# richarddurbin/hash10x

Hardware: AMD Instinct MI355X
Metric: read-pairs/s through --readFQB + --hashDepthRange + --cluster (mosh construction + per-barcode clustering) (higher is better)
Workload: dtype u64; 1 GPU; yeast-like-2.5M; read_pairs=2500000, barcodes=10000, B=24, k=21, w=31, clusterThreshold=5, parallelism=single GPU

## Files before the change

### hash10x_amd/csrc/common.hpp

```cpp
#pragma once
#include <hip/hip_runtime.h>
#include <cstdint>
#include <cstdio>
#include <cstdarg>
#include <cstring>
#include <cstdlib>
#include <ctime>
#include <string>
#include <vector>
#include <map>
#include <mutex>
#include "../../include/h10x.h"

namespace h10x {

constexpr int WAVE = 64;
typedef unsigned long long u64;
typedef uint32_t u32;
typedef uint16_t u16;
typedef uint8_t  u8;

static_assert(sizeof(h10x_block) == 32, "ClusterBlock layout (hash10x.c:62-70)");
static_assert(sizeof(h10x_clushash) == 8, "ClusterHash layout (hash10x.c:35-43)");

struct DevCache {
  std::multimap<size_t, void *> parked; size_t parkedBytes = 0;
  static std::mutex &mu() { static std::mutex m; return m; }
  static DevCache &of(int device, hipStream_t st) { static std::map<std::pair<int, hipStream_t>, DevCache> m; return m[{device, st}]; }
  static bool disabled() { static int v = -1; if (v < 0) v = getenv("H10X_NOPOOL") != nullptr; return v != 0; }
  static unsigned long long &freshCalls() { static unsigned long long v = 0; return v; }
  static unsigned long long &freshBytes() { static unsigned long long v = 0; return v; }
  static int poison() { static int p = -1; if (p < 0) { const char *e = getenv("H10X_POISON"); p = e ? atoi(e) : 0; } return p; }
  void *takeLocked(size_t bytes, size_t &got) {
    auto it = parked.lower_bound(bytes);
    if (it == parked.end() || it->first > 2 * bytes + (1u << 20)) return nullptr;
    void *p = it->second; got = it->first; parkedBytes -= got; parked.erase(it);
    return p;
  }
  static void *take(int device, hipStream_t st, size_t bytes, size_t &got) {
    std::lock_guard<std::mutex> g(mu());
    void *p = of(device, st).takeLocked(bytes, got);
    if (!p && st) p = of(device, nullptr).takeLocked(bytes, got);
    return p;
  }
  static void park(int device, hipStream_t st, void *p, size_t bytes) {
    std::lock_guard<std::mutex> g(mu()); DevCache &c = of(device, st); c.parked.emplace(bytes, p); c.parkedBytes += bytes;
  }
  static void retireStream(int device, hipStream_t st) {
    std::lock_guard<std::mutex> g(mu());
    DevCache &c = of(device, st), &idle = of(device, nullptr);
    for (auto &kv : c.parked) { idle.parked.emplace(kv.first, kv.second); idle.parkedBytes += kv.first; }
    c.parked.clear(); c.parkedBytes = 0;
  }
  static void trim(int device) {
    std::lock_guard<std::mutex> g(mu());
    (void)hipDeviceSynchronize();
    static std::map<std::pair<int, hipStream_t>, DevCache> *dummy = nullptr; (void)dummy;
    for (hipStream_t st : streamsOf(device)) { DevCache &c = of(device, st); for (auto &kv : c.parked) (void)hipFree(kv.second); c.parked.clear(); c.parkedBytes = 0; }
  }
  static std::vector<hipStream_t> &streamsOf(int device) { static std::map<int, std::vector<hipStream_t>> m; auto &v = m[device]; if (v.empty()) v.push_back(nullptr); return v; }
  static void noteStream(int device, hipStream_t st) { std::lock_guard<std::mutex> g(mu()); auto &v = streamsOf(device); for (auto x : v) if (x == st) return; v.push_back(st); }
};
struct AllocScope {
  static hipStream_t &stream() { static thread_local hipStream_t s = nullptr; return s; }
  static int &device() { static thread_local int d = 0; return d; }
};
template <typename T> struct DevBuf {
  T *p = nullptr; size_t n = 0; size_t cap = 0; int dev = 0; hipStream_t st = nullptr;
  DevBuf() = default;
  DevBuf(const DevBuf &) = delete; DevBuf &operator=(const DevBuf &) = delete;
  ~DevBuf() { release(); }
  void release() {
    if (p) { if (DevCache::disabled()) (void)hipFree(p); else DevCache::park(dev, st, p, cap); }
    p = nullptr; n = 0; cap = 0;
  }
  hipError_t alloc(size_t count) {
    release();
    if (!count) count = 1;
    size_t bytes = (count * sizeof(T) + 255) & ~(size_t)255;
    dev = AllocScope::device(); st = AllocScope::stream();
    hipError_t e = hipSuccess;
    void *q = DevCache::disabled() ? nullptr : DevCache::take(dev, st, bytes, cap);
    if (!q) {
      static const bool log = getenv("H10X_ALLOC_LOG") != nullptr;
      timespec t0, t1; if (log) clock_gettime(CLOCK_MONOTONIC, &t0);
      cap = bytes; e = hipMalloc(&q, bytes);
      if (e != hipSuccess && !DevCache::disabled()) { DevCache::trim(dev); e = hipMalloc(&q, bytes); }
      if (e == hipSuccess) { __atomic_fetch_add(&DevCache::freshCalls(), 1, __ATOMIC_RELAXED); __atomic_fetch_add(&DevCache::freshBytes(), (unsigned long long)bytes, __ATOMIC_RELAXED); }
      if (log) { clock_gettime(CLOCK_MONOTONIC, &t1); fprintf(stderr, "h10x alloc: %.1f MB fresh, %.3f ms\n", bytes / 1e6, (t1.tv_sec - t0.tv_sec) * 1e3 + (t1.tv_nsec - t0.tv_nsec) / 1e6); }
    }
    if (e == hipSuccess) { p = (T *)q; n = count; } else { p = nullptr; cap = 0; }
    if (e == hipSuccess && DevCache::poison()) (void)hipMemsetAsync(p, 0xA5, bytes, AllocScope::stream());
    return e;
  }
  void swap(DevBuf &o) { std::swap(p, o.p); std::swap(n, o.n); std::swap(cap, o.cap); std::swap(dev, o.dev); std::swap(st, o.st); }
  size_t bytes() const { return n * sizeof(T); }
};

enum TimerId { T_RUNS = 0, T_MOSH, T_FALLBACK, T_COMPACT, T_SORT_HASH, T_RANK, T_PROBE, T_CLUSHASH, T_CSR,
               T_GOOD, T_CLUSTER, T_CLUSTER_K, T_CLUSTER_MAIN, T_SPLIT, T_COUNT };
static const char *const kTimerNames[T_COUNT] = {
  "block_runs", "mosh_extract", "mosh_fallback", "compact_entries", "sort_by_hash", "index_rank",
  "probe_table", "clushash_build", "csr_build", "good_hashes", "cluster", "cluster_kernel", "cluster_main", "cluster_split" };

struct Timer { hipEvent_t a = nullptr, b = nullptr; double ms = 0; uint64_t launches = 0; bool pending = false; };

enum XchgId { X_HOST_COUNTS = 0, X_ENTRIES, X_FIRST_COUNTS, X_INDEX_BACK, X_INDEX_DEPTH, X_LIST_HEADS, X_LIST_DATA, X_TABLES, X_OWNER_LISTS, X_GATHER, X_COUNT };
static const char *const kXchgNames[X_COUNT] = {
  "host_counts (small host allgathers: sizes, counts)", "entries_to_hash_owners (all-to-all)", "first_seen_counts (allgather)", "indices_back (all-to-all)",
  "index_depth (allgather)", "list_heads (allgather: index + length of the in-range hashes)", "list_data (allgather: the in-range barcode lists)",
  "hash_tables (allgather: hashValue, for --writeHash / the crib)", "owner_lists_rebuild (after --clusterSplit)", "gather_to_rank0" };
struct XchgStat { u64 calls = 0, bytesOut = 0, bytesIn = 0, maxPeerOut = 0; Timer t, tIn; int beside = -1; };

constexpr size_t ROWS_PAD = 128;
constexpr int MAX_SEGS = 8;
struct BlockSeg { u32 localStart, count, globalBase; };
struct SegMap {
  int n; BlockSeg s[MAX_SEGS];
  __host__ __device__ u32 globalOf(u32 l) const {
    for (int k = n - 1; k > 0; --k) if (l >= s[k].localStart) return s[k].globalBase + (l - s[k].localStart);
    return s[0].globalBase + l;
  }
};
struct ShardSegInfo { u32 rank, localStart, count, globalBase; u64 entries; };

struct Ctx {
  h10x_params prm{};
  u64 keyInv = 1; int keyShift = 0; int keyBits = 64;
  bool wantPacked = false; int entCodeBits = 0;
  int device = 0;
  hipStream_t stream = nullptr;
  hipStream_t aux[3] = {nullptr, nullptr, nullptr};
  hipEvent_t evFork = nullptr, evJoin[3] = {nullptr, nullptr, nullptr};
  int numCU = 256;
  bool ownStream = false;
  std::string err;

  DevBuf<u32> hashIndex;
  DevBuf<u64> hashValue;
  DevBuf<u32> hashDepth;
  DevBuf<u64> rowStart;
  DevBuf<u32> rows;
  DevBuf<h10x_block> blocks;
  DevBuf<u64> blockOff;
  DevBuf<h10x_clushash> clusHash;
  u32 hashNumber = 1, nBlocks = 0;
  u32 maxBlockHashes = 0xFFFFFFFFu;
  u64 nEntries = 0, nRecords = 0;
  bool haveState = false;

  DevBuf<u8>  within;
  DevBuf<u16> goodPos;
  DevBuf<u32> nGood;
  DevBuf<u64> goodRow;
  DevBuf<u32> goodEntries;
  DevBuf<u32> clusterRaw;
  bool haveRange = false, haveGood = false; int rangeMin = 0, rangeMax = 0;
  u32 rangeHiMax = 0;
  u32 depthBound = 0xFFFFFFFFu;
  u32 maxGoodDepth = 0, maxGood = 0, meanGood = 0;

  DevBuf<u32> cribCount[2];
  DevBuf<u64> cribFirst[2];
  DevBuf<int16_t> cribChr; DevBuf<u16> cribPos; DevBuf<u8> cribType;
  DevBuf<u32> cribHist;
  u32 cribHistDim = 0; int cribGenomes = 0; bool haveCrib = false;

  struct Comm *comm = nullptr; bool sharded = false;
  u32 codeBase = 0, nBlocksGlobal = 0;
  SegMap segs{1, {{0, 0, 0}}};
  std::vector<ShardSegInfo> allSegs;
  u64 nEntriesGlobal = 0, nRecordsGlobal = 0;
  int rowShift = 0;
  bool ownerListsStale = false;
  DevBuf<u32> oRows, oSegStart, oIndex; u32 oU = 0; u64 oM = 0;
  DevBuf<u64> oHash;
  bool tablesPending = false;

  int64_t optMaxSlots = 0;
  int64_t optClusterLds = 0;
  int64_t optFirstGlobal = 0;
  int64_t optFirstCap = 0;
  int64_t optClusterThreads0 = 0, optClusterBudget0 = 0;
  int64_t optBigRanks = 0;
  int64_t optPrivTable = 0;
  int64_t optProbedTable = 0;
  int64_t optNoPack = 0;
  int64_t optNarrowFirst = 0;
  int64_t optTrEstDiv = 0;
  int64_t optTrClassT = -1;
  int64_t optTrPacked = -1;
  int64_t optStamps = 0;
  int64_t optChunk = 0;
  int64_t optChunkEof = 1;
  std::vector<u64> mergePoints; bool replayDone = false;
  int64_t optRowShift = -1;
  int64_t optReplySort = 0;
  int64_t optOverlap = 1;
  int64_t optOwnerCut = 0;
  int64_t optDeltaLists = -1;
  int64_t optRowsFakeBase = 0;
  int64_t optNbBudget = 0;
  u64 nbStats[4] = {0, 0, 0, 0};
  DevBuf<u32> censusKeys; u64 censusN = 0; bool censusOpen = false;
  DevBuf<u32> censusCodes, censusCounts, censusGoodCodes, censusGoodCounts; u64 censusDistinct = 0, censusGood = 0; bool censusClosed = false;
  DevBuf<u64> wlSlots; u64 wlMask = 0, wlCodes = 0; bool haveWhitelist = false;
  int64_t optFqbSlab = 0;
  int64_t optMolGlobal = 0;
  DevBuf<u32> sgBlock, sgCount; DevBuf<u64> sgOffsets; u64 sgRows = 0; u32 sgCodeMin = 0, sgCodeMax = 0; bool haveShareGraph = false;
  DevBuf<u32> ingestBuf; u64 ingestRecords = 0, ingestCap = 0; bool ingestAsync = false;
  static constexpr int INGEST_SLOTS = 8; hipEvent_t ingestEv[INGEST_SLOTS] = {};
  int64_t optFaultInject = 0;
  int faultAt(int region) { if (optFaultInject != region) return 0; optFaultInject = 0; return fail("injected fault in fork/join region %d", region); }
  bool timing = false;
  u32 *startFlags = nullptr;
  Timer timers[T_COUNT];
  XchgStat xs[X_COUNT];
  h10x_counters ctr{};

  int fail(const char *fmt, ...) {
    char buf[1024]; va_list ap; va_start(ap, fmt); vsnprintf(buf, sizeof buf, fmt, ap); va_end(ap);
    err = buf; return -1;
  }
  static constexpr size_t MAIL_BYTES = 4096, MAIL_ITEMS = 12;
  unsigned char *mail = nullptr; size_t mailUsed = 0; u32 mailSeq = 0; bool mailDirect = false;
  struct PendingRead { void *dst; const void *dev; size_t off, n; };
  std::vector<PendingRead> pendingReads;
  int readback(void *dst, const void *dev, size_t n) {
    if (!mail) {
      if (hipHostMalloc((void **)&mail, MAIL_BYTES + 64, hipHostMallocCoherent | hipHostMallocMapped) != hipSuccess) { mail = nullptr; return fail("hipHostMalloc of the read-back mailbox failed"); }
      memset(mail, 0, MAIL_BYTES + 64);
    }
    const size_t off = mailUsed, step = (n + 7) & ~(size_t)7;
    if (off + step > MAIL_BYTES || pendingReads.size() >= MAIL_ITEMS) {
      mailDirect = true;
      return hipMemcpyAsync(dst, dev, n, hipMemcpyDeviceToHost, stream) == hipSuccess ? 0 : fail("hipMemcpyAsync (device to host) failed");
    }
    mailUsed += step; pendingReads.push_back(PendingRead{dst, dev, off, n});
    return 0;
  }
  int syncReadbacks();
  int forkStreams(int n) {
    if (!evFork) {
      if (hipEventCreateWithFlags(&evFork, hipEventDisableTiming) != hipSuccess) return fail("hipEventCreate failed");
      for (int i = 0; i < 3; ++i) {
        if (hipStreamCreateWithFlags(&aux[i], hipStreamNonBlocking) != hipSuccess) return fail("hipStreamCreate failed");
        if (hipEventCreateWithFlags(&evJoin[i], hipEventDisableTiming) != hipSuccess) return fail("hipEventCreate failed");
      }
    }
    if (hipEventRecord(evFork, stream) != hipSuccess) return fail("hipEventRecord failed");
    for (int i = 0; i < n; ++i) if (hipStreamWaitEvent(aux[i], evFork, 0) != hipSuccess) return fail("hipStreamWaitEvent failed");
    return 0;
  }
  hipStream_t xStream = nullptr; hipEvent_t evXFork = nullptr, evXDone = nullptr; bool xOpen = false;
  DevBuf<u32> xHold[4];
  int xFork() {
    if (!xStream) {
      if (hipStreamCreateWithFlags(&xStream, hipStreamNonBlocking) != hipSuccess) return fail("hipStreamCreate failed");
      if (hipEventCreateWithFlags(&evXFork, hipEventDisableTiming) != hipSuccess || hipEventCreateWithFlags(&evXDone, hipEventDisableTiming) != hipSuccess) return fail("hipEventCreate failed");
    }
    if (hipEventRecord(evXFork, stream) != hipSuccess || hipStreamWaitEvent(xStream, evXFork, 0) != hipSuccess) return fail("hipStreamWaitEvent failed");
    xOpen = true;
    return 0;
  }
  int xJoin() {
    if (!xOpen) return 0;
    xOpen = false;
    if (hipEventRecord(evXDone, xStream) != hipSuccess || hipStreamWaitEvent(stream, evXDone, 0) != hipSuccess) return fail("hipStreamWaitEvent failed");
    for (auto &b : xHold) b.release();
    return 0;
  }
  int joinStreams(int n) {
    for (int i = 0; i < n; ++i) {
      if (hipEventRecord(evJoin[i], aux[i]) != hipSuccess) return fail("hipEventRecord failed");
      if (hipStreamWaitEvent(stream, evJoin[i], 0) != hipSuccess) return fail("hipStreamWaitEvent failed");
    }
    return 0;
  }
  void tstart(Timer &x) {
    if (!timing) return;
    if (!x.a) { (void)hipEventCreate(&x.a); (void)hipEventCreate(&x.b); }
    flush(x);
    (void)hipEventRecord(x.a, stream);
  }
  void tstop(Timer &x) {
    if (!timing) return;
    (void)hipEventRecord(x.b, stream); x.pending = true; ++x.launches;
  }
  void flush(Timer &x) {
    if (x.pending) { float ms = 0; (void)hipEventSynchronize(x.b); (void)hipEventElapsedTime(&ms, x.a, x.b); x.ms += ms; x.pending = false; }
  }
  static constexpr int STAGE_DEPTH = 8;
  TimerId stageStack[STAGE_DEPTH]; int stageOpen = 0;
  TimerId stageTop = T_COUNT;
  Timer stageWait[T_COUNT];
  void stageReset() { stageOpen = 0; stageTop = T_COUNT; }
  void tstart(TimerId t) { if (stageOpen < STAGE_DEPTH) stageStack[stageOpen] = t; ++stageOpen; stageTop = t; tstart(timers[t]); }
  void tstop(TimerId t) {
    if (stageOpen > 0) --stageOpen;
    stageTop = stageOpen > 0 && stageOpen <= STAGE_DEPTH ? stageStack[stageOpen - 1] : T_COUNT;
    tstop(timers[t]);
  }
  void flush(TimerId t) { flush(timers[t]); }
};

struct ForkGuard {
  Ctx *c; bool armed = true;
  explicit ForkGuard(Ctx *c_) : c(c_) {}
  ForkGuard(const ForkGuard &) = delete; ForkGuard &operator=(const ForkGuard &) = delete;
  ~ForkGuard() { if (!armed) return; for (int i = 0; i < 3; ++i) if (c->aux[i]) (void)hipStreamSynchronize(c->aux[i]); (void)hipStreamSynchronize(c->stream); }
  void done() { armed = false; }
};

struct XGuard {
  Ctx *c;
  explicit XGuard(Ctx *c_) : c(c_) {}
  XGuard(const XGuard &) = delete; XGuard &operator=(const XGuard &) = delete;
  ~XGuard() { if (!c->xOpen) return; (void)hipStreamSynchronize(c->xStream); c->xOpen = false; for (auto &b : c->xHold) b.release(); }
};

#define H10X_HIP(ctx, call)                                                                      \
  do { hipError_t e__ = (call);                                                                  \
       if (e__ != hipSuccess) return (ctx)->fail("HIP error %s at %s:%d: %s", hipGetErrorName(e__), __FILE__, __LINE__, #call); } while (0)

#define H10X_TRY(expr) do { int rc__ = (expr); if (rc__) return rc__; } while (0)

static inline unsigned divUp(u64 a, u64 b) { return (unsigned)((a + b - 1) / b); }
template <typename T> static inline T hmin(T a, T b) { return a < b ? a : b; }
template <typename T> static inline T hmax(T a, T b) { return a > b ? a : b; }

__device__ __forceinline__ u32 probe_find(const u32 *__restrict__ table, const u64 *__restrict__ hashValue, int B, u64 h) {
  const u64 mask = ((u64)1 << B) - 1;
  u64 slot = h & mask; const u64 step = ((h >> B) & mask) | 1;
  u32 ix;
  while ((ix = table[slot]) && hashValue[ix] != h) slot = (slot + step) & mask;
  return ix;
}

int stageA_run(Ctx *c, const u32 *dRecords, u64 nRecords,
               DevBuf<u64> &entHash, DevBuf<u32> &entCode, DevBuf<u32> &entRead, bool hashLast = false, bool emptyIsNoBlock = false);
int stageA_sortRecords(Ctx *c, const u32 *dIn, u64 nRecords, u32 *dOut);
int stageA_runStarts(Ctx *c, const u32 *dRec, u64 nRec, std::vector<u64> &starts, std::vector<u32> &zeroRuns);
int replayChunks(const std::vector<u64> &starts, const std::vector<u32> &zeroRuns, u64 chunk, std::vector<u64> &merges, bool eofPass);
int stageB_run(Ctx *c, DevBuf<u64> &entHash, DevBuf<u32> &entCode, DevBuf<u32> &entRead);
void warm_prim(hipStream_t), warm_stageA(hipStream_t), warm_stageB(hipStream_t), warm_stageC(hipStream_t), warm_stageD(hipStream_t), warm_stageE(hipStream_t), warm_stageF(hipStream_t), warm_shard(hipStream_t);
int stageB_buildCSR(Ctx *c);
int stageB_finishClusHash(Ctx *c, DevBuf<u64> &key);
int stageB_finishClusHashFromReplies(Ctx *c, const u32 *replyIdx, const u32 *replyPos, const u32 *entRead);
#ifndef H10X_BS_T0
#define H10X_BS_T0 512
#define H10X_BS_I0 6
#define H10X_BS_T1 1024
#define H10X_BS_I1 6
#endif
constexpr u32 BLOCK_SORT_CAP0 = H10X_BS_T0 * H10X_BS_I0, BLOCK_SORT_CAP1 = H10X_BS_T1 * H10X_BS_I1, BLOCK_SORT_MAX = 8192;
int stageB_buildProbeTable(Ctx *c);
int stageB_blockClassLists(Ctx *c, DevBuf<u32> &lists, DevBuf<u32> &counts);
int stageC_depthRange(Ctx *c, int min, int max);
int stageC_cluster(Ctx *c, int codeMin, int codeMax, int threshold);
int stageC_split(Ctx *c);
int stageC_readMerge(Ctx *c, u32 code);
int stageD_cribGenome(Ctx *c, const u8 *hostCodes, const u64 *seqStart, u32 nSeq, int which, u64 *nPresent, u64 *nAbsent);
int stageD_cribFinish(Ctx *c);
int stageE_histMax(Ctx *c, int which, u64 first, u64 count, u32 *maxValue);
int stageE_histogram(Ctx *c, int which, u64 first, u64 count, u32 bins, u64 *hist);
int stageE_clusterReport(Ctx *c, u32 firstBlock, u32 nBlk, h10x_block_rep *hostB, h10x_cluster_rep *hostC, u64 clusterCap, u64 *nClusters);
int stageE_cribSummary(Ctx *c, u64 *counts12, u32 *hostSeenBase, u32 *hostSeenCluster);
int stageE_cribWords(Ctx *c, u64 first, u64 count, u32 *hostOut);
int stageF_neighbours(Ctx *c, u32 x, u32 *hash, u32 *count, u32 *first, u64 cap, u64 *n);
int stageF_neighbourMax(Ctx *c, const u32 *xs, u32 nq, u64 *maxKey, u32 *nNb);
int stageF_neighbourHist(Ctx *c, const u32 *xs, u32 nq, const u64 *offsets, u32 *hist);
int stageF_codeShare(Ctx *c, const u32 *codes, u32 nq, u64 *offsets, u32 *barcode, u32 *count, u32 *firstRank, u32 *firstHash, u64 cap);
int stageF_codeExplore(Ctx *c, int code, int threshold, u32 *out );
int stageF_codeCrib(Ctx *c, const u32 *codes, u32 n, u32 *out);
int stageL_run(Ctx *c, int64_t minShare, u32 codeMin, u32 codeMax, h10x_share_graph_info *info);
int stageL_get(Ctx *c, u64 *offsets, u32 *block, u32 *count, u64 cap, int toDevice);
void stageL_release(Ctx *c);
int stageJ_censusBegin(Ctx *c, u64 hint);
int stageJ_censusAdd(Ctx *c, const u32 *dRec, u64 n);
int stageJ_censusClose(Ctx *c, int64_t thresh, h10x_census_t *out);
int stageJ_censusExport(Ctx *c, int goodOnly, u32 *codes, u32 *counts, u64 cap);
int stageJ_whitelistSet(Ctx *c, const u32 *hostCodes, u64 n);
int stageJ_fix(Ctx *c, const u32 *dIn, u64 n, u32 *dOut, u64 *nKept, h10x_fix_stats *acc);
u64 stageJ_slab(const Ctx *c);
int stageK_map(Ctx *c, u32 *dMol, u32 *dSlot, u64 cap, h10x_molmap_info *info);
int stageK_records(Ctx *c, u64 *nRecords);
int stageK_split(Ctx *c, const u32 *dIn, u64 n, u32 *dOut, u64 *hostStart, u64 startCap);
int shard_allreduceU64(Ctx *c, u64 *v, u32 n, int op);
int shard_gatherBytes(Ctx *c, const void *send, u64 nbytes, void *recv, u64 cap, u64 *counts);
int shard_exchangeRows(Ctx *c);
int shard_split(Ctx *c, const u32 *dSubBefore, u32 totalSubLocal);
int shard_refreshLayout(Ctx *c);
int shard_materializeTables(Ctx *c);

// ... 47 lines not shown
```

### hash10x_amd/csrc/h10x_api.hip

```cpp
#include "common.hpp"
#include "comm.hpp"
#include "build_id.h"
#include <cstdlib>
#include <ctime>
#include <new>
#include <stdexcept>

using namespace h10x;

static int enter(Ctx &c) {
  if (hipSetDevice(c.device) != hipSuccess) return c.fail("hipSetDevice(%d) failed", c.device);
  AllocScope::stream() = c.stream; AllocScope::device() = c.device;
  DevCache::noteStream(c.device, c.stream);
  c.pendingReads.clear(); c.mailUsed = 0; c.mailDirect = false;
  c.stageReset();
  return 0;
}

struct h10x_ctx { Ctx c; };

extern "C" {

int h10x_abi_version(void) { return H10X_ABI_VERSION; }
const char *h10x_build_id(void) { return H10X_BUILD_ID; }
// ... 729 lines not shown

int h10x_molecule_map_device(h10x_ctx *h, uint32_t *dMol, uint32_t *dSlot, uint64_t cap, h10x_molmap_info *info) {
  if (!h) return -1;
  Ctx &c = h->c; H10X_TRY(enter(c));
  return stageK_map(&c, dMol, dSlot, cap, info);
}
int h10x_molecule_map(h10x_ctx *h, uint32_t *mol, uint32_t *slot, uint64_t cap, h10x_molmap_info *info) {
  if (!h) return -1;
  Ctx &c = h->c; H10X_TRY(enter(c));
  if (!mol && !slot) return stageK_map(&c, nullptr, nullptr, 0, info);
  u64 R = 0;
  H10X_TRY(stageK_records(&c, &R));
  if (cap < R) return c.fail("moleculeMap: room for %llu entries, the state holds %llu records", (u64)cap, R);
  DevBuf<u32> dMol, dSlot;
  if (mol) H10X_HIP(&c, dMol.alloc(R));
  if (slot) H10X_HIP(&c, dSlot.alloc(R));
  H10X_TRY(stageK_map(&c, mol ? dMol.p : nullptr, slot ? dSlot.p : nullptr, R, info));
  if (mol && R) H10X_HIP(&c, hipMemcpyAsync(mol, dMol.p, R * 4, hipMemcpyDeviceToHost, c.stream));
  if (slot && R) H10X_HIP(&c, hipMemcpyAsync(slot, dSlot.p, R * 4, hipMemcpyDeviceToHost, c.stream));
  H10X_HIP(&c, hipStreamSynchronize(c.stream));
  return 0;
}
int h10x_split_fqb_device(h10x_ctx *h, const uint32_t *dIn, uint64_t n, uint32_t *dOut, uint64_t *start, uint64_t startCap) {
  if (!h) return -1;
  Ctx &c = h->c; H10X_TRY(enter(c));
  if (n && (!dIn || !dOut)) return c.fail("h10x_split_fqb_device: null buffer");
  return stageK_split(&c, dIn, n, dOut, (u64 *)start, startCap);
}
int h10x_split_fqb(h10x_ctx *h, const uint32_t *in, uint64_t n, uint32_t *out, uint64_t *start, uint64_t startCap) {
  if (!h) return -1;
  Ctx &c = h->c; H10X_TRY(enter(c));
  if (n && (!in || !out)) return c.fail("h10x_split_fqb: null buffer");
  u64 R = 0;
  H10X_TRY(stageK_records(&c, &R));
  if (n != R) return c.fail("splitFQB: %llu records given, the state was read from %llu", (u64)n, R);
  if (n) { const uintptr_t a = (uintptr_t)in, b = (uintptr_t)out; if (a < b + n * 120 && b < a + n * 120) return c.fail("splitFQB: the input and output buffers overlap"); }
  DevBuf<u32> dIn, dOut;
  H10X_HIP(&c, dIn.alloc(n * 30)); H10X_HIP(&c, dOut.alloc(n * 30));
  if (n) H10X_HIP(&c, hipMemcpyAsync(dIn.p, in, n * 120, hipMemcpyHostToDevice, c.stream));
  H10X_TRY(stageK_split(&c, dIn.p, n, dOut.p, (u64 *)start, startCap));
  if (n) H10X_HIP(&c, hipMemcpyAsync(out, dOut.p, n * 120, hipMemcpyDeviceToHost, c.stream));
  H10X_HIP(&c, hipStreamSynchronize(c.stream));
  return 0;
}

int h10x_crib_genome(h10x_ctx *h, const uint8_t *codes, const uint64_t *seqStart, uint32_t nSeq, int which, uint64_t *nPresent, uint64_t *nAbsent) {
  if (!h) return -1;
  Ctx &c = h->c; H10X_TRY(enter(c));
  if (!seqStart || (seqStart[nSeq] && !codes)) return c.fail("h10x_crib_genome: null argument");
  return stageD_cribGenome(&c, codes, (const u64 *)seqStart, nSeq, which, (u64 *)nPresent, (u64 *)nAbsent);
}
int h10x_crib_finish(h10x_ctx *h) { if (!h) return -1; Ctx &c = h->c; H10X_TRY(enter(c)); return stageD_cribFinish(&c); }
int h10x_crib_sizes(h10x_ctx *h, uint32_t *histDim, uint32_t arrayMax[4]) {
  if (!h) return -1;
  Ctx &c = h->c; H10X_TRY(enter(c));
  if (!c.haveCrib) return c.fail("no crib: use cribBuild first");
  if (histDim) *histDim = c.cribHistDim;
  if (arrayMax) { H10X_HIP(&c, hipMemcpyAsync(arrayMax, c.cribHist.p + (size_t)4 * c.cribHistDim, 16, hipMemcpyDeviceToHost, c.stream)); H10X_HIP(&c, hipStreamSynchronize(c.stream)); }
  return 0;
}
int h10x_crib_export(h10x_ctx *h, int16_t *chr, uint16_t *pos, uint8_t *type, uint32_t *hist) {
  if (!h) return -1;
  Ctx &c = h->c; H10X_TRY(enter(c));
  if (!c.haveCrib) return c.fail("no crib: use cribBuild first");
  const size_t U1 = c.hashNumber;
  if (chr) H10X_HIP(&c, hipMemcpyAsync(chr, c.cribChr.p, U1 * 2, hipMemcpyDeviceToHost, c.stream));
  if (pos) H10X_HIP(&c, hipMemcpyAsync(pos, c.cribPos.p, U1 * 2, hipMemcpyDeviceToHost, c.stream));
  if (type) H10X_HIP(&c, hipMemcpyAsync(type, c.cribType.p, U1, hipMemcpyDeviceToHost, c.stream));
  if (hist) H10X_HIP(&c, hipMemcpyAsync(hist, c.cribHist.p, (size_t)4 * c.cribHistDim * 4, hipMemcpyDeviceToHost, c.stream));
  H10X_HIP(&c, hipStreamSynchronize(c.stream));
  return 0;
}
int h10x_export_ngood(h10x_ctx *h, uint32_t *nGood) {
  if (!h || !nGood) return -1;
  Ctx &c = h->c; H10X_TRY(enter(c));
  if (!c.haveGood) return c.fail("!! you must set hashDepthRange before clusterReport");
  H10X_HIP(&c, hipMemcpyAsync(nGood, c.nGood.p, (size_t)c.nBlocks * 4, hipMemcpyDeviceToHost, c.stream));
  H10X_HIP(&c, hipStreamSynchronize(c.stream));
  return 0;
}

int h10x_get_counters(h10x_ctx *h, h10x_counters *out) { if (!h || !out) return -1; *out = h->c.ctr; return 0; }

int h10x_shard_info(h10x_ctx *h, h10x_shard_info_t *out) {
  if (!h || !out) return -1;
  Ctx &c = h->c;
  if (!c.haveState) return c.fail("no hash state loaded: use readFQB or readHash first");
  memset(out, 0, sizeof *out);
  out->rank = c.sharded ? c.comm->rank : 0; out->nranks = c.sharded ? c.comm->n : 1;
  out->hashNumber = c.hashNumber; out->B = c.prm.B;
  if (c.sharded) { out->nBlocksGlobal = c.nBlocksGlobal; out->nEntriesGlobal = c.nEntriesGlobal; out->nRecordsGlobal = c.nRecordsGlobal; out->nSegs = (uint32_t)c.allSegs.size(); }
  else { out->nBlocksGlobal = c.nBlocks; out->nEntriesGlobal = c.nEntries; out->nRecordsGlobal = c.nRecords; out->nSegs = c.nBlocks > 1 ? 1 : 0; }
  return 0;
}
int h10x_shard_segments(h10x_ctx *h, h10x_shard_seg *out, uint32_t cap) {
  if (!h || !out) return -1;
  Ctx &c = h->c; H10X_TRY(enter(c));
  if (!c.haveState) return c.fail("no hash state loaded: use readFQB or readHash first");
  if (!c.sharded) {
    if (c.nBlocks <= 1) return 0;
    if (cap < 1) return c.fail("h10x_shard_segments: room for %u segments, 1 needed", cap);
    out[0] = h10x_shard_seg{0, 1, c.nBlocks - 1, 1, c.nEntries, 0, 0};
    return 0;
  }
  if (cap < c.allSegs.size()) return c.fail("h10x_shard_segments: room for %u segments, %zu needed", cap, c.allSegs.size());
  u64 g = 0;
  for (size_t i = 0; i < c.allSegs.size(); ++i) {
    const ShardSegInfo &s = c.allSegs[i];
    u64 local = 0;
    if ((int)s.rank == c.comm->rank) H10X_HIP(&c, hipMemcpy(&local, c.blockOff.p + s.localStart, 8, hipMemcpyDeviceToHost));
    out[i] = h10x_shard_seg{s.rank, s.localStart, s.count, s.globalBase, s.entries, local, g};
    g += s.entries;
  }
  return 0;
}
int h10x_shard_prepare_export(h10x_ctx *h) {
  if (!h) return -1;
  Ctx &c = h->c; H10X_TRY(enter(c));
  if (!c.haveState) return c.fail("no hash state loaded: use readFQB or readHash first");
  if (!c.sharded) return 0;
  return shard_materializeTables(&c);
}
int h10x_export_slice(h10x_ctx *h, int table, uint64_t first, uint64_t count, void *dst) {
  if (!h) return -1;
  Ctx &c = h->c; H10X_TRY(enter(c));
  if (!c.haveState) return c.fail("no hash state loaded: use readFQB or readHash first");
  if (!count) return 0;
  if (!dst) return c.fail("h10x_export_slice: null destination");
  const void *src = nullptr; size_t eb = 0; u64 limit = 0;
  switch (table) {
    case H10X_TABLE_HASHINDEX: src = c.hashIndex.p; eb = 4; limit = (u64)1 << c.prm.B; break;
    case H10X_TABLE_HASHVALUE: src = c.hashValue.p; eb = 8; limit = c.hashNumber; break;
    case H10X_TABLE_HASHDEPTH: src = c.hashDepth.p; eb = 4; limit = c.hashNumber; break;
    case H10X_TABLE_BLOCKS:    src = c.blocks.p; eb = sizeof(h10x_block); limit = c.nBlocks; break;
    case H10X_TABLE_CLUSHASH:  src = c.clusHash.p; eb = sizeof(h10x_clushash); limit = c.nEntries; break;
    case H10X_TABLE_CLUSTER_RAW: if (!c.clusterRaw.p || c.clusterRaw.n != 2 * (size_t)c.nBlocks) return c.fail("no --cluster has run on these blocks"); src = c.clusterRaw.p; eb = 8; limit = c.nBlocks; break;
    case H10X_TABLE_WITHIN:    if (!c.haveRange) return c.fail("no hashDepthRange set"); src = c.within.p; eb = 1; limit = c.hashNumber; break;
    case H10X_TABLE_NGOOD:     if (!c.haveGood) return c.fail("!! you must set hashDepthRange before clusterReport"); src = c.nGood.p; eb = 4; limit = c.nBlocks; break;
    default: return c.fail("h10x_export_slice: unknown table %d", table);
  }
  if ((table == H10X_TABLE_HASHINDEX || table == H10X_TABLE_HASHVALUE) && c.tablesPending) return c.fail("h10x_export_slice: call h10x_shard_prepare_export first (collective)");
  if (!src || first > limit || count > limit - first) return c.fail("h10x_export_slice: table %d, range %llu + %llu outside %llu", table, (u64)first, (u64)count, (u64)limit);
  H10X_HIP(&c, hipMemcpyAsync(dst, (const char *)src + first * eb, count * eb, hipMemcpyDeviceToHost, c.stream));
  H10X_HIP(&c, hipStreamSynchronize(c.stream));
  return 0;
}

int h10x_set_option(h10x_ctx *h, const char *name, int64_t value) {
  if (!h || !name) return -1;
  if (!strcmp(name, "stage_a_max_slots")) {
    if (value && (value < 256 || value > 16384 || (value & (value - 1)))) return h->c.fail("stage_a_max_slots must be a power of two in 256..16384 (or 0)");
    h->c.optMaxSlots = value; return 0;
  }
  if (!strcmp(name, "cluster_lds_budget")) { h->c.optClusterLds = value; return 0; }
  if (!strcmp(name, "cluster_first_global")) { h->c.optFirstGlobal = value; return 0; }
  if (!strcmp(name, "cluster_first_cap")) { h->c.optFirstCap = value; return 0; }
  if (!strcmp(name, "cluster_threads0")) { h->c.optClusterThreads0 = value; return 0; }
  if (!strcmp(name, "cluster_budget0")) { h->c.optClusterBudget0 = value; return 0; }
  if (!strcmp(name, "cluster_big_ranks")) { h->c.optBigRanks = value; return 0; }
  if (!strcmp(name, "cluster_narrow_first")) { h->c.optNarrowFirst = value; return 0; }
  if (!strcmp(name, "cluster_tr_packed")) { h->c.optTrPacked = value; return 0; }
  if (!strcmp(name, "cluster_tr_class_t")) { h->c.optTrClassT = value; return 0; }
  if (!strcmp(name, "cluster_tr_est_div")) { h->c.optTrEstDiv = value; return 0; }
  if (!strcmp(name, "index_no_pack")) { h->c.optNoPack = value; return 0; }
  if (!strcmp(name, "index_probed_table")) { if (value < 0 || value > 3) return h->c.fail("index_probed_table must be 0..3"); h->c.optProbedTable = value; return 0; }
  if (!strcmp(name, "index_priv_table")) { if (value < 0 || value > 3) return h->c.fail("index_priv_table must be 0..3"); h->c.optPrivTable = value; return 0; }
  if (!strcmp(name, "cluster_stamps")) { h->c.optStamps = value; return 0; }
  if (!strcmp(name, "chunk_size")) { if (value < 0) return h->c.fail("chunk_size must be >= 0"); h->c.optChunk = value; return 0; }
  if (!strcmp(name, "chunk_eof_pass")) { h->c.optChunkEof = value ? 1 : 0; return 0; }
  if (!strcmp(name, "fault_inject")) { h->c.optFaultInject = value; return 0; }
  if (!strcmp(name, "shard_row_shift")) { if (value < -1 || value > 8) return h->c.fail("shard_row_shift must be -1..8"); h->c.optRowShift = value; return 0; }
  if (!strcmp(name, "shard_reply_sort")) { if (value < 0 || value > 4) return h->c.fail("shard_reply_sort must be 0..4"); h->c.optReplySort = value; return 0; }
  if (!strcmp(name, "shard_overlap")) { h->c.optOverlap = value ? 1 : 0; return 0; }
  if (!strcmp(name, "shard_owner_cut")) { if (value < 0 || value > 1) return h->c.fail("shard_owner_cut must be 0 or 1"); h->c.optOwnerCut = value; return 0; }
  if (!strcmp(name, "shard_delta_lists")) { if (value < -1 || value > 1) return h->c.fail("shard_delta_lists must be -1, 0 or 1"); h->c.optDeltaLists = value; return 0; }
  if (!strcmp(name, "shard_rows_fake_base")) { if (value < 0) return h->c.fail("shard_rows_fake_base must be >= 0"); h->c.optRowsFakeBase = value; return 0; }
  if (!strcmp(name, "molmap_global")) { if (value < 0 || value > 1) return h->c.fail("molmap_global must be 0 or 1"); h->c.optMolGlobal = value; return 0; }
  if (!strcmp(name, "fqb_slab")) { if (value < 0 || value > (1 << 28)) return h->c.fail("fqb_slab must be 0..2^28"); h->c.optFqbSlab = value; return 0; }
  if (!strcmp(name, "neighbour_budget")) { if (value < 0) return h->c.fail("neighbour_budget must be >= 0"); h->c.optNbBudget = value; return 0; }
  return h->c.fail("unknown option %s", name);
}

}
```

### hash10x_amd/csrc/prim.hip

```cpp
#include "prim.hpp"
#include <thread>
#include <rocprim/rocprim.hpp>

namespace h10x {

#define PRIM_TWO_PHASE(c, t, CALL)                                                               \
  do { size_t bytes = 0; void *tmp = nullptr;                                                    \
       hipError_t e = (CALL);                                                                    \
       if (e != hipSuccess) return (c)->fail("rocPRIM size query failed: %s", hipGetErrorName(e)); \
       if (bytes > (t).buf.n) { e = (t).buf.alloc(bytes + (bytes >> 2));                         \
         if (e != hipSuccess) return (c)->fail("out of device memory for %zu bytes of sort/scan scratch", bytes); } \
       tmp = (t).buf.p;                                                                          \
       e = (CALL);                                                                               \
       if (e != hipSuccess) return (c)->fail("rocPRIM call failed: %s", hipGetErrorName(e)); } while (0)

int prim_exclusive_scan_u32(Ctx *c, PrimTemp &t, const u32 *in, u32 *out, size_t n) {
  if (!n) return 0;
  PRIM_TWO_PHASE(c, t, rocprim::exclusive_scan(tmp, bytes, in, out, (u32)0, n, rocprim::plus<u32>(), c->stream));
  return 0;
}
struct RunHead {
  const u64 *key; size_t n; int cb;
  __device__ u32 operator()(size_t i) const { return (i < n && (i == 0 || (key[i] >> cb) != (key[i - 1] >> cb))) ? 1u : 0u; }
};
int prim_run_ordinals_u64(Ctx *c, PrimTemp &t, const u64 *key, int cb, u32 *ord, size_t n) {
  auto flags = rocprim::make_transform_iterator(rocprim::counting_iterator<size_t>(0), RunHead{key, n, cb});
  PRIM_TWO_PHASE(c, t, rocprim::exclusive_scan(tmp, bytes, flags, ord, (u32)0, n + 1, rocprim::plus<u32>(), c->stream));
  return 0;
}
int prim_exclusive_scan_u32_u64(Ctx *c, PrimTemp &t, const u32 *in, u64 *out, size_t n) {
  if (!n) return 0;
  auto in64 = rocprim::make_transform_iterator(in, [] __device__(u32 v) -> u64 { return (u64)v; });
  PRIM_TWO_PHASE(c, t, rocprim::exclusive_scan(tmp, bytes, in64, out, (u64)0, n, rocprim::plus<u64>(), c->stream));
  return 0;
}
int prim_inclusive_scan_u32(Ctx *c, PrimTemp &t, const u32 *in, u32 *out, size_t n) {
  if (!n) return 0;
  PRIM_TWO_PHASE(c, t, rocprim::inclusive_scan(tmp, bytes, in, out, n, rocprim::plus<u32>(), c->stream));
  return 0;
}
int prim_sort_pairs_u64_u32(Ctx *c, PrimTemp &t, const u64 *kin, u64 *kout, const u32 *vin, u32 *vout, size_t n, int b0, int b1) {
  if (!n) return 0;
  PRIM_TWO_PHASE(c, t, rocprim::radix_sort_pairs(tmp, bytes, kin, kout, vin, vout, n, (unsigned)b0, (unsigned)b1, c->stream));
  return 0;
}
int prim_sort_pairs_u32_u32(Ctx *c, PrimTemp &t, const u32 *kin, u32 *kout, const u32 *vin, u32 *vout, size_t n, int b0, int b1) {
  if (!n) return 0;
  PRIM_TWO_PHASE(c, t, rocprim::radix_sort_pairs(tmp, bytes, kin, kout, vin, vout, n, (unsigned)b0, (unsigned)b1, c->stream));
  return 0;
}
struct MailArgs { const unsigned char *src[Ctx::MAIL_ITEMS]; u32 off[Ctx::MAIL_ITEMS], n[Ctx::MAIL_ITEMS]; u32 count; };
__global__ void mail_post_kernel(MailArgs a, unsigned char *mail, u32 *flag, u32 seq) {
  for (u32 i = 0; i < a.count; ++i)
    for (u32 b = threadIdx.x; b < a.n[i]; b += blockDim.x) mail[a.off[i] + b] = a.src[i][b];
  __threadfence_system();
  __syncthreads();
  if (threadIdx.x == 0) __hip_atomic_store(flag, seq, __ATOMIC_RELEASE, __HIP_MEMORY_SCOPE_SYSTEM);
}
int Ctx::syncReadbacks() {
  hipError_t e = hipSuccess;
  if (pendingReads.empty() || mailDirect) e = hipStreamSynchronize(stream);
  if (!pendingReads.empty() && e == hipSuccess) {
    MailArgs a; a.count = (u32)pendingReads.size();
    for (u32 i = 0; i < a.count; ++i) { a.src[i] = (const unsigned char *)pendingReads[i].dev; a.off[i] = (u32)pendingReads[i].off; a.n[i] = (u32)pendingReads[i].n; }
    u32 *flag = (u32 *)(mail + MAIL_BYTES);
    const u32 seq = ++mailSeq ? mailSeq : ++mailSeq;
    mail_post_kernel<<<1, 64, 0, stream>>>(a, mail, flag, seq);
    e = hipGetLastError();
    for (u64 spins = 0; e == hipSuccess && __atomic_load_n(flag, __ATOMIC_ACQUIRE) != seq; ++spins) {
#if !defined(__HIP_DEVICE_COMPILE__)
#if defined(__x86_64__) || defined(__i386__)
      __builtin_ia32_pause();
#else
      std::this_thread::yield();
#endif
#endif
      if ((spins & 0xFFF) == 0xFFF) {
        const hipError_t q = hipStreamQuery(stream);
        if (q == hipErrorNotReady) continue;
        if (q == hipSuccess && __atomic_load_n(flag, __ATOMIC_ACQUIRE) == seq) break;
        e = q == hipSuccess ? hipErrorUnknown : q;
      }
    }
    if (e == hipSuccess) for (const PendingRead &r : pendingReads) memcpy(r.dst, mail + r.off, r.n);
  }
  pendingReads.clear(); mailUsed = 0; mailDirect = false;
  return e == hipSuccess ? 0 : fail("HIP error %s at a read-back", hipGetErrorString(e));
}

int prim_sort_pairs_u32_v16(Ctx *c, PrimTemp &t, const u32 *kin, u32 *kout, const Val16 *vin, Val16 *vout, size_t n, int b0, int b1) {
  if (!n) return 0;
  PRIM_TWO_PHASE(c, t, rocprim::radix_sort_pairs(tmp, bytes, kin, kout, vin, vout, n, (unsigned)b0, (unsigned)b1, c->stream));
  return 0;
}
using SortKeys64Config = rocprim::radix_sort_config<rocprim::default_config, rocprim::default_config,
    rocprim::radix_sort_onesweep_config<rocprim::kernel_config<1024, 8>, rocprim::kernel_config<1024, 8>, 8, rocprim::block_radix_rank_algorithm::match>, 1024 * 1024>;
int prim_sort_keys_u64(Ctx *c, PrimTemp &t, const u64 *kin, u64 *kout, size_t n, int b0, int b1) {
  if (!n) return 0;
  PRIM_TWO_PHASE(c, t, rocprim::radix_sort_keys<SortKeys64Config>(tmp, bytes, kin, kout, n, (unsigned)b0, (unsigned)(b1 > 64 ? 64 : b1), c->stream));
  return 0;
}
int prim_sort_keys_u32(Ctx *c, PrimTemp &t, const u32 *kin, u32 *kout, size_t n, int b0, int b1) {
  if (!n) return 0;
  PRIM_TWO_PHASE(c, t, rocprim::radix_sort_keys(tmp, bytes, kin, kout, n, (unsigned)b0, (unsigned)(b1 > 32 ? 32 : b1), c->stream));
  return 0;
}
int prim_seg_sort_keys_u64(Ctx *c, PrimTemp &t, const u64 *kin, u64 *kout, u32 n, u32 nSeg, const u32 *begin, const u32 *end, int b0, int b1) {
  if (!n || !nSeg) return 0;
  PRIM_TWO_PHASE(c, t, rocprim::segmented_radix_sort_keys(tmp, bytes, kin, kout, n, nSeg, begin, end, (unsigned)b0, (unsigned)b1, c->stream));
  return 0;
}
int prim_seg_sort_keys_u32(Ctx *c, PrimTemp &t, const u32 *kin, u32 *kout, u32 n, u32 nSeg, const u32 *begin, const u32 *end, int b0, int b1) {
  if (!n || !nSeg) return 0;
  PRIM_TWO_PHASE(c, t, rocprim::segmented_radix_sort_keys(tmp, bytes, kin, kout, n, nSeg, begin, end, (unsigned)b0, (unsigned)b1, c->stream));
  return 0;
}
int prim_reduce_max_u32(Ctx *c, PrimTemp &t, const u32 *in, u32 *out, size_t n) {
  PRIM_TWO_PHASE(c, t, rocprim::reduce(tmp, bytes, in, out, (u32)0, n, rocprim::maximum<u32>(), c->stream));
  return 0;
}
int prim_reduce_sum_u32_u64(Ctx *c, PrimTemp &t, const u32 *in, u64 *out, size_t n) {
  auto in64 = rocprim::make_transform_iterator(in, [] __device__(u32 v) -> u64 { return (u64)v; });
  PRIM_TWO_PHASE(c, t, rocprim::reduce(tmp, bytes, in64, out, (u64)0, n, rocprim::plus<u64>(), c->stream));
  return 0;
}

__global__ void warm_prim_kernel() {}
void warm_prim(hipStream_t st) { warm_prim_kernel<<<1, 1, 0, st>>>(); }

}
```

### hash10x_amd/csrc/stage_a.hip

```cpp
#include "common.hpp"
#include <algorithm>
#include "prim.hpp"

namespace h10x {

constexpr u64 EMPTY64 = ~0ULL;
constexpr u32 NHASH_OVERFLOW = 0xFFFFFFFFu;
constexpr int MOSH_THREADS = 256;
constexpr int REC_TILE = 16;
constexpr int SEQ_WORDS = 12;

struct MoshConst {
  int k, w, shift1;
  int n1, n2;
  int run;
  u64 factor1;
};
#define H10X_MOSH_DBG(bit) false

__device__ __forceinline__ u64 kmer_window(const u32 *seq, int p, int k) {
  const int wi = p >> 4, s = (p & 15) * 2;
  const u64 hi = ((u64)seq[wi] << 32) | (u64)seq[wi + 1];
  const u32 lo = seq[wi + 2];
  const u64 x = s ? ((hi << s) | (u64)(lo >> (32 - s))) : hi;
  return x >> (64 - 2 * k);
}

__device__ __forceinline__ u64 revcomp_word(u64 x, int k) {
  u64 r = __brevll(~x);
  r = ((r & 0xAAAAAAAAAAAAAAAAULL) >> 1) | ((r & 0x5555555555555555ULL) << 1);
  return r >> (64 - 2 * k);
}

template <bool W31>
__device__ __forceinline__ bool divisible(u64 h, int w) {
  if (W31) {
    const u32 s = (u32)(h & 0x3FFFFFFFu) + (u32)((h >> 30) & 0x3FFFFFFFu) + (u32)(h >> 60);
    return (s % 31u) == 0;
  }
  return (h % (u64)w) == 0;
}

template <bool W31>
__device__ __forceinline__ bool mosh_of_slot(const u32 *seq, int t, const MoshConst &mc, u64 &h) {
  int p; const u32 *s;
  if (t < mc.n1) { p = 23 + t; s = seq; }
  else { p = t - mc.n1; s = seq + SEQ_WORDS; }
  const u64 f = kmer_window(s, p, mc.k);
  const u64 r = revcomp_word(f, mc.k);
  const u64 hf = (f * mc.factor1) >> mc.shift1;
  const u64 hr = (r * mc.factor1) >> mc.shift1;
  h = hf < hr ? hf : hr;
  return divisible<W31>(h, mc.w);
}

__device__ __forceinline__ void stage_records(const u32 *__restrict__ rec, u64 firstRec, int cnt, u32 *tile) {
  for (int t = threadIdx.x; t < cnt * 20; t += blockDim.x) {
    const int rr = t / 20, wi = t - rr * 20;
    const u32 v = rec[(firstRec + rr) * 30 + (wi < 10 ? wi : wi + 5)];
    tile[rr * 2 * SEQ_WORDS + (wi < 10 ? wi : wi + 2)] = v;
  }
}

__global__ void head_flags_kernel(const u32 *__restrict__ rec, u64 n, u32 *__restrict__ flags) {
  u64 i = (u64)blockIdx.x * blockDim.x + threadIdx.x;
  const u64 stride = (u64)gridDim.x * blockDim.x;
  for (; i < n; i += stride) flags[i] = (i == 0 || rec[i * 30] != rec[(i - 1) * 30]) ? 1u : 0u;
}

__global__ void block_starts_kernel(const u32 *__restrict__ flags, const u32 *__restrict__ code, u64 n, u32 nBlocks,
                                    u64 *__restrict__ startRec ) {
  u64 i = (u64)blockIdx.x * blockDim.x + threadIdx.x;
  const u64 stride = (u64)gridDim.x * blockDim.x;
  if (i == 0) { startRec[0] = 0; startRec[nBlocks] = n; }
  for (; i < n; i += stride) if (flags[i]) startRec[code[i]] = i;
}

__global__ void clear_heads_kernel(u32 *__restrict__ flags, const u64 *__restrict__ at, u32 n) {
  const u32 i = blockIdx.x * blockDim.x + threadIdx.x;
  if (i < n) flags[at[i]] = 0;
}
__global__ void zero_runs_kernel(const u32 *__restrict__ rec, const u64 *__restrict__ startRec, u32 nBlocks, u32 *__restrict__ list, u32 cap, u32 *__restrict__ count) {
  const u32 b = blockIdx.x * blockDim.x + threadIdx.x + 1;
  if (b < nBlocks && rec[startRec[b] * 30] == 0) { const u32 p = atomicAdd(count, 1u); if (p < cap) list[p] = b - 1; }
}

__global__ void classify_kernel(const u64 *__restrict__ startRec, u32 nBlocks, h10x_block *__restrict__ blocks,
                                u32 *__restrict__ slots, u32 maxSlots, int packedOK,
                                u32 *__restrict__ list0, u32 *__restrict__ list1, u32 *__restrict__ list2, u32 *__restrict__ listF,
                                u32 *__restrict__ counts , int hashLast) {
  const u32 c = blockIdx.x * blockDim.x + threadIdx.x;
  const int lane = threadIdx.x & (WAVE - 1);
  int cls = -1; u32 s = 0;
  if (c < nBlocks) {
    h10x_block b; memset(&b, 0, sizeof b);
    if (c > 0) {
      const u64 nr = startRec[c + 1] - startRec[c];
      b.nRead = (u32)nr;
      if (c + 1 < nBlocks || hashLast) {
        u64 want = 256; while (want < nr * 10) want <<= 1;
        if (packedOK && nr <= 65535 && want <= maxSlots) { s = (u32)want; cls = s <= 4096 ? 0 : (s <= 8192 ? 1 : 2); }
        else cls = 3;
      }
    }
    blocks[c] = b; slots[c] = s;
  }
  u32 *const lists[4] = {list0, list1, list2, listF};
#pragma unroll
  for (int k = 0; k < 4; ++k) {
    const u64 bal = __ballot(cls == k);
    if (!bal) continue;
    u32 base = 0;
    if (lane == 0) base = atomicAdd(&counts[k], (u32)__popcll(bal));
    base = (u32)__shfl((int)base, 0);
    if (cls == k) lists[k][base + (u32)__popcll(bal & ((1ULL << lane) - 1))] = c;
  }
}

__device__ __forceinline__ u32 lo32(u64 x) { return (u32)x; }
__device__ __forceinline__ u32 hi32(u64 x) { return (u32)(x >> 32); }
__device__ __forceinline__ u64 mk64(u32 hi, u32 lo) { return ((u64)hi << 32) | lo; }
__device__ __forceinline__ bool entry_empty(u64 v) {
  u32 t = lo32(v) & hi32(v);
  asm("" : "+v"(t));
  return t == 0xFFFFFFFFu;
}
__device__ __forceinline__ u32 set_slot_of(u32 hLo, u32 hHi, u32 mask) {
  return (((hLo ^ (hHi * 0x9E3779B1u)) * 0x85EBCA6Bu) >> 15) & mask;
}
__device__ __forceinline__ bool probe_done(u64 *table, u32 slot, u64 cur, u32 pLo, u32 pHi) {
  if (entry_empty(cur)) return true;
  if (hi32(cur) == pHi && ((lo32(cur) ^ pLo) >> 16) == 0) { atomicMin((u64 *)&table[slot], mk64(pHi, pLo)); return true; }
  return false;
}
constexpr u32 MOSH_QCAP = 96, MOSH_QKEEP = MOSH_QCAP - WAVE;
typedef __attribute__((address_space(3))) volatile u64 lds_queue_t;
__device__ __forceinline__ void queue_push(lds_queue_t *q, u32 &qn , bool ok, u32 hLo, u32 hHi, u32 read16 ) {
  const u64 bal = __builtin_amdgcn_ballot_w64(ok);
  if (!bal) return;
  const u32 pre = __builtin_amdgcn_mbcnt_hi((u32)(bal >> 32), __builtin_amdgcn_mbcnt_lo((u32)bal, 0u));
  if (ok) q[qn + pre] = mk64(hHi | read16, hLo);
  qn += (u32)__popcll(bal);
}
__device__ __forceinline__ bool queue_drain(u64 *table, u32 mask, lds_queue_t *q, u32 &qn, int lane) {
  const u32 n = qn < (u32)WAVE ? qn : (u32)WAVE;
  qn -= n;
  bool go = (u32)lane < n;
  u64 raw = 0;
  if (go) raw = q[qn + lane];
  const u32 hLo = lo32(raw), hHi = hi32(raw) & 0xFFFFu;
  const u32 pLo = (hLo << 16) | (hi32(raw) >> 16), pHi = __builtin_amdgcn_alignbit(hHi, hLo, 16);
  const u64 packed = mk64(pHi, pLo);
  u32 slot = set_slot_of(hLo, hHi, mask);
  for (u32 probes = 0; __builtin_amdgcn_ballot_w64(go); ++probes) {
    if (probes > mask) return false;
    if (go) {
      const u64 cur = atomicCAS((u64 *)&table[slot], EMPTY64, packed);
      if (probe_done(table, slot, cur, pLo, pHi)) go = false; else slot = (slot + 1) & mask;
    }
  }
  return true;
}

__device__ __forceinline__ void mul64_lo(u32 xLo, u32 xHi, u32 fLo, u32 fHi, u32 &pLo, u32 &pHi) {
  const u64 p = (u64)xLo * fLo;
  pLo = lo32(p); pHi = hi32(p) + xLo * fHi + xHi * fLo;
}

__device__ __forceinline__ void min64_halves(u32 aLo, u32 aHi, u32 bLo, u32 bHi, u32 &mLo, u32 &mHi) {
  asm("v_sub_co_u32 %0, vcc, %2, %4\n\tv_subb_co_u32 %0, vcc, %3, %5, vcc\n\tv_cndmask_b32 %0, %4, %2, vcc\n\tv_cndmask_b32 %1, %5, %3, vcc"
      : "=&v"(mLo), "=&v"(mHi) : "v"(aLo), "v"(aHi), "v"(bLo), "v"(bHi) : "vcc");
}
__device__ __forceinline__ u64 roll_product(u64 p, u64 t) {
  u64 r;
  asm("v_lshl_add_u64 %0, %1, 2, %2" : "=v"(r) : "v"(p), "v"(t));
  return r;
}
__device__ __forceinline__ void revcomp_halves(u32 lo, u32 hi, int down , u32 &rLo, u32 &rHi) {
  u32 a = __builtin_bitreverse32(~lo), b = __builtin_bitreverse32(~hi);
  a = ((a >> 1) & 0x55555555u) | ((a << 1) & 0xAAAAAAAAu);
  b = ((b >> 1) & 0x55555555u) | ((b << 1) & 0xAAAAAAAAu);
  rLo = __builtin_amdgcn_alignbit(a, b, (u32)down); rHi = a >> down;
}

template <bool W31, int L , bool FAST>
__global__ __launch_bounds__(1024)
void mosh_lds_kernel(const u32 *__restrict__ rec, const u32 *__restrict__ list, u32 nList,
                     const u64 *__restrict__ startRec, const u32 *__restrict__ slots, const u64 *__restrict__ capOff,
                     MoshConst mc, u32 tableBytes ,
                     u64 *__restrict__ stHash, u32 *__restrict__ stRead, u32 *__restrict__ nHashOut) {
  extern __shared__ __align__(16) unsigned char smem[];
  if (blockIdx.x >= nList) return;
  const u32 code = list[blockIdx.x];
  const u32 S = slots[code], mask = S - 1;
  u64 *table = (u64 *)smem;
  lds_queue_t *queue = (lds_queue_t *)(smem + tableBytes) + (u32)__builtin_amdgcn_readfirstlane((int)(threadIdx.x / WAVE)) * MOSH_QCAP;
  u32 qn = 0;
  __shared__ u32 sOverflow, sCount;
  __shared__ u64 sRoll[32];
  const u64 rec0 = startRec[code];
  const u32 nRead = (u32)(startRec[code + 1] - rec0);

  for (u32 i = threadIdx.x; i < S; i += blockDim.x) table[i] = EMPTY64;
  if (threadIdx.x == 0) { sOverflow = 0; sCount = 0; }
  if (FAST && threadIdx.x < 16) {
    const u64 a = threadIdx.x >> 2, b = threadIdx.x & 3, top = mc.factor1 << (2 * mc.k);
    sRoll[2 * threadIdx.x] = b * mc.factor1 - a * top;
    sRoll[2 * threadIdx.x + 1] = (3 - a) * mc.factor1 - (3 - b) * top;
  }
  __syncthreads();

  const int lane = threadIdx.x & (WAVE - 1), sub = lane & 31, wv = threadIdx.x / WAVE;
  const int lanes1 = (mc.n1 + L - 1) / L, lanes2 = (mc.n2 + L - 1) / L;
  int cnt = 0, pos0 = 0, wordBase = 0;
  if (sub < lanes1) { int t0 = sub * L; if (FAST) t0 = min(t0, mc.n1 - L); cnt = min(L, mc.n1 - t0); pos0 = 23 + t0; }
  else if (sub < lanes1 + lanes2) { int t0 = (sub - lanes1) * L; if (FAST) t0 = min(t0, mc.n2 - L); cnt = min(L, mc.n2 - t0); pos0 = t0; wordBase = 15; }
  const int sh = (pos0 & 15) * 2;
  const int wi = wordBase + (pos0 >> 4) - (FAST && sh == 0 ? 1 : 0);
  const u32 unal = (u32)(32 - sh) & 31u;
  const int k2 = 2 * mc.k, down = 64 - k2;
  const u32 pairsPerRound = (blockDim.x / WAVE) * 2;
  const u32 fLo = lo32(mc.factor1), fHi = hi32(mc.factor1);
  u32 r = (u32)wv * 2 + (u32)(lane >> 5);
  uint4 nx = make_uint4(0, 0, 0, 0);
  const u32 *pn = rec + (rec0 + r) * 30 + wi;
  if (r < nRead && cnt > 0) nx = make_uint4(pn[0], pn[1], pn[2], pn[3]);
  for (; __builtin_amdgcn_ballot_w64(r < nRead); r += pairsPerRound) {
    const uint4 cw = nx;
    const u32 rn = r + pairsPerRound;
    pn += (size_t)pairsPerRound * 30;
    if (rn < nRead && cnt > 0 && !H10X_MOSH_DBG(512)) nx = make_uint4(pn[0], pn[1], pn[2], pn[3]);
    if (H10X_MOSH_DBG(512)) nx = make_uint4(cw.y * 0x9E3779B1u + r, cw.x ^ 0x85EBCA6Bu, cw.w + cw.x, cw.z * 5u + 1u);
    const bool live = r < nRead && !H10X_MOSH_DBG(32);
    if (FAST) {
      const u32 x0 = __builtin_amdgcn_alignbit(cw.x, cw.y, unal), x1 = __builtin_amdgcn_alignbit(cw.y, cw.z, unal), x2 = __builtin_amdgcn_alignbit(cw.z, cw.w, unal);
      const u32 inw = __builtin_amdgcn_alignbit(x1, x2, (u32)down);
      u32 ta[L - 1];
      if constexpr (L == 8) {
        const u32 ze = (x0 & 0xCCCCCCCCu) | ((inw >> 2) & 0x33333333u), zo = ((x0 << 2) & 0xCCCCCCCCu) | (inw & 0x33333333u);
        const u32 zes = ze << 4, zos = zo << 4;
        ta[0] = (ze >> 24) & 0xF0u; ta[1] = (zo >> 24) & 0xF0u; ta[2] = (zes >> 24) & 0xF0u; ta[3] = (zos >> 24) & 0xF0u;
        ta[4] = (ze >> 16) & 0xF0u; ta[5] = (zo >> 16) & 0xF0u; ta[6] = (zes >> 16) & 0xF0u;
#pragma unroll
        for (int j = 0; j < L - 1; ++j) asm("" : "+v"(ta[j]));
      } else {
#pragma unroll
        for (int j = 0; j < L - 1; ++j) { ta[j] = (((x0 >> (30 - 2 * j)) & 3u) << 6) | (((inw >> (30 - 2 * j)) & 3u) << 4); asm("" : "+v"(ta[j])); }
      }
      u64 pr[L];
      {
        const u32 g0 = __builtin_amdgcn_alignbit(x0, x1, 32 - 2 * (L - 1)), g1 = __builtin_amdgcn_alignbit(x1, x2, 32 - 2 * (L - 1));
        u32 rl, rh;
        revcomp_halves(__builtin_amdgcn_alignbit(g0, g1, (u32)down), g0 >> down, down, rl, rh);
        u32 pl, ph;
        mul64_lo(rl, rh, fLo, fHi, pl, ph);
        pr[L - 1] = mk64(ph, pl);
      }
#pragma unroll
      for (int j = L - 2; j >= 0; --j) pr[j] = roll_product(pr[j + 1], *(const u64 *)((const char *)sRoll + ta[j] + 8));
      u64 pf;
      { u32 pl, ph; mul64_lo(__builtin_amdgcn_alignbit(x0, x1, (u32)down), x0 >> down, fLo, fHi, pl, ph); pf = mk64(ph, pl); }
      u32 thr = live && cnt > 0 ? 0xFFFFFFFFu / 31u + 1u : 0u;
      asm("" : "+v"(thr));
      const u32 r16 = r << 16;
#pragma unroll
      for (int j = 0; j < L; ++j) {
        u64 t = 0;
        if (j < L - 1) t = *(const u64 *)((const char *)sRoll + ta[j]);
        u32 mL, mH;
        min64_halves(lo32(pf), hi32(pf), lo32(pr[j]), hi32(pr[j]), mL, mH);
        const u32 hL = __builtin_amdgcn_alignbit(mH, mL, (u32)down), hH = mH >> down;
        bool ok;
        if (W31) ok = ((hL & 0x3FFFFFFFu) + __builtin_amdgcn_alignbit(hH, hL, 30)) * 0xBDEF7BDFu < thr;
        else ok = (mk64(hH, hL) % (u64)mc.w) == 0 && thr != 0;
        queue_push(queue, qn, ok, hL, hH, r16);
        if (H10X_MOSH_DBG(16)) { if (qn > MOSH_QKEEP) qn = 0; }
        else if (qn > MOSH_QKEEP && !queue_drain(table, mask, queue, qn, lane)) sOverflow = 1;
        if (j < L - 1) pf = roll_product(pf, t);
      }
      continue;
    }
    u64 hi = ((u64)cw.x << 32) | cw.y, lo = ((u64)cw.z << 32) | cw.w;
    if (sh) { hi = (hi << sh) | (lo >> (64 - sh)); lo <<= sh; }
    u64 f = hi >> down;
    u64 rc = revcomp_word(f, mc.k);
#pragma unroll
    for (int j = 0; j < L; ++j) {
      const u64 hf = (f * mc.factor1) >> mc.shift1;
      const u64 hr = (rc * mc.factor1) >> mc.shift1;
      const u64 h = hf < hr ? hf : hr;
      queue_push(queue, qn, divisible<W31>(h, mc.w) && live && j < cnt, lo32(h), hi32(h), r << 16);
      if (qn > MOSH_QKEEP && !queue_drain(table, mask, queue, qn, lane)) sOverflow = 1;
      hi = (hi << 2) | (lo >> 62); lo <<= 2;
      f = hi >> down;
      rc = (rc >> 2) | ((u64)(3u - ((u32)f & 3u)) << (k2 - 2));
    }
  }
  while (qn) if (!queue_drain(table, mask, queue, qn, lane)) { sOverflow = 1; break; }
  __syncthreads();

  const u64 out0 = capOff[code];
  const u32 cap = S - (S >> 3);
  for (u32 base = 0; base < (H10X_MOSH_DBG(64) ? 0u : S); base += blockDim.x) {
    const u32 i = base + threadIdx.x;
    const u64 v = i < S ? table[i] : EMPTY64;
    const bool valid = !entry_empty(v);
    const u64 bal = __ballot(valid);
    const int lane = threadIdx.x & (WAVE - 1);
    u32 wbase = 0;
    if (lane == 0 && bal) wbase = atomicAdd(&sCount, (u32)__popcll(bal));
    wbase = __shfl(wbase, 0);
    if (valid) {
      const u32 pos = wbase + (u32)__popcll(bal & ((1ULL << lane) - 1));
      if (pos < cap) { stHash[out0 + pos] = mk64(hi32(v) >> 16, __builtin_amdgcn_alignbit(hi32(v), lo32(v), 16)); stRead[out0 + pos] = lo32(v) & 0xFFFFu; }
    }
  }
  __syncthreads();
  if (threadIdx.x == 0) {
    u32 n = sCount;
    if (sOverflow || n > cap) n = NHASH_OVERFLOW;
    else if (n == 0) { stHash[out0] = 0; stRead[out0] = 0; n = 1; }
    nHashOut[code] = n;
  }
}

template <bool W31>
__global__ __launch_bounds__(MOSH_THREADS)
void mosh_raw_kernel(const u32 *__restrict__ rec, u64 rec0, u32 nRead, MoshConst mc, u64 *__restrict__ rawKey, u32 *__restrict__ rawSlot) {
  __shared__ u32 tile[REC_TILE * 2 * SEQ_WORDS];
  const int nk = mc.n1 + mc.n2;
  for (u32 i = threadIdx.x; i < REC_TILE * 2 * SEQ_WORDS; i += blockDim.x) tile[i] = 0;
  for (u32 r0 = blockIdx.x * REC_TILE; r0 < nRead; r0 += gridDim.x * REC_TILE) {
    const int cnt = (int)min((u32)REC_TILE, nRead - r0);
    __syncthreads();
    stage_records(rec, rec0 + r0, cnt, tile);
    __syncthreads();
    for (int rr = 0; rr < cnt; ++rr)
      for (int t = threadIdx.x; t < nk; t += blockDim.x) {
        u64 h; const bool ok = mosh_of_slot<W31>(tile + rr * 2 * SEQ_WORDS, t, mc, h);
        const u64 slot = (u64)(r0 + rr) * nk + t;
        rawKey[slot] = ok ? h : EMPTY64;
        rawSlot[slot] = (u32)slot;
      }
  }
}

__global__ void unique_flags_kernel(const u64 *__restrict__ key, u64 n, u32 *__restrict__ flags) {
  u64 i = (u64)blockIdx.x * blockDim.x + threadIdx.x;
  const u64 stride = (u64)gridDim.x * blockDim.x;
  for (; i < n; i += stride) flags[i] = (key[i] != EMPTY64 && (i == 0 || key[i] != key[i - 1])) ? 1u : 0u;
}
__global__ void unique_scatter_kernel(const u64 *__restrict__ key, const u32 *__restrict__ slot, const u32 *__restrict__ flags,
                                      const u32 *__restrict__ pos, u64 n, u32 nk, u64 *__restrict__ outHash, u32 *__restrict__ outRead) {
  u64 i = (u64)blockIdx.x * blockDim.x + threadIdx.x;
  const u64 stride = (u64)gridDim.x * blockDim.x;
  for (; i < n; i += stride) if (flags[i]) { outHash[pos[i]] = key[i]; outRead[pos[i]] = slot[i] / nk; }
}

__global__ void set_nhash_kernel(h10x_block *__restrict__ blocks, const u32 *__restrict__ nHash, u32 nBlocks) {
  const u32 c = blockIdx.x * blockDim.x + threadIdx.x;
  if (c < nBlocks) blocks[c].nHash = nHash[c];
}

struct SrcPtr { const u64 *hash; const u32 *read; };
__global__ void count_overflow_kernel(const u32 *__restrict__ nHash, u32 nBlocks, u32 *__restrict__ count) {
  const u32 c = blockIdx.x * blockDim.x + threadIdx.x;
  const u64 bal = __ballot(c < nBlocks && nHash[c] == NHASH_OVERFLOW);
  if ((threadIdx.x & (WAVE - 1)) == 0 && bal) atomicAdd(count, (u32)__popcll(bal));
}

__global__ void compact_entries_kernel(const u64 *__restrict__ stHash, const u32 *__restrict__ stRead, const u64 *__restrict__ capOff,
                                       const SrcPtr *__restrict__ fb ,
                                       const u32 *__restrict__ nHash, const u64 *__restrict__ blockOff, u32 nBlocks,
                                       u64 keyInv, int keyShift, int codeBits ,
                                       u64 *__restrict__ entHash, u32 *__restrict__ entCode, u32 *__restrict__ entRead) {
  for (u32 c = blockIdx.x + 1; c < nBlocks; c += gridDim.x) {
    const u32 n = nHash[c]; if (!n) continue;
    const u64 *sh; const u32 *sr;
    if (fb[c].hash) { sh = fb[c].hash; sr = fb[c].read; } else { sh = stHash + capOff[c]; sr = stRead + capOff[c]; }
    const u64 o = blockOff[c];
    if (codeBits) for (u32 i = threadIdx.x; i < n; i += blockDim.x) { entHash[o + i] = (((sh[i] >> keyShift) * keyInv) << codeBits) | c; entRead[o + i] = sr[i]; }
    else for (u32 i = threadIdx.x; i < n; i += blockDim.x) { entHash[o + i] = (sh[i] >> keyShift) * keyInv; entCode[o + i] = c; entRead[o + i] = sr[i]; }
  }
}

__global__ void sort_keys_kernel(const u32 *__restrict__ rec, u64 n, u32 *__restrict__ key, u32 *__restrict__ idx) {
  u64 i = (u64)blockIdx.x * blockDim.x + threadIdx.x;
  const u64 stride = (u64)gridDim.x * blockDim.x;
  for (; i < n; i += stride) { key[i] = __builtin_bswap32(rec[i * 30]); idx[i] = (u32)i; }
}
__global__ void gather_records_kernel(const u32 *__restrict__ rec, const u32 *__restrict__ idx, u64 n, u32 *__restrict__ out) {
  u64 t = (u64)blockIdx.x * blockDim.x + threadIdx.x;
  const u64 stride = (u64)gridDim.x * blockDim.x, total = n * 30;
  for (; t < total; t += stride) { const u64 j = t / 30; const u32 w = (u32)(t - j * 30); out[t] = rec[(u64)idx[j] * 30 + w]; }
}
int stageA_sortRecords(Ctx *c, const u32 *dIn, u64 n, u32 *dOut) {
  hipStream_t st = c->stream; PrimTemp pt;
  if (n >= (1ULL << 32)) return c->fail("record sort: %llu records exceed this build's 2^32 limit", (u64)n);
  if (!n) return 0;
  DevBuf<u32> key, keyS, idx, idxS;
  H10X_HIP(c, key.alloc(n)); H10X_HIP(c, keyS.alloc(n)); H10X_HIP(c, idx.alloc(n)); H10X_HIP(c, idxS.alloc(n));
  const unsigned g = (unsigned)hmin<u64>(divUp(n, 256), 65535u * 4);
  sort_keys_kernel<<<g, 256, 0, st>>>(dIn, n, key.p, idx.p);
  H10X_TRY(prim_sort_pairs_u32_u32(c, pt, key.p, keyS.p, idx.p, idxS.p, n, 0, 32));
  gather_records_kernel<<<(unsigned)hmin<u64>(divUp(n * 30, 256), 65535u * 16), 256, 0, st>>>(dIn, idxS.p, n, dOut);
  H10X_HIP(c, hipGetLastError());
  H10X_HIP(c, hipStreamSynchronize(st));
  return 0;
}

int replayChunks(const std::vector<u64> &starts, const std::vector<u32> &zeroRuns, u64 chunk, std::vector<u64> &merges, bool eofPass) {
  merges.clear();
  const size_t R = starts.size() - 1; const u64 total = starts[R];
  if (!R || !total) return 0;
  std::vector<u32> zr(zeroRuns); std::sort(zr.begin(), zr.end());
  auto isZero = [&](size_t r) { return std::binary_search(zr.begin(), zr.end(), (u32)r); };
  auto runOf = [&](u64 pos) { return (size_t)(std::upper_bound(starts.begin(), starts.begin() + R, pos) - starts.begin()) - 1; };
  std::vector<size_t> swallowed;
  u64 pos = 0, head = 0; bool open = false, barcodeZero = true;
  while (pos < total) {
    const u64 carry = open ? pos - head : 0;
    if (chunk <= carry) return 1;
    if (barcodeZero && open) {
      const size_t r = runOf(pos);
      if (starts[r] == pos) { merges.push_back(pos); swallowed.push_back(r); }
    }
    if (!open) { head = pos; open = true; }
    const u64 end = head + chunk < total ? head + chunk : total;
    size_t q = runOf(end - 1);
    barcodeZero = isZero(q);
    while (std::binary_search(swallowed.begin(), swallowed.end(), q)) --q;
    head = starts[q];
    pos = end;
  }
  if (eofPass && open && total - head >= chunk) return 1;
  return 0;
}

int stageA_runStarts(Ctx *c, const u32 *dRec, u64 nRec, std::vector<u64> &starts, std::vector<u32> &zeroRuns) {
  hipStream_t st = c->stream; PrimTemp pt;
  starts.assign(1, 0); zeroRuns.clear();
  if (!nRec) return 0;
  DevBuf<u32> flags, code; DevBuf<u64> startRec;
  H10X_HIP(c, flags.alloc(nRec)); H10X_HIP(c, code.alloc(nRec));
  const unsigned g = (unsigned)hmin<u64>(divUp(nRec, 256), 65535u * 4);
  head_flags_kernel<<<g, 256, 0, st>>>(dRec, nRec, flags.p);
  H10X_TRY(prim_inclusive_scan_u32(c, pt, flags.p, code.p, nRec));
  u32 nRuns = 0;
  H10X_TRY(c->readback(&nRuns, code.p + (nRec - 1), 4));
  H10X_TRY(c->syncReadbacks());
  const u32 nBlocks = nRuns + 1;
  H10X_HIP(c, startRec.alloc((size_t)nBlocks + 1));
  block_starts_kernel<<<g, 256, 0, st>>>(flags.p, code.p, nRec, nBlocks, startRec.p);
  constexpr u32 ZCAP = 4096;
  DevBuf<u32> zl, zc; H10X_HIP(c, zl.alloc(ZCAP)); H10X_HIP(c, zc.alloc(1)); H10X_HIP(c, hipMemsetAsync(zc.p, 0, 4, st));
  zero_runs_kernel<<<divUp(nBlocks, 256), 256, 0, st>>>(dRec, startRec.p, nBlocks, zl.p, ZCAP, zc.p);
  starts.resize((size_t)nRuns + 1);
  H10X_HIP(c, hipMemcpyAsync(starts.data(), startRec.p + 1, ((size_t)nRuns + 1) * 8, hipMemcpyDeviceToHost, st));
  u32 nz = 0;
  H10X_TRY(c->readback(&nz, zc.p, 4));
  H10X_TRY(c->syncReadbacks());
  if (nz > ZCAP) return c->fail("%u separate runs of the all-A barcode: the input is not grouped by barcode", nz);
  zeroRuns.resize(nz);
  if (nz) { H10X_HIP(c, hipMemcpyAsync(zeroRuns.data(), zl.p, (size_t)nz * 4, hipMemcpyDeviceToHost, st)); H10X_HIP(c, hipStreamSynchronize(st)); }
  return 0;
}

int stageA_run(Ctx *c, const u32 *dRec, u64 nRec, DevBuf<u64> &entHash, DevBuf<u32> &entCode, DevBuf<u32> &entRead, bool hashLast, bool emptyIsNoBlock) {
  hipStream_t st = c->stream;
  PrimTemp pt;
  const int k = c->prm.k;
  MoshConst mc; mc.k = k; mc.w = c->prm.w; mc.shift1 = 64 - 2 * k; mc.factor1 = c->prm.factor1;
  mc.n1 = 127 - k + 1 > 0 ? 127 - k + 1 : 0;
  mc.n2 = 150 - k + 1 > 0 ? 150 - k + 1 : 0;
  mc.run = 8; while ((mc.n1 + mc.run - 1) / mc.run + (mc.n2 + mc.run - 1) / mc.run > 32) ++mc.run;
  const bool w31 = c->prm.w == 31;

  c->tstart(T_RUNS);
  u32 nBlocks = 2;
  DevBuf<u64> startRec;
  if (nRec) {
    DevBuf<u32> flags, code;
    H10X_HIP(c, flags.alloc(nRec)); H10X_HIP(c, code.alloc(nRec));
    const unsigned g = (unsigned)hmin<u64>(divUp(nRec, 256), 65535u * 4);
    if (c->optChunk > 0 && !c->replayDone) {
      std::vector<u64> starts; std::vector<u32> zeroRuns;
      H10X_TRY(stageA_runStarts(c, dRec, nRec, starts, zeroRuns));
      if (replayChunks(starts, zeroRuns, (u64)c->optChunk, c->mergePoints, c->optChunkEof != 0)) return c->fail("chunkSize too small");
    }
    c->replayDone = false;
    head_flags_kernel<<<g, 256, 0, st>>>(dRec, nRec, flags.p);
    if (!c->mergePoints.empty()) {
      DevBuf<u64> at; H10X_HIP(c, at.alloc(c->mergePoints.size()));
      H10X_HIP(c, hipMemcpyAsync(at.p, c->mergePoints.data(), c->mergePoints.size() * 8, hipMemcpyHostToDevice, st));
      clear_heads_kernel<<<divUp(c->mergePoints.size(), 256), 256, 0, st>>>(flags.p, at.p, (u32)c->mergePoints.size());
      H10X_HIP(c, hipStreamSynchronize(st));
      c->mergePoints.clear();
    }
    H10X_TRY(prim_inclusive_scan_u32(c, pt, flags.p, code.p, nRec));
    u32 nRuns = 0;
    H10X_TRY(c->readback(&nRuns, code.p + (nRec - 1), 4));
    H10X_TRY(c->syncReadbacks());
    nBlocks = nRuns + 1;
    H10X_HIP(c, startRec.alloc((size_t)nBlocks + 1));
    block_starts_kernel<<<g, 256, 0, st>>>(flags.p, code.p, nRec, nBlocks, startRec.p);
  } else {
    if (emptyIsNoBlock) nBlocks = 1;
    H10X_HIP(c, startRec.alloc(3));
    H10X_HIP(c, hipMemsetAsync(startRec.p, 0, 24, st));
  }
  c->nBlocks = nBlocks; c->nRecords = nRec;
  H10X_HIP(c, c->blocks.alloc(nBlocks));

  u32 maxSlots = 16384;
  if (c->optMaxSlots > 0) maxSlots = (u32)c->optMaxSlots;
  const int packedOK = (2 * k + 16 <= 64) ? 1 : 0;
  DevBuf<u32> slots, list0, list1, list2, listF, counts, nHash;
  H10X_HIP(c, slots.alloc(nBlocks)); H10X_HIP(c, list0.alloc(nBlocks)); H10X_HIP(c, list1.alloc(nBlocks)); H10X_HIP(c, list2.alloc(nBlocks));
  H10X_HIP(c, listF.alloc(nBlocks)); H10X_HIP(c, counts.alloc(4)); H10X_HIP(c, nHash.alloc((size_t)nBlocks + 1));
  H10X_HIP(c, hipMemsetAsync(counts.p, 0, 16, st));
  H10X_HIP(c, hipMemsetAsync(nHash.p, 0, ((size_t)nBlocks + 1) * 4, st));
  classify_kernel<<<divUp(nBlocks, 256), 256, 0, st>>>(startRec.p, nBlocks, c->blocks.p, slots.p, maxSlots, packedOK,
                                                      list0.p, list1.p, list2.p, listF.p, counts.p, hashLast ? 1 : 0);
  DevBuf<u64> capOff; H10X_HIP(c, capOff.alloc((size_t)nBlocks + 1));
  H10X_TRY(prim_exclusive_scan_u32_u64(c, pt, slots.p, capOff.p, nBlocks));
  u32 hc[4]; u64 capTotal = 0; u32 lastSlots = 0;
  H10X_TRY(c->readback(hc, counts.p, 16));
  H10X_TRY(c->readback(&capTotal, capOff.p + (nBlocks - 1), 8));
  H10X_TRY(c->readback(&lastSlots, slots.p + (nBlocks - 1), 4));
  H10X_TRY(c->syncReadbacks());
  capTotal += lastSlots;
  c->tstop(T_RUNS);

  DevBuf<u64> stHash; DevBuf<u32> stRead;
  H10X_HIP(c, stHash.alloc(capTotal)); H10X_HIP(c, stRead.alloc(capTotal));
  c->tstart(T_MOSH);
  ForkGuard forkGuard(c);
  H10X_TRY(c->forkStreams(2));
#define H10X_MOSH_LAUNCH(W, LL, FK, TH, STREAM)                                                                                    \
    { if (lds > 48 * 1024) H10X_HIP(c, hipFuncSetAttribute((const void *)mosh_lds_kernel<W, LL, FK>, hipFuncAttributeMaxDynamicSharedMemorySize, (int)lds)); \
      mosh_lds_kernel<W, LL, FK><<<n, TH, lds, STREAM>>>(dRec, list, n, startRec.p, slots.p, capOff.p, mc, (u32)tableBytes, stHash.p, stRead.p, nHash.p); }
#define H10X_MOSH_CLASS(TH, STREAM)                                                                                                \
    { if (fastK && w31) H10X_MOSH_LAUNCH(true, 8, true, TH, STREAM) else if (fastK) H10X_MOSH_LAUNCH(false, 8, true, TH, STREAM)   \
      else if (w31 && mc.run == 8) H10X_MOSH_LAUNCH(true, 8, false, TH, STREAM) else if (w31) H10X_MOSH_LAUNCH(true, 9, false, TH, STREAM) \
      else if (mc.run == 8) H10X_MOSH_LAUNCH(false, 8, false, TH, STREAM) else H10X_MOSH_LAUNCH(false, 9, false, TH, STREAM) }
  const bool fastK = k >= 17 && k <= 30 && mc.run == 8;
  for (int cls = 2; cls >= 0; --cls) {
    const u32 n = hc[cls]; if (!n) continue;
    const u32 *list = cls == 0 ? list0.p : cls == 1 ? list1.p : list2.p;
    const size_t tableBytes = (size_t)hmin<u32>(4096u << cls, maxSlots) * 8;
    const size_t lds = tableBytes + (size_t)((cls == 2 ? 1024 : 512) / WAVE) * MOSH_QCAP * 8;
    if (cls == 2) H10X_MOSH_CLASS(1024, c->aux[0]) else if (cls == 1) H10X_MOSH_CLASS(512, c->aux[1]) else H10X_MOSH_CLASS(512, st)
    H10X_HIP(c, hipGetLastError());
  }
#undef H10X_MOSH_CLASS
#undef H10X_MOSH_LAUNCH
  H10X_TRY(c->faultAt(1));
  H10X_TRY(c->joinStreams(2));
  forkGuard.done();
  c->tstop(T_MOSH);

  DevBuf<u32> nOverflow; H10X_HIP(c, nOverflow.alloc(1)); H10X_HIP(c, hipMemsetAsync(nOverflow.p, 0, 4, st));
  count_overflow_kernel<<<divUp(nBlocks, 256), 256, 0, st>>>(nHash.p, nBlocks, nOverflow.p);
  H10X_HIP(c, c->blockOff.alloc((size_t)nBlocks + 1));
  H10X_TRY(prim_exclusive_scan_u32_u64(c, pt, nHash.p, c->blockOff.p, (size_t)nBlocks + 1));
  u64 H = 0, lastStart = 0; u32 hOverflow = 0, hMaxHash = 0xFFFFFFFFu;
  DevBuf<u32> dMaxHash; H10X_HIP(c, dMaxHash.alloc(1));
  H10X_TRY(prim_reduce_max_u32(c, pt, nHash.p, dMaxHash.p, nBlocks));
  H10X_TRY(c->readback(&hMaxHash, dMaxHash.p, 4));
  H10X_TRY(c->readback(&H, c->blockOff.p + nBlocks, 8));
  H10X_TRY(c->readback(&lastStart, startRec.p + (nBlocks - 1), 8));
  H10X_TRY(c->readback(&hOverflow, nOverflow.p, 4));
  H10X_TRY(c->syncReadbacks());
  const bool anyFallback = hc[3] || hOverflow;
  std::vector<u32> hNHash, hListF(hc[3]);
  std::vector<u64> hStart;
  if (anyFallback) {
    hNHash.resize(nBlocks + 1); hStart.resize(nBlocks + 1);
    H10X_HIP(c, hipMemcpyAsync(hNHash.data(), nHash.p, (size_t)nBlocks * 4, hipMemcpyDeviceToHost, st));
    H10X_HIP(c, hipMemcpyAsync(hStart.data(), startRec.p, ((size_t)nBlocks + 1) * 8, hipMemcpyDeviceToHost, st));
    if (hc[3]) H10X_HIP(c, hipMemcpyAsync(hListF.data(), listF.p, (size_t)hc[3] * 4, hipMemcpyDeviceToHost, st));
    H10X_HIP(c, hipStreamSynchronize(st));
    for (u32 b = 1; b + (hashLast ? 0 : 1) < nBlocks; ++b) if (hNHash[b] == NHASH_OVERFLOW) hListF.push_back(b);
  }
  std::vector<SrcPtr> hFb;
  std::vector<DevBuf<u64> *> keepH; std::vector<DevBuf<u32> *> keepR;
  c->ctr.fallback_blocks = hListF.size();
  if (!hListF.empty()) {
    hFb.assign(nBlocks, SrcPtr{nullptr, nullptr});
    c->tstart(T_FALLBACK);
    const u32 nk = (u32)(mc.n1 + mc.n2);
    for (u32 b : hListF) {
      const u32 nr = (u32)(hStart[b + 1] - hStart[b]);
      const u64 nSlot = (u64)nr * nk;
      DevBuf<u64> *oh = new DevBuf<u64>(); DevBuf<u32> *orr = new DevBuf<u32>(); keepH.push_back(oh); keepR.push_back(orr);
      u32 nUniq = 0;
      if (nSlot >= (1ULL << 32)) return c->fail("barcode block %u too large for the global mosh path (%llu k-mer slots)", b, (u64)nSlot);
      if (nSlot) {
        DevBuf<u64> k0, k1; DevBuf<u32> v0, v1, fl, ps;
        H10X_HIP(c, k0.alloc(nSlot)); H10X_HIP(c, k1.alloc(nSlot)); H10X_HIP(c, v0.alloc(nSlot)); H10X_HIP(c, v1.alloc(nSlot));
        H10X_HIP(c, fl.alloc(nSlot + 1)); H10X_HIP(c, ps.alloc(nSlot + 1));
        const unsigned g = (unsigned)hmin<u64>(divUp(nr, REC_TILE), 4096);
        if (w31) mosh_raw_kernel<true><<<g, MOSH_THREADS, 0, st>>>(dRec, hStart[b], nr, mc, k0.p, v0.p);
        else     mosh_raw_kernel<false><<<g, MOSH_THREADS, 0, st>>>(dRec, hStart[b], nr, mc, k0.p, v0.p);
        H10X_TRY(prim_sort_pairs_u64_u32(c, pt, k0.p, k1.p, v0.p, v1.p, nSlot, 0, 64));
        const unsigned g2 = (unsigned)hmin<u64>(divUp(nSlot, 256), 65535);
        unique_flags_kernel<<<g2, 256, 0, st>>>(k1.p, nSlot, fl.p);
        H10X_HIP(c, hipMemsetAsync(fl.p + nSlot, 0, 4, st));
        H10X_TRY(prim_exclusive_scan_u32(c, pt, fl.p, ps.p, nSlot + 1));
        H10X_HIP(c, hipMemcpyAsync(&nUniq, ps.p + nSlot, 4, hipMemcpyDeviceToHost, st));
        H10X_HIP(c, hipStreamSynchronize(st));
        H10X_HIP(c, oh->alloc(nUniq ? nUniq : 1)); H10X_HIP(c, orr->alloc(nUniq ? nUniq : 1));
        if (nUniq) unique_scatter_kernel<<<g2, 256, 0, st>>>(k1.p, v1.p, fl.p, ps.p, nSlot, nk, oh->p, orr->p);
        H10X_HIP(c, hipStreamSynchronize(st));
      } else { H10X_HIP(c, oh->alloc(1)); H10X_HIP(c, orr->alloc(1)); }
      if (!nUniq) {
        H10X_HIP(c, hipMemsetAsync(oh->p, 0, 8, st)); H10X_HIP(c, hipMemsetAsync(orr->p, 0, 4, st)); nUniq = 1;
      }
      hNHash[b] = nUniq; hFb[b] = SrcPtr{oh->p, orr->p};
    }
    H10X_HIP(c, hipMemcpyAsync(nHash.p, hNHash.data(), (size_t)nBlocks * 4, hipMemcpyHostToDevice, st));
    c->tstop(T_FALLBACK);
  }

  c->tstart(T_COMPACT);
  DevBuf<SrcPtr> dFb; H10X_HIP(c, dFb.alloc(nBlocks));
  if (hFb.empty()) H10X_HIP(c, hipMemsetAsync(dFb.p, 0, (size_t)nBlocks * sizeof(SrcPtr), st));
  else {
    H10X_HIP(c, hipMemcpyAsync(dFb.p, hFb.data(), (size_t)nBlocks * sizeof(SrcPtr), hipMemcpyHostToDevice, st));
    H10X_TRY(prim_exclusive_scan_u32_u64(c, pt, nHash.p, c->blockOff.p, (size_t)nBlocks + 1));
    H10X_HIP(c, hipMemcpyAsync(&H, c->blockOff.p + nBlocks, 8, hipMemcpyDeviceToHost, st));
    H10X_HIP(c, hipStreamSynchronize(st));
  }
  if (H >= (1ULL << 32)) return c->fail("%llu (barcode,hash) entries exceed this build's 2^32 per-GPU limit", (u64)H);
  c->nEntries = H;
  if (!hNHash.empty()) { hMaxHash = 0; for (u32 b = 0; b < nBlocks; ++b) hMaxHash = hNHash[b] > hMaxHash ? hNHash[b] : hMaxHash; }
  c->maxBlockHashes = hMaxHash;
  set_nhash_kernel<<<divUp(nBlocks, 256), 256, 0, st>>>(c->blocks.p, nHash.p, nBlocks);
  H10X_HIP(c, entHash.alloc(H)); H10X_HIP(c, entRead.alloc(H));
  {
    u64 m = (u64)c->prm.w; int s = 0; while (!(m & 1)) { m >>= 1; ++s; }
    u64 inv = m; for (int it = 0; it < 6; ++it) inv *= 2 - m * inv;
    const int k2 = 2 * c->prm.k; const u64 maxH = k2 >= 64 ? ~0ULL : ((u64)1 << k2) - 1, maxQ = maxH / (u64)c->prm.w;
    int b = 1; while (b < 64 && (maxQ >> b)) ++b;
    c->keyInv = inv; c->keyShift = s; c->keyBits = b;
    int cb = 1; while (cb < 32 && ((nBlocks - 1) >> cb)) ++cb;
    c->entCodeBits = (c->wantPacked && b + cb <= 63) ? cb : 0;
  }
  if (!c->entCodeBits) H10X_HIP(c, entCode.alloc(H));
  if (H) compact_entries_kernel<<<hmin<u32>(nBlocks, 8192), 256, 0, st>>>(stHash.p, stRead.p, capOff.p, dFb.p, nHash.p, c->blockOff.p, nBlocks,
                                                                        c->keyInv, c->keyShift, c->entCodeBits, entHash.p, entCode.p, entRead.p);
  H10X_HIP(c, hipGetLastError());
  if (!hFb.empty()) H10X_HIP(c, hipStreamSynchronize(st));
  c->tstop(T_COMPACT);
  for (auto *p : keepH) delete p;
  for (auto *p : keepR) delete p;

  u64 hashedPairs = hashLast ? nRec : (nBlocks >= 2 ? lastStart : 0);
  c->ctr.pairs = nRec; c->ctr.kmers = hashedPairs * (u64)(mc.n1 + mc.n2); c->ctr.entries = H;
  return 0;
}

__global__ void warm_stageA_kernel() {}
void warm_stageA(hipStream_t st) { warm_stageA_kernel<<<1, 1, 0, st>>>(); }

}
```

### hash10x_amd/csrc/stage_b.hip

```cpp
#include "common.hpp"
#include "prim.hpp"
#include <rocprim/block/block_radix_sort.hpp>

namespace h10x {

constexpr u32 SLOT_EMPTY = 0xFFFFFFFFu;
static int bitsFor(u64 maxValue) { int b = 1; while (b < 64 && (maxValue >> b)) ++b; return b; }

__global__ void seg_scatter_kernel(const u64 *__restrict__ sHash, const u32 *__restrict__ sCode,
                                   const u32 *__restrict__ ord, u64 n, u64 *__restrict__ dHash, u32 *__restrict__ dFirst,
                                   u32 *__restrict__ segStart, u32 *__restrict__ iota) {
  u64 i = (u64)blockIdx.x * blockDim.x + threadIdx.x;
  const u64 stride = (u64)gridDim.x * blockDim.x;
  for (; i < n; i += stride) if (ord[i + 1] != ord[i]) {
    const u32 d = ord[i];
    dHash[d] = sHash[i]; dFirst[d] = sCode[i]; segStart[d] = (u32)i; iota[d] = d;
  }
}
__global__ void seg_scatter_packed_kernel(const u64 *__restrict__ sKey, int cb,
                                          const u32 *__restrict__ ord, u64 n, Val16 *__restrict__ dVal, u32 *__restrict__ dFirst, u32 *__restrict__ rows) {
  u64 i = (u64)blockIdx.x * blockDim.x + threadIdx.x;
  const u64 stride = (u64)gridDim.x * blockDim.x;
  const u64 cmask = ((u64)1 << cb) - 1;
  for (; i < n; i += stride) {
    const u64 k = sKey[i]; const u32 code = (u32)(k & cmask);
    rows[i] = code;
    const u32 d = ord[i], d1 = ord[i + 1];
    if (d1 != d) { dVal[d].a = k >> cb; dVal[d].b = (u32)i; dFirst[d] = code; }
    if (i + 1 == n || ord[i + 2] != d1) dVal[d1 - 1].c = (u32)i + 1;
  }
}
__global__ void assign_index_v16_kernel(const Val16 *__restrict__ val, u32 U, u64 w , u64 *__restrict__ hashValue, u32 *__restrict__ hashDepth,
                                        u64 *__restrict__ rowStart) {
  const u32 i = blockIdx.x * blockDim.x + threadIdx.x;
  if (i == 0) { hashValue[0] = 0; hashDepth[0] = 0; rowStart[0] = 0; }
  if (i >= U) return;
  const Val16 v = val[i];
  hashValue[i + 1] = v.a * w; hashDepth[i + 1] = v.c - v.b; rowStart[i + 1] = v.b;
}

__global__ void assign_index_kernel(const u32 *__restrict__ order, const u64 *__restrict__ dHash, const u32 *__restrict__ segStart,
                                    u32 U, u64 w , u64 *__restrict__ hashValue, u32 *__restrict__ hashDepth, u64 *__restrict__ rowStart) {
  const u32 i = blockIdx.x * blockDim.x + threadIdx.x;
  if (i == 0) { hashValue[0] = 0; hashDepth[0] = 0; rowStart[0] = 0; }
  if (i >= U) return;
  const u32 d = order[i];
  hashValue[i + 1] = dHash[d] * w;
  hashDepth[i + 1] = segStart[d + 1] - segStart[d];
  rowStart[i + 1] = segStart[d];
}

__global__ void probe_insert_kernel(const u64 *__restrict__ hashValue, u32 hashNumber, int B, u32 *__restrict__ table) {
  const u32 first = blockIdx.x * blockDim.x + threadIdx.x + 1;
  const u64 mask = ((u64)1 << B) - 1;
  for (u32 start = first; start < hashNumber; start += gridDim.x * blockDim.x) {
    u32 cur = start;
    u64 h = hashValue[cur];
    u64 slot = h & mask, step = ((h >> B) & mask) | 1;
    for (;;) {
      const u32 old = atomicMin(&table[slot], cur);
      if (old == SLOT_EMPTY) break;
      if (old > cur) {
        cur = old; h = hashValue[cur]; step = ((h >> B) & mask) | 1;
      }
      slot = (slot + step) & mask;
    }
  }
}
__global__ void probe_finish_kernel(u32 *__restrict__ table, u64 n) {
  u64 i = (u64)blockIdx.x * blockDim.x + threadIdx.x;
  const u64 stride = (u64)gridDim.x * blockDim.x;
  for (; i < n; i += stride) if (table[i] == SLOT_EMPTY) table[i] = 0;
}

constexpr u64 SLOT_EMPTY64 = ~0ULL;
__global__ void probe_insert64_kernel(const u64 *__restrict__ hashValue, u32 hashNumber, int B, u64 w, int qBits, u64 *__restrict__ table) {
  const u32 first = blockIdx.x * blockDim.x + threadIdx.x + 1;
  const u64 mask = ((u64)1 << B) - 1, qmask = ((u64)1 << qBits) - 1;
  for (u32 start = first; start < hashNumber; start += gridDim.x * blockDim.x) {
    u64 h = hashValue[start];
    u64 cur = ((u64)start << qBits) | (h / w);
    u64 slot = h & mask, step = ((h >> B) & mask) | 1;
    for (;;) {
      const u64 old = atomicMin((unsigned long long *)&table[slot], (unsigned long long)cur);
      if (old == SLOT_EMPTY64) break;
      if (old > cur) {
        cur = old; h = (old & qmask) * w; step = ((h >> B) & mask) | 1;
      }
      slot = (slot + step) & mask;
    }
  }
}
__global__ void probe_insertP_kernel(const u64 *__restrict__ hashValue, u32 hashNumber, int B, int SH, int PB, u64 *__restrict__ table, u32 *__restrict__ fail) {
  const u32 first = blockIdx.x * blockDim.x + threadIdx.x + 1;
  const u64 mask = ((u64)1 << B) - 1, pmask = ((u64)1 << PB) - 1, umask = ((u64)1 << (SH - PB)) - 1;
  for (u32 start = first; start < hashNumber; start += gridDim.x * blockDim.x) {
    const u64 h = hashValue[start];
    u64 cur = ((u64)start << SH) | ((h >> B) << PB);
    u64 slot = h & mask, step = ((h >> B) & mask) | 1;
    for (;;) {
      const u64 old = atomicMin((unsigned long long *)&table[slot], (unsigned long long)cur);
      if (old == SLOT_EMPTY64) break;
      if (old > cur) { cur = old; step = (((cur >> PB) & umask) & mask) | 1; }
      if ((cur & pmask) == pmask) { *fail = 1; break; }
      ++cur;
      slot = (slot + step) & mask;
    }
  }
}
__global__ void probe_finish64_kernel(const u64 *__restrict__ table64, u64 n, int qBits, u32 *__restrict__ table) {
  u64 i = (u64)blockIdx.x * blockDim.x + threadIdx.x;
  const u64 stride = (u64)gridDim.x * blockDim.x;
  for (; i < n; i += stride) { const u64 e = table64[i]; table[i] = e == SLOT_EMPTY64 ? 0u : (u32)(e >> qBits); }
}
__global__ void lookup_pack64_kernel(const u64 *__restrict__ entHash , const u32 *__restrict__ entRead, u64 n,
                                     const u64 *__restrict__ table64, int B, u64 w, int qBits, int cb, u64 *__restrict__ key) {
  u64 i = (u64)blockIdx.x * blockDim.x + threadIdx.x;
  const u64 stride = (u64)gridDim.x * blockDim.x;
  const u64 mask = ((u64)1 << B) - 1, qmask = ((u64)1 << qBits) - 1;
  for (; i < n; i += stride) {
    const u64 q = entHash[i] >> cb, h = q * w;
    u64 slot = h & mask; const u64 step = ((h >> B) & mask) | 1;
    u64 e;
    while ((e = table64[slot]) != SLOT_EMPTY64 && (e & qmask) != q) slot = (slot + step) & mask;
    const u32 ix = e == SLOT_EMPTY64 ? 0u : (u32)(e >> qBits);
    key[i] = ((u64)ix << 32) | (u64)(entRead[i] & 0xFFFFu);
  }
}

constexpr u32 PRIV_MAX_DISP = 256;
__global__ void priv_insert_kernel(const u64 *__restrict__ hashValue, u32 hashNumber, u64 w, int T, u64 *__restrict__ table) {
  const u32 first = blockIdx.x * blockDim.x + threadIdx.x + 1;
  const u64 mask = ((u64)1 << T) - 1;
  for (u32 i = first; i < hashNumber; i += gridDim.x * blockDim.x) {
    const u64 q = hashValue[i] / w, low = ((q >> T) << 8);
    u64 slot = q & mask;
    for (u32 d = 0; d < PRIV_MAX_DISP; ++d, slot = (slot + 1) & mask)
      if (atomicCAS((unsigned long long *)&table[slot], (unsigned long long)SLOT_EMPTY64, (unsigned long long)(((u64)i << 32) | low | d)) == SLOT_EMPTY64) break;
  }
}
__device__ __forceinline__ u32 priv_find(const u64 *__restrict__ table, int T, u64 q, const u32 *__restrict__ hashIndex, const u64 *__restrict__ hashValue, int B, u64 w, u64 e0) {
  const u64 mask = ((u64)1 << T) - 1;
  const u32 want = (u32)((q >> T) << 8);
  u64 slot = q & mask;
  for (u32 d = 0; d < PRIV_MAX_DISP; ++d, slot = (slot + 1) & mask) {
    const u64 e = d ? table[slot] : e0;
    if ((u32)e == (want | d)) return (u32)(e >> 32);
    if (e == SLOT_EMPTY64) break;
  }
  return probe_find(hashIndex, hashValue, B, q * w);
}

__global__ void lookup_pack_kernel(const u64 *__restrict__ entHash, const u32 *__restrict__ entRead, u64 n,
                                   const u32 *__restrict__ table, const u64 *__restrict__ hashValue, int B, u64 w , int cb, u64 *__restrict__ key) {
  u64 i = (u64)blockIdx.x * blockDim.x + threadIdx.x;
  const u64 stride = (u64)gridDim.x * blockDim.x;
  for (; i < n; i += stride) {
    const u32 ix = probe_find(table, hashValue, B, (entHash[i] >> cb) * w);
    key[i] = ((u64)ix << 32) | (u64)(entRead[i] & 0xFFFFu);
  }
}
__global__ void offsets32_kernel(const u64 *__restrict__ off, u32 n, u32 *__restrict__ out) {
  const u32 i = blockIdx.x * blockDim.x + threadIdx.x;
  if (i < n) out[i] = (u32)off[i];
}
__global__ void write_clushash_kernel(const u64 *__restrict__ key, u64 n, h10x_clushash *__restrict__ out) {
  u64 i = (u64)blockIdx.x * blockDim.x + threadIdx.x;
  const u64 stride = (u64)gridDim.x * blockDim.x;
  for (; i < n; i += stride) {
    const u64 v = key[i];
    h10x_clushash c; c.hash = (u32)(v >> 32); c.read = (u16)(v & 0xFFFF); c.subCluster = 0; c.flags = 0;
    out[i] = c;
  }
}


__global__ void block_class_kernel(const u64 *__restrict__ blockOff, u32 nBlocks, u32 *__restrict__ lists, u32 *__restrict__ counts) {
  const u32 c = blockIdx.x * blockDim.x + threadIdx.x;
  const int lane = threadIdx.x & (WAVE - 1);
  int cls = -1;
  if (c < nBlocks) { const u64 n = blockOff[c + 1] - blockOff[c]; cls = n <= BLOCK_SORT_CAP0 ? 0 : (n <= BLOCK_SORT_CAP1 ? 1 : (n <= BLOCK_SORT_MAX ? 2 : -1)); }
#pragma unroll
  for (int k = 0; k < 3; ++k) {
    const u64 bal = __ballot(cls == k);
    if (!bal) continue;
    u32 base = 0;
    if (lane == 0) base = atomicAdd(&counts[k], (u32)__popcll(bal));
    base = (u32)__shfl((int)base, 0);
    if (cls == k) lists[(size_t)k * nBlocks + base + (u32)__popcll(bal & ((1ULL << lane) - 1))] = c;
  }
}
int stageB_blockClassLists(Ctx *c, DevBuf<u32> &lists, DevBuf<u32> &counts) {
  H10X_HIP(c, lists.alloc((size_t)3 * c->nBlocks)); H10X_HIP(c, counts.alloc(4));
  H10X_HIP(c, hipMemsetAsync(counts.p, 0, 16, c->stream));
  if (c->nBlocks) block_class_kernel<<<divUp(c->nBlocks, 256), 256, 0, c->stream>>>(c->blockOff.p, c->nBlocks, lists.p, counts.p);
  return 0;
}

template <int THREADS, int IPT> struct BlockIndexSort {
  static constexpr int CAP = THREADS * IPT;
  static constexpr int NB = 4096, LOGNB = 12;
  static constexpr int CPT = NB / THREADS;
  static constexpr int WAVES = THREADS / WAVE;
  struct Storage { u32 cnt[NB + 4]; u32 key[CAP]; u16 val[CAP]; u32 bm[CAP / 32]; u32 waveTot[WAVES]; u32 kmax, firstZero, runCount; };
  __device__ __forceinline__ static void sort(u32 (&k)[IPT], u32 (&v)[IPT], u32 n, Storage &s) {
    const u32 tid = threadIdx.x, lane = tid & (WAVE - 1), wave = tid / WAVE;
#pragma unroll
    for (int i = 0; i < CPT; ++i) s.cnt[(u32)i * THREADS + tid] = 0;
    if (tid < 4) s.cnt[NB + tid] = 0;
    if (tid < CAP / 32) s.bm[tid] = 0;
    if (tid == 0) { s.kmax = 0; s.firstZero = CAP; s.runCount = 0; }
    u32 m = 0;
#pragma unroll
    for (int j = 0; j < IPT; ++j) if ((u32)j * THREADS + tid < n) m = k[j] > m ? k[j] : m;
#pragma unroll
    for (int d = 32; d; d >>= 1) { const u32 o2 = (u32)__shfl_xor((int)m, d); m = o2 > m ? o2 : m; }
    __syncthreads();
    if (lane == 0) atomicMax(&s.kmax, m);
    __syncthreads();
    const u32 kmax = s.kmax;
#pragma unroll
    for (int j = 0; j < IPT; ++j) if ((u32)j * THREADS + tid < n) { const u32 d = kmax - k[j]; if (d < (u32)CAP) atomicOr(&s.bm[d >> 5], 1u << (d & 31)); }
    __syncthreads();
    if (tid < CAP / 32) { const u32 w = ~s.bm[tid]; if (w) atomicMin(&s.firstZero, tid * 32 + (u32)__ffs((int)w) - 1u); }
    __syncthreads();
    u32 run = s.firstZero;
    {
      u32 mineInRun = 0;
#pragma unroll
      for (int j = 0; j < IPT; ++j) if ((u32)j * THREADS + tid < n && kmax - k[j] < run) ++mineInRun;
#pragma unroll
      for (int d = 32; d; d >>= 1) mineInRun += (u32)__shfl_xor((int)mineInRun, d);
      if (lane == 0 && mineInRun) atomicAdd(&s.runCount, mineInRun);
      __syncthreads();
      if (s.runCount != run) run = 0;
    }
    const u32 lim = run ? (kmax >= run ? kmax - run : 0) : kmax + 1u;
    const int sh = lim > (u32)NB ? (32 - __clz((int)(lim - 1))) - LOGNB : 0;
    u32 r[IPT];
#pragma unroll
    for (int j = 0; j < IPT; ++j) { r[j] = 0; if ((u32)j * THREADS + tid < n && kmax - k[j] >= run) r[j] = atomicAdd(&s.cnt[k[j] >> sh], 1u); }
    __syncthreads();
    {
      u32 c[CPT], t = 0;
#pragma unroll
      for (int i = 0; i < CPT; ++i) { c[i] = s.cnt[tid * CPT + (u32)i]; t += c[i]; }
      u32 inc = t;
#pragma unroll
      for (int d = 1; d < WAVE; d <<= 1) { const u32 o2 = (u32)__shfl_up((int)inc, d); if (lane >= (u32)d) inc += o2; }
      if (lane == WAVE - 1) s.waveTot[wave] = inc;
      __syncthreads();
      u32 base = inc - t;
      for (u32 q = 0; q < wave; ++q) base += s.waveTot[q];
#pragma unroll
      for (int i = 0; i < CPT; ++i) { s.cnt[tid * CPT + (u32)i] = base; base += c[i]; }
      if (tid == THREADS - 1) s.cnt[NB] = base;
      __syncthreads();
    }
#pragma unroll
    for (int j = 0; j < IPT; ++j) if ((u32)j * THREADS + tid < n && kmax - k[j] >= run) { r[j] += s.cnt[k[j] >> sh]; s.key[r[j]] = k[j]; }
    __syncthreads();
#pragma unroll
    for (int j = 0; j < IPT; ++j) if ((u32)j * THREADS + tid < n) {
      const u32 d = kmax - k[j];
      if (d < run) r[j] = n - 1u - d;
      else {
        const u32 b = k[j] >> sh, st = s.cnt[b], en = s.cnt[b + 1];
        u32 rank = 0;
        for (u32 q = st; q < en; ++q) { const u32 x = s.key[q]; rank += (x < k[j] || (x == k[j] && q < r[j])) ? 1u : 0u; }
        r[j] = st + rank;
      }
    }
    __syncthreads();
#pragma unroll
    for (int j = 0; j < IPT; ++j) if ((u32)j * THREADS + tid < n) { s.key[r[j]] = k[j]; s.val[r[j]] = (u16)v[j]; }
    __syncthreads();
#pragma unroll
    for (int j = 0; j < IPT; ++j) { const u32 e = (u32)j * THREADS + tid; if (e < n) { k[j] = s.key[e]; v[j] = s.val[e]; } }
  }
};

template <int THREADS, int IPT, bool LOOKUP>
__global__ __launch_bounds__(THREADS)
void clushash_block_kernel(const u64 *__restrict__ entHash , const u32 *__restrict__ entRead, const u64 *__restrict__ key ,
                           const u64 *__restrict__ blockOff, const u32 *__restrict__ list, const u32 *__restrict__ count ,
                           const u64 *__restrict__ table64, int B, u64 w, int qBits, int cb , int sortBits,
                           h10x_clushash *__restrict__ out, int privT = 0 ,
                           const u32 *__restrict__ hashIndex = nullptr, const u64 *__restrict__ hashValue = nullptr,
                           const u32 *__restrict__ replyIdx = nullptr, const u32 *__restrict__ replyPos = nullptr ,
                           int probeBits = 0 ) {
  using Sort = BlockIndexSort<THREADS, IPT>;
  __shared__ typename Sort::Storage storage;
  const u32 nList = *count;
  for (u32 wi = blockIdx.x; wi < nList; wi += gridDim.x) {
    const u32 c = list[wi];
    const u64 o = blockOff[c]; const u64 n64 = blockOff[c + 1] - o;
    if (n64 == 0) continue;
    const u32 n = (u32)n64;
    u32 k[IPT], v[IPT];
    const u64 mask = ((u64)1 << B) - 1, qmask = qBits >= 64 ? ~0ULL : ((u64)1 << qBits) - 1;
    if (LOOKUP) {
      u64 q[IPT];
#pragma unroll
      for (int j = 0; j < IPT; ++j) { const u32 e = (u32)j * THREADS + threadIdx.x; q[j] = entHash[o + (e < n ? e : n - 1)] >> cb; }
#pragma unroll
      for (int j = 0; j < IPT; ++j) { const u32 e = (u32)j * THREADS + threadIdx.x; v[j] = entRead[o + (e < n ? e : n - 1)] & 0xFFFFu; }
      constexpr int LKG = IPT;
#pragma unroll
      for (int j0 = 0; j0 < IPT; j0 += LKG) {
        u64 t[LKG];
#pragma unroll
        for (int g = 0; g < LKG; ++g) { const int j = j0 + g < IPT ? j0 + g : IPT - 1; t[g] = table64[privT ? (q[j] & (((u64)1 << privT) - 1)) : ((q[j] * w) & mask)]; }
#pragma unroll
        for (int g = 0; g < LKG; ++g) {
          const int j = j0 + g;
          if (j < IPT) {
            const u32 e = (u32)j * THREADS + threadIdx.x;
            u32 kk;
            if (privT) kk = priv_find(table64, privT, q[j], hashIndex, hashValue, B, w, t[g]);
            else {
              const u64 h = q[j] * w; u64 slot = h & mask; const u64 step = ((h >> B) & mask) | 1;
              u64 tt = t[g];
              if (probeBits) { u64 want = (h >> B) << probeBits; while (tt != SLOT_EMPTY64 && (tt & qmask) != want) { slot = (slot + step) & mask; ++want; tt = table64[slot]; } }
              else while (tt != SLOT_EMPTY64 && (tt & qmask) != q[j]) { slot = (slot + step) & mask; tt = table64[slot]; }
              kk = tt == SLOT_EMPTY64 ? 0u : (u32)(tt >> qBits);
            }
            k[j] = e < n ? kk : 0xFFFFFFFFu;
          }
        }
      }
    } else if (replyPos) {
      u32 pp[IPT];
#pragma unroll
      for (int j = 0; j < IPT; ++j) { const u32 e = (u32)j * THREADS + threadIdx.x; pp[j] = replyPos[o + (e < n ? e : n - 1)]; }
#pragma unroll
      for (int j = 0; j < IPT; ++j) { const u32 e = (u32)j * THREADS + threadIdx.x; v[j] = entRead[o + (e < n ? e : n - 1)] & 0xFFFFu; }
#pragma unroll
      for (int j = 0; j < IPT; ++j) { const u32 e = (u32)j * THREADS + threadIdx.x; const u32 kk = replyIdx[pp[j]]; k[j] = e < n ? kk : 0xFFFFFFFFu; }
    } else {
#pragma unroll
      for (int j = 0; j < IPT; ++j) {
        const u32 e = (u32)j * THREADS + threadIdx.x;
        k[j] = 0xFFFFFFFFu; v[j] = 0;
        if (e < n) { const u64 t = key[o + e]; k[j] = (u32)(t >> 32); v[j] = (u32)t & 0xFFFFu; }
      }
    }
    __syncthreads();
    Sort::sort(k, v, n, storage);
#pragma unroll
    for (int j = 0; j < IPT; ++j) {
      const u32 e = (u32)j * THREADS + threadIdx.x;
      if (e < n) { h10x_clushash r; r.hash = k[j]; r.read = (u16)v[j]; r.subCluster = 0; r.flags = 0; out[o + e] = r; }
    }
  }
}

static int clusHashByBlocks(Ctx *c, const u64 *entHash, const u32 *entRead, const u64 *key, const u64 *table64, int privT = 0, const u32 *replyIdx = nullptr, const u32 *replyPos = nullptr,
                            int probeSH = 0, int probeBits = 0 ) {
  hipStream_t st = c->stream; const u32 nBlocks = c->nBlocks;
  H10X_HIP(c, c->clusHash.alloc(c->nEntries));
  if (!c->nEntries || nBlocks < 2) return 0;
  int sortBits = bitsFor(c->hashNumber) + 1 > 32 ? 32 : bitsFor(c->hashNumber) + 1;
  const int B = c->prm.B; const u64 w = (u64)c->prm.w; const int qBits = probeBits ? probeSH : c->keyBits;
  DevBuf<u32> lists, counts;
  H10X_TRY(stageB_blockClassLists(c, lists, counts));
  const unsigned gridBig = hmin<u32>(nBlocks, (u32)c->numCU * 8), gridSmall = hmin<u32>(nBlocks, 65535u * 4);
#define H10X_CH_LAUNCH(T, I, LOOK, CLS, STREAM) clushash_block_kernel<T, I, LOOK><<<(CLS == 0 ? gridSmall : gridBig), T, 0, STREAM>>>(entHash, entRead, key, c->blockOff.p, \
    lists.p + (size_t)CLS * nBlocks, counts.p + CLS, table64, B, w, qBits, (key || replyPos) ? 0 : c->entCodeBits, sortBits, c->clusHash.p, privT, c->hashIndex.p, c->hashValue.p, replyIdx, replyPos, probeBits)
  const int side = c->maxBlockHashes > BLOCK_SORT_CAP1 ? 2 : (c->maxBlockHashes > BLOCK_SORT_CAP0 ? 1 : 0);
  ForkGuard forkGuard(c);
  if (side) H10X_TRY(c->forkStreams(side));
  if (key || replyPos) { H10X_CH_LAUNCH(H10X_BS_T0, H10X_BS_I0, false, 0, st); if (side >= 1) H10X_CH_LAUNCH(H10X_BS_T1, H10X_BS_I1, false, 1, c->aux[0]); if (side >= 2) H10X_CH_LAUNCH(1024, 8, false, 2, c->aux[1]); }
  else { H10X_CH_LAUNCH(H10X_BS_T0, H10X_BS_I0, true, 0, st); if (side >= 1) H10X_CH_LAUNCH(H10X_BS_T1, H10X_BS_I1, true, 1, c->aux[0]); if (side >= 2) H10X_CH_LAUNCH(1024, 8, true, 2, c->aux[1]); }
#undef H10X_CH_LAUNCH
  H10X_TRY(c->faultAt(2));
  if (side) H10X_TRY(c->joinStreams(side));
  forkGuard.done();
  H10X_HIP(c, hipGetLastError());
  return 0;
}

int stageB_run(Ctx *c, DevBuf<u64> &entHash, DevBuf<u32> &entCode, DevBuf<u32> &entRead) {
  hipStream_t st = c->stream; PrimTemp pt;
  const u64 H = c->nEntries; const int B = c->prm.B; const u32 nBlocks = c->nBlocks;
  const unsigned gH = (unsigned)hmin<u64>(divUp(H ? H : 1, 256), 65535u * 2);
  const u64 tableSize = (u64)1 << B;

  c->tstart(T_SORT_HASH);
  DevBuf<u64> sHash; DevBuf<u32> sCode;
  const int cb = c->entCodeBits;
  H10X_HIP(c, sHash.alloc(H)); H10X_HIP(c, sCode.alloc(H + ROWS_PAD));
  if (cb) H10X_TRY(prim_sort_keys_u64(c, pt, entHash.p, sHash.p, H, cb, cb + c->keyBits));
  else H10X_TRY(prim_sort_pairs_u64_u32(c, pt, entHash.p, sHash.p, entCode.p, sCode.p, H, 0, c->keyBits));
  c->tstop(T_SORT_HASH);

  c->tstart(T_RANK);
  u32 U = 0;
  DevBuf<u64> dHash; DevBuf<u32> dFirst, segStart, iota, order, dFirstSorted; DevBuf<Val16> dVal, dValSorted;
  {
    DevBuf<u32> ord;
    H10X_HIP(c, ord.alloc(H + 2));
    H10X_TRY(prim_run_ordinals_u64(c, pt, sHash.p, cb, ord.p, H));
    H10X_TRY(c->readback(&U, ord.p + H, 4));
    H10X_TRY(c->syncReadbacks());
    if ((u64)U + 1 > (tableSize >> 2) - 2) return c->fail("hashTableSize is too small");
    H10X_HIP(c, dFirst.alloc(U)); H10X_HIP(c, dFirstSorted.alloc(U));
    if (cb) { H10X_HIP(c, dVal.alloc(U)); H10X_HIP(c, dValSorted.alloc(U)); }
    else { H10X_HIP(c, dHash.alloc(U)); H10X_HIP(c, segStart.alloc((size_t)U + 1)); H10X_HIP(c, iota.alloc(U)); H10X_HIP(c, order.alloc(U)); }
    if (H && cb) seg_scatter_packed_kernel<<<gH, 256, 0, st>>>(sHash.p, cb, ord.p, H, dVal.p, dFirst.p, sCode.p);
    else if (H) {
      seg_scatter_kernel<<<gH, 256, 0, st>>>(sHash.p, sCode.p, ord.p, H, dHash.p, dFirst.p, segStart.p, iota.p);
      H10X_HIP(c, hipMemsetD32Async((hipDeviceptr_t)(segStart.p + U), (int)(u32)H, 1, st));
    }
  }
  c->hashNumber = U + 1; c->depthBound = nBlocks;
  H10X_HIP(c, c->hashValue.alloc((size_t)U + 1)); H10X_HIP(c, c->hashDepth.alloc((size_t)U + 1));
  H10X_HIP(c, c->rowStart.alloc((size_t)U + 2));
  if (cb) {
    H10X_TRY(prim_sort_pairs_u32_v16(c, pt, dFirst.p, dFirstSorted.p, dVal.p, dValSorted.p, U, 0, bitsFor(nBlocks)));
    assign_index_v16_kernel<<<divUp((u64)U + 1, 256), 256, 0, st>>>(dValSorted.p, U, (u64)c->prm.w, c->hashValue.p, c->hashDepth.p, c->rowStart.p);
  } else {
    H10X_TRY(prim_sort_pairs_u32_u32(c, pt, dFirst.p, dFirstSorted.p, iota.p, order.p, U, 0, bitsFor(nBlocks)));
    assign_index_kernel<<<divUp((u64)U + 1, 256), 256, 0, st>>>(order.p, dHash.p, segStart.p, U, (u64)c->prm.w, c->hashValue.p, c->hashDepth.p, c->rowStart.p);
  }
  c->rows.swap(sCode);
  c->tstop(T_RANK);
  sHash.release(); dHash.release(); dFirst.release(); iota.release(); dFirstSorted.release(); dVal.release(); dValSorted.release();

  const bool forcePriv = (c->optPrivTable == 1 || c->optPrivTable == 3) && c->keyBits <= 40;
  const bool wideTable = !forcePriv && c->keyBits + (B - 2) <= 64 && c->keyBits < 64;
  DevBuf<u64> table64;
  const int hashBits = 2 * c->prm.k, UB = hashBits > B ? hashBits - B : 0, PBroom = 64 - (B - 2) - UB;
  int PB = 0, SH = 0; bool probed = false;
  if (!forcePriv && c->optProbedTable != 2 && (!wideTable || c->optProbedTable == 1 || c->optProbedTable == 3) && PBroom >= 12 && c->keyBits < 64) {
    PB = PBroom > 24 ? 24 : PBroom; if (c->optProbedTable == 3) PB = 1;
    SH = UB + PB;
    c->tstart(T_PROBE);
    DevBuf<u32> failFlag; u32 failed = 0;
    H10X_HIP(c, table64.alloc(tableSize)); H10X_HIP(c, c->hashIndex.alloc(tableSize)); H10X_HIP(c, failFlag.alloc(1));
    H10X_HIP(c, hipMemsetAsync(table64.p, 0xFF, tableSize * 8, st)); H10X_HIP(c, hipMemsetAsync(failFlag.p, 0, 4, st));
    if (U) probe_insertP_kernel<<<hmin<u32>(divUp(U, 256), 16384), 256, 0, st>>>(c->hashValue.p, U + 1, B, SH, PB, table64.p, failFlag.p);
    H10X_TRY(c->readback(&failed, failFlag.p, 4));
    H10X_TRY(c->syncReadbacks());
    probed = !failed;
    if (probed) probe_finish64_kernel<<<(unsigned)hmin<u64>(divUp(tableSize, 256), 65535u * 2), 256, 0, st>>>(table64.p, tableSize, SH, c->hashIndex.p);
    else { table64.release(); c->hashIndex.release(); }
    c->tstop(T_PROBE);
    c->ctr.index_table_form = probed ? 2 : 3;
  }
  if (probed) {}
  else if (wideTable) {
    if (c->ctr.index_table_form != 3) c->ctr.index_table_form = 1;
    c->tstart(T_PROBE);
    H10X_HIP(c, table64.alloc(tableSize)); H10X_HIP(c, c->hashIndex.alloc(tableSize));
    H10X_HIP(c, hipMemsetAsync(table64.p, 0xFF, tableSize * 8, st));
    if (U) probe_insert64_kernel<<<hmin<u32>(divUp(U, 256), 16384), 256, 0, st>>>(c->hashValue.p, U + 1, B, (u64)c->prm.w, c->keyBits, table64.p);
    probe_finish64_kernel<<<(unsigned)hmin<u64>(divUp(tableSize, 256), 65535u * 2), 256, 0, st>>>(table64.p, tableSize, c->keyBits, c->hashIndex.p);
    c->tstop(T_PROBE);
  } else { if (c->ctr.index_table_form != 3) c->ctr.index_table_form = 0; H10X_TRY(stageB_buildProbeTable(c)); }

  c->tstart(T_CLUSHASH);
  if (H && probed && c->maxBlockHashes <= BLOCK_SORT_MAX) {
    H10X_TRY(clusHashByBlocks(c, entHash.p, entRead.p, nullptr, table64.p, 0, nullptr, nullptr, SH, PB));
    table64.release();
  } else if (H && !probed && wideTable && c->maxBlockHashes <= BLOCK_SORT_MAX) {
    H10X_TRY(clusHashByBlocks(c, entHash.p, entRead.p, nullptr, table64.p));
    table64.release();
  } else if (H && !probed && !wideTable && c->maxBlockHashes <= BLOCK_SORT_MAX && c->keyBits <= 40 && c->optPrivTable != 2) {
    int T = 16; while (((u64)1 << T) < 2 * ((u64)U + 1) && T < 32) ++T;
    if (c->optPrivTable == 3) { T = 4; while (((u64)1 << T) < ((u64)U + 1) / 2 && T < 32) ++T; }
    if (T < c->keyBits - 24) T = c->keyBits - 24;
    DevBuf<u64> priv;
    H10X_HIP(c, priv.alloc((size_t)1 << T));
    H10X_HIP(c, hipMemsetAsync(priv.p, 0xFF, ((size_t)1 << T) * 8, st));
    if (U) priv_insert_kernel<<<hmin<u32>(divUp(U, 256), 16384), 256, 0, st>>>(c->hashValue.p, U + 1, (u64)c->prm.w, T, priv.p);
    H10X_TRY(clusHashByBlocks(c, entHash.p, entRead.p, nullptr, priv.p, T));
  } else if (H) {
    DevBuf<u64> key; H10X_HIP(c, key.alloc(H));
    if (wideTable && !probed) lookup_pack64_kernel<<<gH, 256, 0, st>>>(entHash.p, entRead.p, H, table64.p, B, (u64)c->prm.w, c->keyBits, cb, key.p);
    else lookup_pack_kernel<<<gH, 256, 0, st>>>(entHash.p, entRead.p, H, c->hashIndex.p, c->hashValue.p, B, (u64)c->prm.w, cb, key.p);
    table64.release();
    H10X_TRY(stageB_finishClusHash(c, key));
  } else H10X_HIP(c, c->clusHash.alloc(0));
  c->tstop(T_CLUSHASH);
  c->ctr.distinct = U;
  c->haveState = true;
  return 0;
}

int stageB_buildProbeTable(Ctx *c) {
  hipStream_t st = c->stream; const int B = c->prm.B; const u64 tableSize = (u64)1 << B; const u32 U = c->hashNumber - 1;
  c->tstart(T_PROBE);
  H10X_HIP(c, c->hashIndex.alloc(tableSize));
  H10X_HIP(c, hipMemsetAsync(c->hashIndex.p, 0xFF, tableSize * 4, st));
  if (U) probe_insert_kernel<<<hmin<u32>(divUp(U, 256), 16384), 256, 0, st>>>(c->hashValue.p, U + 1, B, c->hashIndex.p);
  probe_finish_kernel<<<(unsigned)hmin<u64>(divUp(tableSize, 256), 65535u * 2), 256, 0, st>>>(c->hashIndex.p, tableSize);
  c->tstop(T_PROBE);
  return 0;
}

__global__ void reply_key_kernel(const u32 *__restrict__ replyIdx, const u32 *__restrict__ replyPos, const u32 *__restrict__ entRead, u64 n, u64 *__restrict__ key) {
  u64 e = (u64)blockIdx.x * blockDim.x + threadIdx.x; const u64 stride = (u64)gridDim.x * blockDim.x;
  for (; e < n; e += stride) key[e] = ((u64)replyIdx[replyPos[e]] << 32) | (u64)(entRead[e] & 0xFFFFu);
}
int stageB_finishClusHashFromReplies(Ctx *c, const u32 *replyIdx, const u32 *replyPos, const u32 *entRead) {
  if (c->maxBlockHashes <= BLOCK_SORT_MAX) return clusHashByBlocks(c, nullptr, entRead, nullptr, nullptr, 0, replyIdx, replyPos);
  const u64 H = c->nEntries;
  DevBuf<u64> key; H10X_HIP(c, key.alloc(H));
  if (H) reply_key_kernel<<<(unsigned)hmin<u64>(divUp(H, 256), 65535u * 2), 256, 0, c->stream>>>(replyIdx, replyPos, entRead, H, key.p);
  return stageB_finishClusHash(c, key);
}

int stageB_finishClusHash(Ctx *c, DevBuf<u64> &key) {
  hipStream_t st = c->stream; PrimTemp pt; const u64 H = c->nEntries; const u32 nBlocks = c->nBlocks;
  const unsigned gH = (unsigned)hmin<u64>(divUp(H ? H : 1, 256), 65535u * 2);
  if (c->maxBlockHashes <= BLOCK_SORT_MAX) return clusHashByBlocks(c, nullptr, nullptr, key.p, nullptr);
  H10X_HIP(c, c->clusHash.alloc(H));
  if (!H) return 0;
  DevBuf<u64> keyS; DevBuf<u32> off32;
  H10X_HIP(c, keyS.alloc(H)); H10X_HIP(c, off32.alloc((size_t)nBlocks + 1));
  offsets32_kernel<<<divUp((u64)nBlocks + 1, 256), 256, 0, st>>>(c->blockOff.p, nBlocks + 1, off32.p);
  H10X_TRY(prim_seg_sort_keys_u64(c, pt, key.p, keyS.p, (u32)H, nBlocks, off32.p, off32.p + 1, 32, 32 + bitsFor(c->hashNumber)));
  write_clushash_kernel<<<gH, 256, 0, st>>>(keyS.p, H, c->clusHash.p);
  H10X_HIP(c, hipGetLastError());
  H10X_HIP(c, hipStreamSynchronize(st));
  return 0;
}

__global__ void entry_code_kernel(const h10x_clushash *__restrict__ ch, const u64 *__restrict__ blockOff, u32 nBlocks,
                                  u32 *__restrict__ keyIdx, u32 *__restrict__ valCode) {
  for (u32 c = blockIdx.x + 1; c < nBlocks; c += gridDim.x) {
    const u64 o = blockOff[c], n = blockOff[c + 1] - o;
    for (u64 i = threadIdx.x; i < n; i += blockDim.x) { keyIdx[o + i] = ch[o + i].hash; valCode[o + i] = c; }
  }
}

int stageB_buildCSR(Ctx *c) {
  hipStream_t st = c->stream; PrimTemp pt;
  const u64 H = c->nEntries; const u32 U1 = c->hashNumber;
  c->tstart(T_CSR);
  H10X_HIP(c, c->rowStart.alloc((size_t)U1 + 1));
  H10X_TRY(prim_exclusive_scan_u32_u64(c, pt, c->hashDepth.p, c->rowStart.p, U1));
  u64 lastOff = 0; u32 lastDepth = 0;
  if (U1) {
    H10X_HIP(c, hipMemcpyAsync(&lastOff, c->rowStart.p + (U1 - 1), 8, hipMemcpyDeviceToHost, st));
    H10X_HIP(c, hipMemcpyAsync(&lastDepth, c->hashDepth.p + (U1 - 1), 4, hipMemcpyDeviceToHost, st));
    H10X_HIP(c, hipStreamSynchronize(st));
  }
  if (lastOff + lastDepth != H)
    return c->fail("inconsistent hash state: sum of hashDepth %llu != %llu (barcode,hash) entries", (u64)(lastOff + lastDepth), (u64)H);
  H10X_HIP(c, c->rows.alloc(H + ROWS_PAD));
  if (H) {
    DevBuf<u32> k0, k1, v0;
    H10X_HIP(c, k0.alloc(H)); H10X_HIP(c, k1.alloc(H)); H10X_HIP(c, v0.alloc(H));
    entry_code_kernel<<<hmin<u32>(c->nBlocks, 8192), 256, 0, st>>>(c->clusHash.p, c->blockOff.p, c->nBlocks, k0.p, v0.p);
    H10X_TRY(prim_sort_pairs_u32_u32(c, pt, k0.p, k1.p, v0.p, c->rows.p, H, 0, bitsFor(U1)));
    H10X_HIP(c, hipStreamSynchronize(st));
  }
  c->tstop(T_CSR);
  return 0;
}

// ... 5 lines not shown
```

### hash10x_amd/csrc/stage_c.hip

```cpp
#include "common.hpp"
#include <chrono>
#include "prim.hpp"
#include <type_traits>
#include <rocprim/block/block_radix_sort.hpp>

namespace h10x {


constexpr int CL_THREADS_SMALL = 1024;
constexpr int CL_THREADS_HUGE = 1024;
constexpr u16 NONE16 = 0xFFFF;
constexpr u32 NOHANDLE = 0xFFFFFFFFu;
constexpr int ROWS_IN_FLIGHT = 4;
constexpr int RCHUNK = 4;

__global__ void within_kernel(const u32 *__restrict__ depth, u32 hashNumber, int lo, int hi, u8 *__restrict__ within) {
  const u32 i = blockIdx.x * blockDim.x + threadIdx.x;
  if (i >= hashNumber) return;
  const int n = (int)depth[i];
  if (n >= lo && n < hi) within[i] = 1;
}
__global__ void within_depth_kernel(const u32 *__restrict__ depth, const u8 *__restrict__ within, u32 hashNumber, u32 *__restrict__ out,
                                    const u64 *__restrict__ rowStart, u32 rowShift, u64 *__restrict__ rowInfo ) {
  const u32 i = blockIdx.x * blockDim.x + threadIdx.x;
  if (i < hashNumber) {
    const u32 wd = within[i] ? depth[i] + 1 : 0;
    out[i] = wd; if (rowInfo) rowInfo[i] = (u64)(u32)(rowStart[i] >> rowShift) | ((u64)wd << 32);
  }
}

template <typename KT>
__global__ __launch_bounds__(256)
void good_keys_kernel(const h10x_clushash *__restrict__ ch, const u64 *__restrict__ blockOff, const h10x_block *__restrict__ blocks,
                      u32 nBlocks, const u32 *__restrict__ wdepth ,
                      KT *__restrict__ key, u32 *__restrict__ nGood, u32 *__restrict__ segEnd, u32 *__restrict__ entries ) {
  __shared__ u32 sCount; __shared__ unsigned long long sDepth;
  for (u32 c = blockIdx.x; c < nBlocks; c += gridDim.x) {
    const u64 o = blockOff[c]; const u32 nHash = blocks[c].nHash;
    __syncthreads();
    if (threadIdx.x == 0) { sCount = 0; sDepth = 0; }
    __syncthreads();
    unsigned long long myDepth = 0;
    if (nHash <= 65535) {
      for (u32 base = 0; base < nHash; base += blockDim.x) {
        const u32 p = base + threadIdx.x;
        u32 wd = 0; bool good = false;
        if (p < nHash) { wd = wdepth[ch[o + p].hash]; good = wd != 0; if (good) myDepth += wd - 1; }
        const u64 bal = __ballot(good);
        const int lane = threadIdx.x & (WAVE - 1);
        u32 wb = 0;
        if (lane == 0 && bal) wb = atomicAdd(&sCount, (u32)__popcll(bal));
        wb = __shfl(wb, 0);
        if (good) key[o + wb + (u32)__popcll(bal & ((1ULL << lane) - 1))] = (KT)(((KT)(wd - 1) << 16) | (KT)p);
      }
    }
    for (int sft = 32; sft; sft >>= 1) myDepth += __shfl_down(myDepth, sft);
    if ((threadIdx.x & (WAVE - 1)) == 0 && myDepth) atomicAdd(&sDepth, myDepth);
    __syncthreads();
    if (threadIdx.x == 0) { nGood[c] = sCount; segEnd[c] = (u32)o + sCount; entries[c] = sDepth > 0xFFFFFFFFull ? 0xFFFFFFFFu : (u32)sDepth; }
  }
}
template <typename KT>
__global__ void good_pos_kernel(const KT *__restrict__ key, u64 n, u16 *__restrict__ pos) {
  u64 i = (u64)blockIdx.x * blockDim.x + threadIdx.x;
  const u64 stride = (u64)gridDim.x * blockDim.x;
  for (; i < n; i += stride) pos[i] = (u16)(key[i] & 0xFFFF);
}
__global__ void offsets32c_kernel(const u64 *__restrict__ off, u32 n, u32 *__restrict__ out) {
  const u32 i = blockIdx.x * blockDim.x + threadIdx.x;
  if (i < n) out[i] = (u32)off[i];
}

template <int THREADS, int IPT>
__global__ __launch_bounds__(THREADS)
void good_block_kernel(const h10x_clushash *__restrict__ ch, const u64 *__restrict__ blockOff, const h10x_block *__restrict__ blocks,
                       const u32 *__restrict__ list, const u32 *__restrict__ count ,
                       const u64 *__restrict__ rowInfo , int sortBits,
                       u16 *__restrict__ goodPos, u32 *__restrict__ nGood, u32 *__restrict__ entries ,
                       u64 *__restrict__ goodRow ) {
  using Sort = rocprim::block_radix_sort<u32, THREADS, IPT, u64>;
  __shared__ typename Sort::storage_type storage;
  __shared__ u32 sCount; __shared__ unsigned long long sDepth;
  const u32 nList = *count;
  for (u32 wi = blockIdx.x; wi < nList; wi += gridDim.x) {
    const u32 c = list[wi];
    const u32 nHash = blocks[c].nHash;
    const u64 o = blockOff[c];
    __syncthreads();
    if (threadIdx.x == 0) { sCount = 0; sDepth = 0; }
    __syncthreads();
    u32 k[IPT]; u64 v[IPT]; u32 mine = 0; unsigned long long myDepth = 0;
#pragma unroll
    for (int j = 0; j < IPT; ++j) { k[j] = 0xFFFFFFFFu; v[j] = threadIdx.x * IPT + (u32)j; }
    if (nHash) {
      u32 hs[IPT]; u64 ri[IPT];
#pragma unroll
      for (int j = 0; j < IPT; ++j) { const u32 p = threadIdx.x * IPT + (u32)j; hs[j] = ch[o + (p < nHash ? p : nHash - 1)].hash; }
#pragma unroll
      for (int j = 0; j < IPT; ++j) ri[j] = rowInfo[hs[j]];
#pragma unroll
      for (int j = 0; j < IPT; ++j) {
        const u32 p = threadIdx.x * IPT + (u32)j; const u32 wd = (u32)(ri[j] >> 32);
        if (p < nHash && wd) { k[j] = wd - 1; ++mine; myDepth += wd - 1; v[j] = (u64)p | ((ri[j] & 0xFFFFFFFFull) << 16); }
      }
    }
    for (int sft = 32; sft; sft >>= 1) { mine += (u32)__shfl_down((int)mine, sft); myDepth += __shfl_down(myDepth, sft); }
    if ((threadIdx.x & (WAVE - 1)) == 0 && mine) { atomicAdd(&sCount, mine); atomicAdd(&sDepth, myDepth); }
    Sort().sort_to_striped(k, v, storage, 0, sortBits);
    __syncthreads();
    const u32 nG = sCount;
#pragma unroll
    for (int j = 0; j < IPT; ++j) {
      const u32 e = (u32)j * THREADS + threadIdx.x;
      if (e < nG) {
        goodPos[o + e] = (u16)v[j];
        goodRow[o + e] = (u64)(u32)(v[j] >> 16) | ((u64)k[j] << 32);
      }
    }
    if (threadIdx.x == 0) { nGood[c] = nG; entries[c] = sDepth > 0xFFFFFFFFull ? 0xFFFFFFFFu : (u32)sDepth; }
  }
}

__global__ void good_rows_kernel(const h10x_clushash *__restrict__ ch, const u64 *__restrict__ blockOff, const u32 *__restrict__ nGood, const u16 *__restrict__ goodPos, u32 nBlocks,
                                 const u32 *__restrict__ hashDepth, const u64 *__restrict__ rowStart, u32 rowShift, u64 *__restrict__ goodRow);
static int bitsForC(u64 maxValue) { int b = 1; while (b < 64 && (maxValue >> b)) ++b; return b; }

int stageC_depthRange(Ctx *c, int lo, int hi) {
  hipStream_t st = c->stream; PrimTemp pt;
  if (!c->haveState) return c->fail("no hash state loaded: use readFQB or readHash first");
  c->haveGood = false;
  c->tstart(T_GOOD);
  const u32 U1 = c->hashNumber; const u32 nBlocks = c->nBlocks; const u64 H = c->nEntries;
  if (!(c->haveRange && lo == c->rangeMin && hi == c->rangeMax)) {
    if (!c->haveRange) { H10X_HIP(c, c->within.alloc(U1)); H10X_HIP(c, hipMemsetAsync(c->within.p, 0, U1, st)); }
    within_kernel<<<divUp(U1, 256), 256, 0, st>>>(c->hashDepth.p, U1, lo, hi, c->within.p);
    c->haveRange = true; c->rangeMin = lo; c->rangeMax = hi;
    if (hi > 0 && (u32)hi > c->rangeHiMax) c->rangeHiMax = (u32)hi;
  }
  XGuard xGuard(c);
  if (c->sharded) { c->tstop(T_GOOD); H10X_TRY(shard_exchangeRows(c)); c->tstart(T_GOOD); }
  DevBuf<u64> key, keyS; DevBuf<u32> key32, keyS32, off32, segEnd, wdepth, red;
  H10X_HIP(c, off32.alloc((size_t)nBlocks + 1));
  H10X_HIP(c, segEnd.alloc(nBlocks)); H10X_HIP(c, wdepth.alloc(U1)); H10X_HIP(c, red.alloc(2));
  H10X_HIP(c, c->nGood.alloc(nBlocks)); H10X_HIP(c, c->goodPos.alloc(H)); H10X_HIP(c, c->goodEntries.alloc(nBlocks)); H10X_HIP(c, c->goodRow.alloc(H));
  const u32 goodDepthBound = hmin<u32>(c->depthBound, c->rangeHiMax ? c->rangeHiMax - 1 : 0);
  const bool narrow = goodDepthBound <= 65535u;
  const bool byBlocks = narrow && c->maxBlockHashes <= BLOCK_SORT_MAX;
  DevBuf<u64> rowInfo; if (byBlocks) H10X_HIP(c, rowInfo.alloc(U1));
  within_depth_kernel<<<divUp(U1, 256), 256, 0, st>>>(c->hashDepth.p, c->within.p, U1, wdepth.p, c->rowStart.p, (u32)c->rowShift, rowInfo.p);
  H10X_TRY(prim_reduce_max_u32(c, pt, wdepth.p, red.p, U1));
  if (byBlocks) {
    int db = 1; while (db < 16 && (goodDepthBound >> db)) ++db;
    const int sortBits = db + 1;
    DevBuf<u32> lists, counts;
    H10X_TRY(stageB_blockClassLists(c, lists, counts));
    const unsigned gridBig = hmin<u32>(nBlocks, (u32)c->numCU * 8), gridSmall = hmin<u32>(nBlocks, 65535u * 4);
    const int side = c->maxBlockHashes > BLOCK_SORT_CAP1 ? 2 : (c->maxBlockHashes > BLOCK_SORT_CAP0 ? 1 : 0);
    ForkGuard forkGuard(c);
    if (side) H10X_TRY(c->forkStreams(side));
#define H10X_GOOD_LAUNCH(T, I, CLS, STREAM)                                                                                         \
    { const u32 *const L = lists.p + (size_t)CLS * nBlocks, *const N = counts.p + CLS; const unsigned grid = CLS == 0 ? gridSmall : gridBig; \
      good_block_kernel<T, I><<<grid, T, 0, STREAM>>>(c->clusHash.p, c->blockOff.p, c->blocks.p, L, N, rowInfo.p, sortBits, c->goodPos.p, c->nGood.p, c->goodEntries.p, c->goodRow.p); }
    H10X_GOOD_LAUNCH(H10X_BS_T0, H10X_BS_I0, 0, st)
    if (side >= 1) H10X_GOOD_LAUNCH(H10X_BS_T1, H10X_BS_I1, 1, c->aux[0])
    if (side >= 2) H10X_GOOD_LAUNCH(1024, 8, 2, c->aux[1])
#undef H10X_GOOD_LAUNCH
    H10X_TRY(c->faultAt(3));
    if (side) H10X_TRY(c->joinStreams(side));
    forkGuard.done();
  }
  else if (narrow) { H10X_HIP(c, key32.alloc(H)); H10X_HIP(c, keyS32.alloc(H)); } else { H10X_HIP(c, key.alloc(H)); H10X_HIP(c, keyS.alloc(H)); }
  if (byBlocks) {}
  else if (narrow) good_keys_kernel<u32><<<hmin<u32>(nBlocks, 16384), 256, 0, st>>>(c->clusHash.p, c->blockOff.p, c->blocks.p, nBlocks, wdepth.p,
                                                                             key32.p, c->nGood.p, segEnd.p, c->goodEntries.p);
  else good_keys_kernel<u64><<<hmin<u32>(nBlocks, 16384), 256, 0, st>>>(c->clusHash.p, c->blockOff.p, c->blocks.p, nBlocks, wdepth.p,
                                                                      key.p, c->nGood.p, segEnd.p, c->goodEntries.p);
  H10X_TRY(prim_reduce_max_u32(c, pt, c->nGood.p, red.p + 1, nBlocks));
  DevBuf<u64> redSum; H10X_HIP(c, redSum.alloc(1));
  H10X_TRY(prim_reduce_sum_u32_u64(c, pt, c->nGood.p, redSum.p, nBlocks));
  u32 hr[2]; u64 sumGood = 0;
  H10X_TRY(c->readback(hr, red.p, 8));
  H10X_TRY(c->readback(&sumGood, redSum.p, 8));
  H10X_TRY(c->syncReadbacks());
  hr[0] = hr[0] ? hr[0] - 1 : 0;
  c->maxGoodDepth = hr[0]; c->maxGood = hr[1]; c->meanGood = nBlocks > 1 ? (u32)(sumGood / (nBlocks - 1)) : 0;
  offsets32c_kernel<<<divUp((u64)nBlocks + 1, 256), 256, 0, st>>>(c->blockOff.p, nBlocks + 1, off32.p);
  if (H && !byBlocks) {
    if (narrow) {
      H10X_TRY(prim_seg_sort_keys_u32(c, pt, key32.p, keyS32.p, (u32)H, nBlocks, off32.p, segEnd.p, 0, 16 + bitsForC(hr[0])));
      good_pos_kernel<u32><<<(unsigned)hmin<u64>(divUp(H, 256), 65535u * 2), 256, 0, st>>>(keyS32.p, H, c->goodPos.p);
    } else {
      H10X_TRY(prim_seg_sort_keys_u64(c, pt, key.p, keyS.p, (u32)H, nBlocks, off32.p, segEnd.p, 0, 16 + bitsForC(hr[0])));
      good_pos_kernel<u64><<<(unsigned)hmin<u64>(divUp(H, 256), 65535u * 2), 256, 0, st>>>(keyS.p, H, c->goodPos.p);
    }
  }
  if (!byBlocks && nBlocks) good_rows_kernel<<<hmin<u32>(nBlocks, 65535u * 4), 256, 0, st>>>(c->clusHash.p, c->blockOff.p, c->nGood.p, c->goodPos.p, nBlocks, c->hashDepth.p, c->rowStart.p,
                                                                                           (u32)c->rowShift, c->goodRow.p);
  H10X_HIP(c, hipGetLastError());
  H10X_TRY(c->xJoin());
  c->haveGood = true;
  c->tstop(T_GOOD);
  return 0;
}

struct ClusterArgs {
  h10x_block *blocks; const u64 *blockOff; h10x_clushash *clusHash;
  const u16 *goodPos; const u32 *nGood;
  const u64 *goodRow;
  const u32 *rows;
  const u32 *list; u32 nList; u32 *workCounter;
  u32 *started;
  const u32 *front; u32 nFront;
  u32 nBlocks; int threshold;
  SegMap segs;
  u32 rowShift;
  u32 nBlocksFirst;
  u32 firstCap;
  u32 hashMinSlots;
  u32 hashBits;
  u16 *handles; size_t handleStride; u32 hStride;
  const u32 *entries;
  u32 *overflow, *overflowCount;
  unsigned char *scratch; size_t scratchStride;
  u32 maxGood;
  u32 ldsBudget;
  u64 *res;
  u64 *stats;
  u64 *phase;
  u32 narrowFirst;
  u32 tpClassT;
};

#define RES_PACK(best, q, tot) ((u64)(best) | ((u64)(q) << 16) | ((u64)(tot) << 40))
constexpr u32 RES_COUNT_MAX = (1u << 24) - 1;
struct Work {
  u16 *first;
  u32 *bm; u16 *pre;
  u16 *root;
  u32 *hist;
  u32 histWords;
};
__host__ __device__ inline size_t pad16(size_t b) { return (b + 15) & ~(size_t)15; }
__host__ __device__ inline size_t workBytes(u32 nFirst, u32 n, u32 nWaves, u32 bmWords) {
  size_t b = pad16((size_t)nFirst * 2) + pad16((size_t)bmWords * 4) + pad16((size_t)bmWords * 2);
  b += pad16((size_t)n * 2);
  b += (size_t)nWaves * (((size_t)n + 3) / 4) * 4;
  return b + 16;
}
constexpr u32 MIN_HIST_WAVES = 5;
constexpr u32 RANKED_FIRST_PER_RANK = 6;
__host__ __device__ inline u32 rankedFirstEstimate(u32 nBarcodes, u32 n) { const u64 e = (u64)RANKED_FIRST_PER_RANK * n; return e < nBarcodes ? (u32)e : nBarcodes; }
__host__ __device__ inline u32 rankedFirstEstimateE(u32 nBarcodes, u32 n, u32 entries, u32 div = 7) { const u32 a = rankedFirstEstimate(nBarcodes, n), b = entries / div; const u32 m = a > b ? a : b; return m < nBarcodes ? m : nBarcodes; }
__host__ __device__ inline u32 histWaves(u32 nFirst, u32 n, u32 maxWaves, u32 bmWords, size_t budget) {
  const size_t fixed = workBytes(nFirst, n, 0, bmWords), per = (((size_t)n + 3) / 4) * 4;
  if (fixed + MIN_HIST_WAVES * per > budget) return 0;
  const size_t wv = (budget - fixed) / (per ? per : 1);
  return wv < maxWaves ? (u32)wv : maxWaves;
}
__device__ inline Work carve(unsigned char *base, u32 nFirst, u32 n, u32 bmWords = 0) {
  Work w; size_t o = 0;
  w.first = (u16 *)(base + o); o += pad16((size_t)nFirst * 2);
  w.bm = (u32 *)(base + o); o += pad16((size_t)bmWords * 4);
  w.pre = (u16 *)(base + o); o += pad16((size_t)bmWords * 2);
  w.root = (u16 *)(base + o); o += pad16((size_t)n * 2);
  w.hist = (u32 *)(base + o); w.histWords = (n + 3) / 4;
  return w;
}
__host__ __device__ inline size_t mergeBytes(u32 nRep) {
  return (((size_t)nRep + 15) & ~(size_t)15) + 256 * 8 * 4 + 256 * 4 + 512 * 4 + 16;
}

template <bool IN_LDS, typename T> __device__ __forceinline__ T ld_shared(const T *p) {
  if (IN_LDS) return *p;
  return __hip_atomic_load(p, __ATOMIC_RELAXED, __HIP_MEMORY_SCOPE_AGENT);
}

template <bool IN_LDS>
__device__ __forceinline__ void min_u16(u16 *arr, u32 idx, u32 val) {
  u32 *w = (u32 *)arr + (idx >> 1); const int sh = (idx & 1) * 16;
  u32 old = ld_shared<IN_LDS>(w);
  for (;;) {
    if (((old >> sh) & 0xFFFFu) <= val) return;
    const u32 nw = (old & ~(0xFFFFu << sh)) | (val << sh);
    const u32 prev = atomicCAS(w, old, nw);
    if (prev == old) return;
    old = prev;
  }
}

template <bool FIRST_LDS> struct FirstDense {
  static constexpr bool MASK_TAIL = false;
  static constexpr bool SELF = true;
  u32 none;
  u16 *first; u32 wide;
  __device__ __forceinline__ u32 update(u32 cj, u32 i) const {
    if (FIRST_LDS && wide) atomicMin(&((u32 *)first)[cj], i); else min_u16<FIRST_LDS>(first, cj, i);
    return cj;
  }
  __device__ __forceinline__ u32 peek(u32 h) const {
    if (FIRST_LDS) return *(const u16 *)((const unsigned char *)first + (u32)(h << (1 + wide)));
    return ld_shared<FIRST_LDS>(&first[h]);
  }
  __device__ __forceinline__ u32 lookup(u32 cj) const { return peek(cj); }
  __device__ __forceinline__ u32 entry(const void *row, u32 j, u32 code) const { const u32 cj = ((const u32 *)row)[j]; return cj != code ? lookup(cj) : (u32)NONE16; }
};
struct FirstRanked {
  static constexpr bool SELF = false;
  static constexpr bool MASK_TAIL = false;
  u16 *first; const u32 *bm; const u16 *pre; u32 wide;
  u32 none;
  __device__ __forceinline__ u32 at(u32 cj) const { const u32 w = cj >> 5; return pre[w] + (u32)__popc(bm[w] & ((1u << (cj & 31)) - 1u)); }
  __device__ __forceinline__ u32 update(u32 cj, u32 i) const { const u32 h = at(cj); if (wide) atomicMin(&((u32 *)first)[h], i); else min_u16<true>(first, h, i); return h; }
  __device__ __forceinline__ u32 peek(u32 h) const { return *(const u16 *)((const unsigned char *)first + (u32)(h << (1 + wide))); }
  __device__ __forceinline__ u32 lookup(u32 cj) const { return peek(at(cj)); }
  __device__ __forceinline__ u32 entry(const void *row, u32 j, u32 code) const { const u32 cj = ((const u32 *)row)[j]; return cj != code ? lookup(cj) : (u32)NONE16; }
};
constexpr u32 TR_QUEUE = 16384;
constexpr u32 TR_MIN_SLOTS = 1024;
constexpr u32 TR_MAX_SLOTS = 65532;
struct SlotTable {
  u32 *tab; u32 NB , xsh , tsh; u32 *ovf; u32 hbase ;
  u32 base3;
  typedef __attribute__((address_space(3))) u32 lds_u32;
  typedef u32 u32x4 __attribute__((ext_vector_type(4)));
  typedef __attribute__((address_space(3))) u32x4 lds_u32x4;
  static constexpr u32 SCRAMBLE = 0x9E3779u;
  static constexpr u32 MAXD = 63;
  static constexpr u32 NOTFOUND = 0xFFFFFFFFu;
  __device__ __forceinline__ void shape(u32 *t, u32 slots, u32 hashBits, u32 *o, u32 hb) {
    tab = t; NB = slots / 4; xsh = 32 - hashBits; ovf = o; hbase = hb; base3 = 0;
    const u32 lg = 31 - (u32)__clz((int)NB), x = 32 - hashBits + lg; tsh = x < 31 ? x : 31;
  }
  __device__ __forceinline__ void inLds() { base3 = (u32)(size_t)(lds_u32 *)tab; }
  __device__ __forceinline__ u32 search(u32 cj, u32 i, bool insert, bool &ins) const {
    const u32 x = __umul24(cj, SCRAMBLE) << xsh;
    u32 b = __umulhi(x, NB);
    const u32 tag = (x * NB) >> tsh;
    const u32 step = 2 * (tag & 7u) + 1;
    ins = false;
    for (u32 key = tag; key < (MAXD << 10); key += 1u << 10) {
// ... 2031 lines not shown
```

### hash10x_amd/host/h10x_host.c

```c
#define _GNU_SOURCE
#include "h10x_host.h"
#include <stdio.h>
#include <stdlib.h>
#include <string.h>
#include <stdarg.h>
#include <limits.h>
#include <time.h>
#include <fcntl.h>
#include <pthread.h>
#include <unistd.h>
#include <sys/types.h>
#include <sys/stat.h>
#include <sys/mman.h>

#define ARRAY_MAGIC 8918274
typedef struct { int32_t magic, pad0; uint64_t base; int32_t dim, size, max, pad1; } array_hdr;

enum { N_KNOBS = 23 };
struct h10x_session {
  int k, w, r, B, N, chunk, ct, device;
  int timing;
  int knob[N_KNOBS];
  int16_t *cribChr; uint16_t *cribPos; uint8_t *cribType; uint32_t *cribDepth; uint32_t cribN;
  h10x_ctx *ctx;
  int ctxK, ctxW, ctxR, ctxB, ctxDev;
  int depthDim, depthMax, blocksDim, blocksMax;
  uint32_t *depthTail; int depthTailFrom;
  int sgBlocks;
  char err[1024];
};
static const char *const knobName[N_KNOBS] = {"cluster_stamps", "cluster_lds_budget", "cluster_first_global", "cluster_first_cap",
                                              "cluster_big_ranks", "cluster_threads0", "cluster_budget0", "shard_row_shift", "shard_rows_fake_base", "stage_a_max_slots", "cluster_narrow_first", "index_no_pack", "shard_delta_lists", "index_priv_table", "cluster_tr_packed", "cluster_tr_est_div", "cluster_tr_class_t", "shard_reply_sort", "shard_owner_cut", "shard_overlap", "index_probed_table", "fqb_slab", "molmap_global"};

static int fail(h10x_session *s, const char *fmt, ...) {
  va_list ap; va_start(ap, fmt); vsnprintf(s->err, sizeof s->err, fmt, ap); va_end(ap);
  return -1;
}
static int fail_ctx(h10x_session *s) { snprintf(s->err, sizeof s->err, "%s", h10x_last_error(s->ctx)); return -1; }

h10x_session *h10x_session_new(void) {
  if (h10x_abi_version() != H10X_ABI_VERSION) {
    fprintf(stderr, "h10x: libh10x_hip.so speaks ABI %d, this host layer was built for %d: rebuild both (make -C hash10x_amd/csrc && make -C hash10x_amd/host)\n", h10x_abi_version(), H10X_ABI_VERSION);
    return 0;
  }
  h10x_session *s = (h10x_session *)calloc(1, sizeof *s);
  if (!s) return 0;
  s->k = 21; s->w = 31; s->r = 17; s->B = 28; s->N = 0; s->chunk = 100000; s->ct = 5; s->device = 0;
  for (int i = 0; i < N_KNOBS; ++i)
    if (!strcmp(knobName[i], "shard_delta_lists") || !strcmp(knobName[i], "shard_row_shift") || !strcmp(knobName[i], "cluster_tr_packed") || !strcmp(knobName[i], "cluster_tr_class_t")) s->knob[i] = -1;
    else if (!strcmp(knobName[i], "shard_overlap")) s->knob[i] = 1;
  s->blocksDim = 1200;
  return s;
}
static void crib_free(h10x_session *s) { free(s->cribChr); free(s->cribPos); free(s->cribType); free(s->cribDepth); s->cribChr = 0; s->cribPos = 0; s->cribType = 0; s->cribDepth = 0; s->cribN = 0; }
void h10x_session_free(h10x_session *s) {
  if (!s) return;
  if (s->ctx) h10x_destroy(s->ctx);
  crib_free(s); free(s->depthTail); free(s);
}
const char *h10x_session_error(const h10x_session *s) { return s->err; }
h10x_ctx *h10x_session_ctx(h10x_session *s) { return s->ctx; }

static int *param_slot(h10x_session *s, const char *n) {
  static const char *const names[] = {"k", "w", "r", "B", "N", "c", "ct", "device", "timing", "share_graph_blocks", 0};
  int *const slots[] = {&s->k, &s->w, &s->r, &s->B, &s->N, &s->chunk, &s->ct, &s->device, &s->timing, &s->sgBlocks};
  for (int i = 0; names[i]; ++i) if (!strcmp(n, names[i])) return slots[i];
  for (int i = 0; i < N_KNOBS; ++i) if (!strcmp(n, knobName[i])) return &s->knob[i];
  return 0;
}
int h10x_session_set(h10x_session *s, const char *name, int value) {
  int *p = param_slot(s, name); if (!p) return fail(s, "unknown parameter %s", name);
  *p = value;
  if (s->ctx && p >= s->knob && p < s->knob + N_KNOBS && h10x_set_option(s->ctx, name, value)) return fail_ctx(s);
  return 0;
}
int h10x_session_get(const h10x_session *s, const char *name) {
  int *p = param_slot((h10x_session *)s, name); return p ? *p : 0;
}

int h10x_host_array_dim(int dim, int size, int64_t last) {
  while (last >= dim) dim = dim * size < (1 << 23) ? dim * 2 : dim + 1024 + (1 << 23) / size;
  return dim;
}

int64_t h10x_host_check_chunks(const uint32_t *rec, uint64_t total, int N, int chunk, char *err, int errlen) {
  const uint64_t limit = N > 0 && (uint64_t)N < total ? (uint64_t)N : total;
  uint64_t pos = 0, runLen = 0; uint32_t cur = 0;
  while (pos < limit) {
    if (runLen >= (uint64_t)chunk) { if (err) snprintf(err, (size_t)errlen, "chunkSize too small"); return -1; }
    uint64_t end = pos + ((uint64_t)chunk - runLen); if (end > limit) end = limit;
    if (!cur) cur = rec[30 * pos];
    for (; pos < end; ++pos) { const uint32_t b = rec[30 * pos]; if (b == cur) ++runLen; else { cur = b; runLen = 1; } }
  }
  if (!(N > 0 && (uint64_t)N <= total) && runLen >= (uint64_t)chunk) { if (err) snprintf(err, (size_t)errlen, "chunkSize too small"); return -1; }
  return (int64_t)limit;
}

int h10x_host_partition(const uint32_t *rec, uint64_t n, int nParts, uint64_t *cut) {
  if (nParts < 1 || !cut) return -1;
  cut[0] = 0; cut[nParts] = n;
  for (int g = 1; g < nParts; ++g) {
    uint64_t p = (uint64_t)(((__uint128_t)n * (unsigned)g) / (unsigned)nParts);
    if (p < cut[g - 1]) p = cut[g - 1];
    while (p > 0 && p < n && rec[30 * p] == rec[30 * (p - 1)]) ++p;
    cut[g] = p;
  }
  return 0;
}

int h10x_host_partition_file(const char *path, uint64_t n, int nParts, uint64_t *cut, char *err, int errlen) {
  if (nParts < 1 || !cut) return -1;
  const int fd = open(path, O_RDONLY);
  if (fd < 0) { if (err) snprintf(err, (size_t)errlen, "failed to open fqb file %s", path); return -1; }
  cut[0] = 0; cut[nParts] = n;
  for (int g = 1; g < nParts; ++g) {
    uint64_t p = (uint64_t)(((__uint128_t)n * (unsigned)g) / (unsigned)nParts);
    if (p < cut[g - 1]) p = cut[g - 1];
    uint32_t prev = 0, here = 0;
    if (p > 0 && p < n && pread(fd, &prev, 4, (off_t)((p - 1) * 120)) != 4) { close(fd); if (err) snprintf(err, (size_t)errlen, "file read problem"); return -1; }
    while (p > 0 && p < n) {
      if (pread(fd, &here, 4, (off_t)(p * 120)) != 4) { close(fd); if (err) snprintf(err, (size_t)errlen, "file read problem"); return -1; }
      if (here != prev) break;
      ++p;
    }
    cut[g] = p;
  }
  close(fd);
  return 0;
}

static double now_ms(void) { struct timespec t; clock_gettime(CLOCK_MONOTONIC, &t); return 1e3 * t.tv_sec + 1e-6 * t.tv_nsec; }
static int hostprof(void) { static int v = -1; if (v < 0) v = getenv("H10X_HOSTPROF") != 0; return v; }

static int apply_options(h10x_session *s) {
  h10x_timing_enable(s->ctx, s->timing);
  for (int i = 0; i < N_KNOBS; ++i) if (h10x_set_option(s->ctx, knobName[i], s->knob[i])) return fail_ctx(s);
  if (h10x_set_option(s->ctx, "chunk_size", 0)) return fail_ctx(s);
  return 0;
}

static int session_init(h10x_session *s) {
  double t0 = now_ms();
  const int reuse = s->ctx && s->ctxK == s->k && s->ctxW == s->w && s->ctxR == s->r && s->ctxB == s->B && s->ctxDev == s->device && s->k > 0 && s->w > 0;
  if (!reuse) {
    if (s->ctx) { h10x_destroy(s->ctx); s->ctx = 0; }
    double t1 = now_ms();
    h10x_params p; memset(&p, 0, sizeof p);
    p.k = s->k; p.w = s->w; p.B = s->B;
    if (s->k > 0 && s->w > 0) p.factor1 = h10x_factor1_from_seed(s->r);
    if (h10x_create(&s->ctx, &p, s->device, 0, s->err, (int)sizeof s->err)) return -1;
    s->ctxK = s->k; s->ctxW = s->w; s->ctxR = s->r; s->ctxB = s->B; s->ctxDev = s->device;
    if (hostprof()) fprintf(stderr, "hostprof: destroy %.3f ms, create %.3f ms\n", t1 - t0, now_ms() - t1);
  } else h10x_timing_reset(s->ctx);
  s->depthDim = 1 << 20; s->depthMax = 0;
  free(s->depthTail); s->depthTail = 0;
  crib_free(s);
  return apply_options(s);
}

static int after_readFQB(h10x_session *s) {
  h10x_shard_info_t z; if (h10x_shard_info(s->ctx, &z)) return fail_ctx(s);
  if (z.hashNumber > 1) { s->depthDim = h10x_host_array_dim(1 << 20, 4, (int64_t)z.hashNumber - 1); s->depthMax = (int)z.hashNumber; }
  else { s->depthDim = 1 << 20; s->depthMax = 0; }
  s->blocksDim = h10x_host_array_dim(s->blocksDim > 0 ? s->blocksDim : 1200, 32, (int64_t)z.nBlocksGlobal - 1);
  s->blocksMax = (int)z.nBlocksGlobal;
  return 0;
}

int h10x_session_begin(h10x_session *s) { return session_init(s) ? -1 : 0; }
int h10x_session_after_read(h10x_session *s) { return after_readFQB(s); }

int h10x_session_readFQB_mem(h10x_session *s, const uint32_t *rec, uint64_t n) {
  if (session_init(s)) return -1;
  const int cutByN = s->N > 0 && (uint64_t)s->N <= n;
  if (s->N > 0 && (uint64_t)s->N < n) n = (uint64_t)s->N;
  if (h10x_set_option(s->ctx, "chunk_size", s->chunk) || h10x_set_option(s->ctx, "chunk_eof_pass", !cutByN)) return fail_ctx(s);
  if (h10x_read_fqb(s->ctx, rec, n)) return fail_ctx(s);
  return after_readFQB(s);
}

int h10x_session_readFQB_dev(h10x_session *s, const uint32_t *devRec, uint64_t n) {
  if (session_init(s)) return -1;
  if (s->N > 0 && (uint64_t)s->N < n) n = (uint64_t)s->N;
  if (h10x_read_fqb_device(s->ctx, devRec, n)) return fail_ctx(s);
  return after_readFQB(s);
// ... 1477 lines not shown
```

### include/h10x.h

```cpp
#ifndef H10X_H
#define H10X_H
#include <stdint.h>

#ifdef __cplusplus
extern "C" {
#endif

#define H10X_ABI_VERSION 3

typedef struct h10x_ctx h10x_ctx;

typedef struct {
  int32_t  k;
  int32_t  w;
  int32_t  B;
  int32_t  reserved;
  uint64_t factor1;
} h10x_params;

typedef struct {
  uint32_t nRead, nHash, nSubCluster, clusterParent;
  uint64_t clusHash;
  double   pointToMin;
} h10x_block;
// ... 138 lines not shown

int  h10x_neighbours(h10x_ctx *ctx, uint32_t x, uint32_t *hash, uint32_t *count, uint32_t *firstCode, uint64_t cap, uint64_t *n);
int  h10x_neighbour_max(h10x_ctx *ctx, const uint32_t *xs, uint32_t nq, uint64_t *maxKey, uint32_t *nNeighbours);
int  h10x_neighbour_hist(h10x_ctx *ctx, const uint32_t *xs, uint32_t nq, const uint64_t *offsets, uint32_t *hist);
int  h10x_neighbour_stats(h10x_ctx *ctx, uint64_t out[4], int reset);

typedef struct {
  uint32_t nHash, nGood;
  uint32_t clustered;
  uint32_t raw;
  uint32_t merged;
  uint32_t abandoned;
  uint32_t histMax;
  uint32_t nShare;
} h10x_code_explore_rep;
int  h10x_code_share(h10x_ctx *ctx, const uint32_t *codes, uint32_t nq, uint64_t *offsets, uint32_t *barcode, uint32_t *count,
                     uint32_t *firstRank, uint32_t *firstHash, uint64_t cap);
int  h10x_code_explore(h10x_ctx *ctx, int32_t code, int32_t threshold, h10x_code_explore_rep *rep);
int  h10x_code_crib_counts(h10x_ctx *ctx, const uint32_t *codes, uint32_t n, uint32_t *out);

typedef struct {
  uint64_t rows, listEntries, entriesRead;
  uint32_t maxCount, batches, windows;
  uint32_t codeMin, codeMax, nBlocks;
} h10x_share_graph_info;
int  h10x_share_graph_run(h10x_ctx *ctx, int64_t minShare, uint32_t codeMin, uint32_t codeMax, h10x_share_graph_info *info);
int  h10x_share_graph_get(h10x_ctx *ctx, uint64_t *offsets, uint32_t *block, uint32_t *count, uint64_t cap);
int  h10x_share_graph_get_device(h10x_ctx *ctx, uint64_t *dev_offsets, uint32_t *dev_block, uint32_t *dev_count, uint64_t cap);

typedef struct h10x_mosh h10x_mosh;
typedef struct {
  int32_t  B, k, w, reserved;
  uint64_t factor1, factor2;
  uint32_t max;
  uint32_t size;
} h10x_mosh_info_t;
void h10x_factors_from_seed(int32_t seed, uint64_t *factor1, uint64_t *factor2);
int  h10x_mosh_create(h10x_mosh **set, int32_t B, int32_t k, int32_t w, int32_t seed, int device, char *err, int errlen);
int  h10x_mosh_load(h10x_mosh **set, int32_t B, int32_t k, int32_t w, uint64_t factor1, uint64_t factor2, const uint32_t *index,
                    const uint64_t *value, const uint16_t *depth, const uint8_t *info, uint32_t size, int device, char *err, int errlen);
void h10x_mosh_destroy(h10x_mosh *set);
const char *h10x_mosh_error(const h10x_mosh *set);
int  h10x_mosh_info(const h10x_mosh *set, h10x_mosh_info_t *out);
int  h10x_mosh_set_option(h10x_mosh *set, const char *name, int64_t value);
int  h10x_mosh_add(h10x_mosh *set, const uint8_t *codes, const uint64_t *seqStart, uint32_t nSeq, int skipOdd23, uint64_t seqBase,
                   uint64_t *nHashes);
int  h10x_mosh_scan(h10x_mosh *set, const uint8_t *codes, const uint64_t *seqStart, uint32_t nSeq, int skipOdd23, uint64_t seqBase,
                    uint64_t *hash, uint32_t *seq, uint32_t *pos, uint64_t cap, uint64_t *n);
int  h10x_mosh_merge(h10x_mosh *set, int32_t k2, int32_t w2, uint64_t factor1_2, const uint64_t *value2, const uint16_t *depth2,
                     const uint8_t *info2, uint32_t size2, int *merged);
int  h10x_mosh_prune(h10x_mosh *set, int32_t min, int32_t max, uint32_t *nBefore, uint32_t *nAfter);
int  h10x_mosh_set_copy(h10x_mosh *set, int32_t copy1min, int32_t copy2min, int32_t copyMmin);
int  h10x_mosh_set_copy_m(h10x_mosh *set, int32_t copyMmin);
int  h10x_mosh_summary(h10x_mosh *set, uint32_t *hist65536, uint32_t *copy4);
int  h10x_mosh_export(h10x_mosh *set, uint64_t indexFirst, uint64_t indexCount, uint32_t *index, uint64_t *value, uint16_t *depth,
                      uint8_t *info);
int  h10x_mosh_lookup(h10x_mosh *set, const uint64_t *hashes, uint64_t n, uint32_t *index, uint16_t *depth);

typedef struct h10x_readset h10x_readset;
typedef struct {
  int32_t  len, nHit;
  uint64_t hitPtr, dxPtr;
  uint8_t  bad, otherFlags;
  uint16_t pad1;
  int32_t  nMiss, contained;
  int32_t  nCopy[4];
  uint32_t pad2[4];
  uint32_t tail;
} h10x_read_t;
typedef struct {
  uint32_t iy; int32_t nHit, offset;
  uint8_t  isPlus, isBad, visited, pad;
  int32_t  nPlus, nMinus;
  double   d, sd;
  int64_t  sumZ, sumZ2;
} h10x_overlap_t;
typedef struct { uint32_t nReads , dim ; uint64_t totHit; } h10x_readset_info_t;
int  h10x_readset_create(h10x_readset **rs, h10x_mosh *set);
int  h10x_readset_add(h10x_readset *rs, const uint8_t *codes, const uint64_t *seqStart, uint32_t nSeq);
int  h10x_readset_load(h10x_readset **rs, h10x_mosh *set, const h10x_read_t *reads, uint32_t nReads, uint32_t dim, const uint32_t *hit,
                       const uint16_t *dx);
void h10x_readset_destroy(h10x_readset *rs);
const char *h10x_readset_error(const h10x_readset *rs);
int  h10x_readset_info(h10x_readset *rs, h10x_readset_info_t *out);
int  h10x_readset_export(h10x_readset *rs, const h10x_read_t **reads, const uint64_t **hitStart, const uint32_t **hit, const uint16_t **dx);
int  h10x_readset_overlap_cap(h10x_readset *rs, uint32_t ix, uint32_t *cap);
int  h10x_readset_overlaps(h10x_readset *rs, uint32_t ix, h10x_overlap_t *out, uint32_t cap, uint32_t *n, int32_t counts3[3]);
int  h10x_readset_mark_bad(h10x_readset *rs, int32_t found3[3]);
int  h10x_readset_mark_contained(h10x_readset *rs, int32_t *nContained, int32_t *nNotContained, uint64_t *totLenNotContained);
int  h10x_readset_stats_sums(h10x_readset *rs, uint64_t out16[16]);

typedef struct h10x_refmap h10x_refmap;
typedef struct { uint32_t size , max , setMax ; int32_t packed; } h10x_refmap_info_t;
typedef struct {
  uint32_t loc, loc2;
  uint32_t idClass, id2;
} h10x_mapseed_t;
typedef struct {
  uint32_t pos0, posN;
  uint32_t loc0, locN, n1, n2, query;
} h10x_maprec_t;
int  h10x_refmap_create(h10x_refmap **rm, h10x_mosh *set, uint32_t size);
int  h10x_refmap_add(h10x_refmap *rm, const uint8_t *codes, const uint64_t *seqStart, uint32_t nSeq, uint32_t idBase, uint64_t *nHits);
int  h10x_refmap_pack(h10x_refmap *rm, uint32_t *n1, uint32_t *n2, uint32_t *nM);
int  h10x_refmap_load(h10x_refmap **rm, h10x_mosh *set, const uint32_t *index, const uint32_t *offset, const uint32_t *id, const uint32_t *depth, const uint32_t *rev,
                      const uint32_t *loc, uint32_t max, uint32_t nIds);
void h10x_refmap_destroy(h10x_refmap *rm);
const char *h10x_refmap_error(const h10x_refmap *rm);
int  h10x_refmap_info(const h10x_refmap *rm, h10x_refmap_info_t *out);
int  h10x_refmap_export(h10x_refmap *rm, const uint32_t **index, const uint32_t **offset, const uint32_t **id, const uint32_t **depth, const uint32_t **rev, const uint32_t **loc);
int  h10x_refmap_query(h10x_refmap *rm, const uint8_t *codes, const uint64_t *seqStart, uint32_t nSeq, int wantSeeds);
int  h10x_refmap_results(h10x_refmap *rm, uint32_t *nQueries, const uint32_t **counts4, const uint64_t **recStart, const h10x_maprec_t **recs, const uint64_t **seedStart,
                         const h10x_mapseed_t **seeds, const uint32_t **seedPos);

void *h10x_device_malloc(int device, uint64_t bytes);
int   h10x_device_mem_info(int device, uint64_t *freeBytes, uint64_t *totalBytes);
int   h10x_device_free(int device, void *ptr);
int   h10x_device_upload(int device, void *dst, const void *src, uint64_t bytes);
int   h10x_device_download(int device, void *dst, const void *src, uint64_t bytes);
int   h10x_device_synchronize(int device);

int  h10x_timing_enable(h10x_ctx *ctx, int on);
int  h10x_timing_count(const h10x_ctx *ctx);
const char *h10x_timing_name(const h10x_ctx *ctx, int i);
int  h10x_timing_get(h10x_ctx *ctx, int i, double *total_ms, uint64_t *launches);
int  h10x_timing_reset(h10x_ctx *ctx);
int  h10x_timing_wait_get(h10x_ctx *ctx, int i, double *ms);
int  h10x_exchange_count(void);
const char *h10x_exchange_name(int i);
int  h10x_exchange_get(h10x_ctx *ctx, int i, uint64_t *calls, uint64_t *bytesOut, uint64_t *bytesIn, uint64_t *maxPeerOut, double *ms, double *msInStages);
int  h10x_exchange_beside(h10x_ctx *ctx, int i);
typedef struct {
  uint64_t pairs;
  uint64_t kmers;
  uint64_t entries;
  uint64_t distinct;
  uint64_t clustered_codes;
  uint64_t sum_good;
  uint64_t sum_good_depth;
  uint64_t sum_hash_clustered;
  uint64_t fallback_blocks;
  uint64_t cluster_class_counts[4];
  uint64_t cluster_first_mode;
  uint64_t cluster_overflow_blocks;
  uint64_t cluster_main[4];
  uint64_t cluster_phase_ticks[8];
  uint64_t list_words[2];
  uint64_t index_table_form;
  uint64_t shard_reply_path;
} h10x_counters;
int  h10x_get_counters(h10x_ctx *ctx, h10x_counters *out);
int  h10x_set_option(h10x_ctx *ctx, const char *name, int64_t value);

#ifdef __cplusplus
}
#endif
#endif
```

Before: 505.2 million read-pairs/s.

## Fuse size scans, reductions and readback mailbox into one single-workgroup kernel

Adds a single-workgroup sizes kernel that computes the exclusive scan, total, max and sentinel count of a small u32 array in one pass. For arrays below a threshold it is fused with the mailbox-post readback kernel, replacing chains of library scan, reduce and count launches plus separate readbacks. It also folds the nHash zeroing into classify, the nHash write into the compaction kernel, and the within computation into within_depth, and it skips allocating the fallback pointer table when no fallback exists. This trims many tiny launches and sync points, at the cost of serialising work on one workgroup for mid-size arrays.

```diff
diff --git a/hash10x_amd/csrc/common.hpp b/hash10x_amd/csrc/common.hpp
--- a/hash10x_amd/csrc/common.hpp
+++ b/hash10x_amd/csrc/common.hpp
@@ -124,6 +124,12 @@
 };
 struct ShardSegInfo { u32 rank, localStart, count, globalBase; u64 entries; };
 
+struct SizesRes { u64 total; u32 max, count; };
+struct PrimTemp;
+struct SizesJob { const u32 *in; u64 *out ; size_t n; u32 sentinel; SizesRes *res ; PrimTemp *temp; };
+constexpr size_t SIZES_MAX_N = 16384;
+constexpr u32 RUN_TILE = H10X_RUN_TILE;
+
 struct Ctx {
   h10x_params prm{};
   u64 keyInv = 1; int keyShift = 0; int keyBits = 64;
@@ -178,6 +184,7 @@
   bool tablesPending = false;
 
   int64_t optMaxSlots = 0;
+  int64_t optSizesMax = 0;
   int64_t optClusterLds = 0;
   int64_t optFirstGlobal = 0;
   int64_t optFirstCap = 0;
@@ -240,6 +247,7 @@
     return 0;
   }
   int syncReadbacks();
+  int syncReadbacks(const SizesJob *job);
   int forkStreams(int n) {
     if (!evFork) {
       if (hipEventCreateWithFlags(&evFork, hipEventDisableTiming) != hipSuccess) return fail("hipEventCreate failed");
diff --git a/hash10x_amd/csrc/h10x_api.hip b/hash10x_amd/csrc/h10x_api.hip
--- a/hash10x_amd/csrc/h10x_api.hip
+++ b/hash10x_amd/csrc/h10x_api.hip
@@ -905,6 +905,7 @@
     if (value && (value < 256 || value > 16384 || (value & (value - 1)))) return h->c.fail("stage_a_max_slots must be a power of two in 256..16384 (or 0)");
     h->c.optMaxSlots = value; return 0;
   }
+  if (!strcmp(name, "sizes_max_n")) { if (value < 0) return h->c.fail("sizes_max_n must be >= 0"); h->c.optSizesMax = value; return 0; }
   if (!strcmp(name, "cluster_lds_budget")) { h->c.optClusterLds = value; return 0; }
   if (!strcmp(name, "cluster_first_global")) { h->c.optFirstGlobal = value; return 0; }
   if (!strcmp(name, "cluster_first_cap")) { h->c.optFirstCap = value; return 0; }
diff --git a/hash10x_amd/csrc/prim.hip b/hash10x_amd/csrc/prim.hip
--- a/hash10x_amd/csrc/prim.hip
+++ b/hash10x_amd/csrc/prim.hip
@@ -50,22 +50,99 @@
   return 0;
 }
 struct MailArgs { const unsigned char *src[Ctx::MAIL_ITEMS]; u32 off[Ctx::MAIL_ITEMS], n[Ctx::MAIL_ITEMS]; u32 count; };
-__global__ void mail_post_kernel(MailArgs a, unsigned char *mail, u32 *flag, u32 seq) {
+__device__ __forceinline__ void mail_post(const MailArgs &a, unsigned char *mail, u32 *flag, u32 seq) {
   for (u32 i = 0; i < a.count; ++i)
     for (u32 b = threadIdx.x; b < a.n[i]; b += blockDim.x) mail[a.off[i] + b] = a.src[i][b];
   __threadfence_system();
   __syncthreads();
   if (threadIdx.x == 0) __hip_atomic_store(flag, seq, __ATOMIC_RELEASE, __HIP_MEMORY_SCOPE_SYSTEM);
 }
-int Ctx::syncReadbacks() {
+__global__ void mail_post_kernel(MailArgs a, unsigned char *mail, u32 *flag, u32 seq) { mail_post(a, mail, flag, seq); }
+
+constexpr int SIZES_THREADS = 1024, SIZES_IPT = 16, SIZES_TILE = SIZES_THREADS * SIZES_IPT, SIZES_WAVES = SIZES_THREADS / WAVE;
+__global__ __launch_bounds__(SIZES_THREADS)
+void sizes_kernel(const u32 *__restrict__ in, u32 n, u32 sentinel, u64 *out, SizesRes *res , MailArgs a, unsigned char *mail, u32 *flag, u32 seq) {
+  __shared__ u64 waveTot[2][SIZES_WAVES];
+  __shared__ u32 waveMax[SIZES_WAVES], waveCnt[SIZES_WAVES];
+  const u32 tid = threadIdx.x, lane = tid & (WAVE - 1), wave = tid / WAVE;
+  u64 carry = 0; u32 mx = 0, cnt = 0; int set = 0;
+  const bool aligned = ((size_t)in & 15) == 0;
+  for (u32 base = 0; base < n; base += SIZES_TILE, set ^= 1) {
+    u32 v[SIZES_IPT]; u64 t = 0;
+#pragma unroll
+    for (int j4 = 0; j4 < SIZES_IPT; j4 += 4) {
+      const u32 i = base + tid * SIZES_IPT + (u32)j4;
+      if (aligned && i + 3 < n) { const uint4 q = *(const uint4 *)(in + i); v[j4] = q.x; v[j4 + 1] = q.y; v[j4 + 2] = q.z; v[j4 + 3] = q.w; }
+      else {
+#pragma unroll
+        for (int j = 0; j < 4; ++j) v[j4 + j] = i + (u32)j < n ? in[i + (u32)j] : 0u;
+      }
+    }
+#pragma unroll
+    for (int j = 0; j < SIZES_IPT; ++j) {
+      const u32 i = base + tid * SIZES_IPT + (u32)j;
+      if (i < n) { mx = v[j] > mx ? v[j] : mx; cnt += v[j] == sentinel ? 1u : 0u; }
+      t += v[j];
+    }
+    u64 inc = t;
+#pragma unroll
+    for (int d = 1; d < WAVE; d <<= 1) { const u64 o = __shfl_up(inc, d); if (lane >= (u32)d) inc += o; }
+    if (lane == WAVE - 1) waveTot[set][wave] = inc;
+    __syncthreads();
+    u64 before = 0, all = 0;
+#pragma unroll
+    for (int q = 0; q < SIZES_WAVES; ++q) { const u64 w = waveTot[set][q]; all += w; if ((u32)q < wave) before += w; }
+    u64 run = carry + before + inc - t;
+#pragma unroll
+    for (int j = 0; j < SIZES_IPT; ++j) { const u32 i = base + tid * SIZES_IPT + (u32)j; if (out && i < n) out[i] = run; run += v[j]; }
+    carry += all;
+  }
+#pragma unroll
+  for (int d = 32; d; d >>= 1) { const u32 o = (u32)__shfl_xor((int)mx, d); mx = o > mx ? o : mx; cnt += (u32)__shfl_xor((int)cnt, d); }
+  if (lane == 0) { waveMax[wave] = mx; waveCnt[wave] = cnt; }
+  __syncthreads();
+  if (tid == 0) {
+    for (int q = 1; q < SIZES_WAVES; ++q) { mx = waveMax[q] > mx ? waveMax[q] : mx; cnt += waveCnt[q]; }
+    res->total = carry; res->max = mx; res->count = cnt;
+  }
+  if (!flag) return;
+  __threadfence();
+  __syncthreads();
+  mail_post(a, mail, flag, seq);
+}
+__global__ void count_equal_kernel(const u32 *__restrict__ in, u32 n, u32 value, u32 *__restrict__ count) {
+  const u32 c = blockIdx.x * blockDim.x + threadIdx.x;
+  const u64 bal = __ballot(c < n && in[c] == value);
+  if ((threadIdx.x & (WAVE - 1)) == 0 && bal) atomicAdd(count, (u32)__popcll(bal));
+}
+__global__ void sizes_total_kernel(const u32 *__restrict__ in, const u64 *__restrict__ out, u32 n, SizesRes *__restrict__ res) { res->total = out[n - 1] + in[n - 1]; }
+
+int Ctx::syncReadbacks() { return syncReadbacks(nullptr); }
+int Ctx::syncReadbacks(const SizesJob *job) {
   hipError_t e = hipSuccess;
+  bool fused = false;
+  if (job && job->n) {
+    if (job->n <= (size_t)(optSizesMax > 0 ? optSizesMax : SIZES_MAX_N)) fused = !pendingReads.empty() && !mailDirect;
+    else {
+      PrimTemp &pt = *job->temp;
+      count_equal_kernel<<<divUp(job->n, 256), 256, 0, stream>>>(job->in, (u32)job->n, job->sentinel, &job->res->count);
+      if (job->out) {
+        H10X_TRY(prim_exclusive_scan_u32_u64(this, pt, job->in, job->out, job->n));
+        sizes_total_kernel<<<1, 1, 0, stream>>>(job->in, job->out, (u32)job->n, job->res);
+      } else H10X_TRY(prim_reduce_sum_u32_u64(this, pt, job->in, &job->res->total, job->n));
+      H10X_TRY(prim_reduce_max_u32(this, pt, job->in, &job->res->max, job->n));
+      job = nullptr;
+    }
+    if (job && !fused) { sizes_kernel<<<1, SIZES_THREADS, 0, stream>>>(job->in, (u32)job->n, job->sentinel, job->out, job->res, MailArgs{}, nullptr, nullptr, 0u); job = nullptr; }
+  } else job = nullptr;
   if (pendingReads.empty() || mailDirect) e = hipStreamSynchronize(stream);
   if (!pendingReads.empty() && e == hipSuccess) {
     MailArgs a; a.count = (u32)pendingReads.size();
     for (u32 i = 0; i < a.count; ++i) { a.src[i] = (const unsigned char *)pendingReads[i].dev; a.off[i] = (u32)pendingReads[i].off; a.n[i] = (u32)pendingReads[i].n; }
     u32 *flag = (u32 *)(mail + MAIL_BYTES);
     const u32 seq = ++mailSeq ? mailSeq : ++mailSeq;
-    mail_post_kernel<<<1, 64, 0, stream>>>(a, mail, flag, seq);
+    if (fused) sizes_kernel<<<1, SIZES_THREADS, 0, stream>>>(job->in, (u32)job->n, job->sentinel, job->out, job->res, a, mail, flag, seq);
+    else mail_post_kernel<<<1, 64, 0, stream>>>(a, mail, flag, seq);
     e = hipGetLastError();
     for (u64 spins = 0; e == hipSuccess && __atomic_load_n(flag, __ATOMIC_ACQUIRE) != seq; ++spins) {
 #if !defined(__HIP_DEVICE_COMPILE__)
diff --git a/hash10x_amd/csrc/stage_a.hip b/hash10x_amd/csrc/stage_a.hip
--- a/hash10x_amd/csrc/stage_a.hip
+++ b/hash10x_amd/csrc/stage_a.hip
@@ -88,7 +88,7 @@
 __global__ void classify_kernel(const u64 *__restrict__ startRec, u32 nBlocks, h10x_block *__restrict__ blocks,
                                 u32 *__restrict__ slots, u32 maxSlots, int packedOK,
                                 u32 *__restrict__ list0, u32 *__restrict__ list1, u32 *__restrict__ list2, u32 *__restrict__ listF,
-                                u32 *__restrict__ counts , int hashLast) {
+                                u32 *__restrict__ counts , int hashLast, u32 *__restrict__ nHash ) {
   const u32 c = blockIdx.x * blockDim.x + threadIdx.x;
   const int lane = threadIdx.x & (WAVE - 1);
   int cls = -1; u32 s = 0;
@@ -103,7 +103,8 @@
         else cls = 3;
       }
     }
-    blocks[c] = b; slots[c] = s;
+    blocks[c] = b; slots[c] = s; nHash[c] = 0;
+    if (c == 0) nHash[nBlocks] = 0;
   }
   u32 *const lists[4] = {list0, list1, list2, listF};
 #pragma unroll
@@ -357,27 +358,18 @@
   for (; i < n; i += stride) if (flags[i]) { outHash[pos[i]] = key[i]; outRead[pos[i]] = slot[i] / nk; }
 }
 
-__global__ void set_nhash_kernel(h10x_block *__restrict__ blocks, const u32 *__restrict__ nHash, u32 nBlocks) {
-  const u32 c = blockIdx.x * blockDim.x + threadIdx.x;
-  if (c < nBlocks) blocks[c].nHash = nHash[c];
-}
-
 struct SrcPtr { const u64 *hash; const u32 *read; };
-__global__ void count_overflow_kernel(const u32 *__restrict__ nHash, u32 nBlocks, u32 *__restrict__ count) {
-  const u32 c = blockIdx.x * blockDim.x + threadIdx.x;
-  const u64 bal = __ballot(c < nBlocks && nHash[c] == NHASH_OVERFLOW);
-  if ((threadIdx.x & (WAVE - 1)) == 0 && bal) atomicAdd(count, (u32)__popcll(bal));
-}
-
 __global__ void compact_entries_kernel(const u64 *__restrict__ stHash, const u32 *__restrict__ stRead, const u64 *__restrict__ capOff,
                                        const SrcPtr *__restrict__ fb ,
                                        const u32 *__restrict__ nHash, const u64 *__restrict__ blockOff, u32 nBlocks,
                                        u64 keyInv, int keyShift, int codeBits ,
-                                       u64 *__restrict__ entHash, u32 *__restrict__ entCode, u32 *__restrict__ entRead) {
+                                       u64 *__restrict__ entHash, u32 *__restrict__ entCode, u32 *__restrict__ entRead, h10x_block *__restrict__ blocks) {
   for (u32 c = blockIdx.x + 1; c < nBlocks; c += gridDim.x) {
-    const u32 n = nHash[c]; if (!n) continue;
+    const u32 n = nHash[c];
+    if (threadIdx.x == 0) blocks[c].nHash = n;
+    if (!n) continue;
     const u64 *sh; const u32 *sr;
-    if (fb[c].hash) { sh = fb[c].hash; sr = fb[c].read; } else { sh = stHash + capOff[c]; sr = stRead + capOff[c]; }
+    if (fb && fb[c].hash) { sh = fb[c].hash; sr = fb[c].read; } else { sh = stHash + capOff[c]; sr = stRead + capOff[c]; }
     const u64 o = blockOff[c];
     if (codeBits) for (u32 i = threadIdx.x; i < n; i += blockDim.x) { entHash[o + i] = (((sh[i] >> keyShift) * keyInv) << codeBits) | c; entRead[o + i] = sr[i]; }
     else for (u32 i = threadIdx.x; i < n; i += blockDim.x) { entHash[o + i] = (sh[i] >> keyShift) * keyInv; entCode[o + i] = c; entRead[o + i] = sr[i]; }
@@ -515,21 +507,19 @@
   u32 maxSlots = 16384;
   if (c->optMaxSlots > 0) maxSlots = (u32)c->optMaxSlots;
   const int packedOK = (2 * k + 16 <= 64) ? 1 : 0;
-  DevBuf<u32> slots, list0, list1, list2, listF, counts, nHash;
+  DevBuf<u32> slots, list0, list1, list2, listF, small, nHash;
   H10X_HIP(c, slots.alloc(nBlocks)); H10X_HIP(c, list0.alloc(nBlocks)); H10X_HIP(c, list1.alloc(nBlocks)); H10X_HIP(c, list2.alloc(nBlocks));
-  H10X_HIP(c, listF.alloc(nBlocks)); H10X_HIP(c, counts.alloc(4)); H10X_HIP(c, nHash.alloc((size_t)nBlocks + 1));
-  H10X_HIP(c, hipMemsetAsync(counts.p, 0, 16, st));
-  H10X_HIP(c, hipMemsetAsync(nHash.p, 0, ((size_t)nBlocks + 1) * 4, st));
+  H10X_HIP(c, listF.alloc(nBlocks)); H10X_HIP(c, small.alloc(12)); H10X_HIP(c, nHash.alloc((size_t)nBlocks + 1));
+  H10X_HIP(c, hipMemsetAsync(small.p, 0, 48, st));
+  u32 *const counts = small.p; SizesRes *const resSlots = (SizesRes *)(small.p + 4), *const resHash = (SizesRes *)(small.p + 8);
   classify_kernel<<<divUp(nBlocks, 256), 256, 0, st>>>(startRec.p, nBlocks, c->blocks.p, slots.p, maxSlots, packedOK,
-                                                      list0.p, list1.p, list2.p, listF.p, counts.p, hashLast ? 1 : 0);
+                                                      list0.p, list1.p, list2.p, listF.p, counts, hashLast ? 1 : 0, nHash.p);
   DevBuf<u64> capOff; H10X_HIP(c, capOff.alloc((size_t)nBlocks + 1));
-  H10X_TRY(prim_exclusive_scan_u32_u64(c, pt, slots.p, capOff.p, nBlocks));
-  u32 hc[4]; u64 capTotal = 0; u32 lastSlots = 0;
-  H10X_TRY(c->readback(hc, counts.p, 16));
-  H10X_TRY(c->readback(&capTotal, capOff.p + (nBlocks - 1), 8));
-  H10X_TRY(c->readback(&lastSlots, slots.p + (nBlocks - 1), 4));
-  H10X_TRY(c->syncReadbacks());
-  capTotal += lastSlots;
+  u32 hc[4]; SizesRes hSlots{0, 0, 0};
+  H10X_TRY(c->readback(hc, counts, 16));
+  H10X_TRY(c->readback(&hSlots, resSlots, sizeof hSlots));
+  { const SizesJob job{slots.p, capOff.p, nBlocks, 0xFFFFFFFFu, resSlots, &pt}; H10X_TRY(c->syncReadbacks(&job)); }
+  const u64 capTotal = hSlots.total;
   c->tstop(T_RUNS);
 
   DevBuf<u64> stHash; DevBuf<u32> stRead;
@@ -560,18 +550,12 @@
   forkGuard.done();
   c->tstop(T_MOSH);
 
-  DevBuf<u32> nOverflow; H10X_HIP(c, nOverflow.alloc(1)); H10X_HIP(c, hipMemsetAsync(nOverflow.p, 0, 4, st));
-  count_overflow_kernel<<<divUp(nBlocks, 256), 256, 0, st>>>(nHash.p, nBlocks, nOverflow.p);
   H10X_HIP(c, c->blockOff.alloc((size_t)nBlocks + 1));
-  H10X_TRY(prim_exclusive_scan_u32_u64(c, pt, nHash.p, c->blockOff.p, (size_t)nBlocks + 1));
-  u64 H = 0, lastStart = 0; u32 hOverflow = 0, hMaxHash = 0xFFFFFFFFu;
-  DevBuf<u32> dMaxHash; H10X_HIP(c, dMaxHash.alloc(1));
-  H10X_TRY(prim_reduce_max_u32(c, pt, nHash.p, dMaxHash.p, nBlocks));
-  H10X_TRY(c->readback(&hMaxHash, dMaxHash.p, 4));
-  H10X_TRY(c->readback(&H, c->blockOff.p + nBlocks, 8));
+  u64 lastStart = 0; SizesRes hSizes{0, 0xFFFFFFFFu, 0};
+  H10X_TRY(c->readback(&hSizes, resHash, sizeof hSizes));
   H10X_TRY(c->readback(&lastStart, startRec.p + (nBlocks - 1), 8));
-  H10X_TRY(c->readback(&hOverflow, nOverflow.p, 4));
-  H10X_TRY(c->syncReadbacks());
+  { const SizesJob job{nHash.p, c->blockOff.p, (size_t)nBlocks + 1, NHASH_OVERFLOW, resHash, &pt}; H10X_TRY(c->syncReadbacks(&job)); }
+  u64 H = hSizes.total; const u32 hOverflow = hSizes.count; u32 hMaxHash = hSizes.max;
   const bool anyFallback = hc[3] || hOverflow;
   std::vector<u32> hNHash, hListF(hc[3]);
   std::vector<u64> hStart;
@@ -624,9 +608,9 @@
   }
 
   c->tstart(T_COMPACT);
-  DevBuf<SrcPtr> dFb; H10X_HIP(c, dFb.alloc(nBlocks));
-  if (hFb.empty()) H10X_HIP(c, hipMemsetAsync(dFb.p, 0, (size_t)nBlocks * sizeof(SrcPtr), st));
-  else {
+  DevBuf<SrcPtr> dFb;
+  if (!hFb.empty()) {
+    H10X_HIP(c, dFb.alloc(nBlocks));
     H10X_HIP(c, hipMemcpyAsync(dFb.p, hFb.data(), (size_t)nBlocks * sizeof(SrcPtr), hipMemcpyHostToDevice, st));
     H10X_TRY(prim_exclusive_scan_u32_u64(c, pt, nHash.p, c->blockOff.p, (size_t)nBlocks + 1));
     H10X_HIP(c, hipMemcpyAsync(&H, c->blockOff.p + nBlocks, 8, hipMemcpyDeviceToHost, st));
@@ -636,7 +620,6 @@
   c->nEntries = H;
   if (!hNHash.empty()) { hMaxHash = 0; for (u32 b = 0; b < nBlocks; ++b) hMaxHash = hNHash[b] > hMaxHash ? hNHash[b] : hMaxHash; }
   c->maxBlockHashes = hMaxHash;
-  set_nhash_kernel<<<divUp(nBlocks, 256), 256, 0, st>>>(c->blocks.p, nHash.p, nBlocks);
   H10X_HIP(c, entHash.alloc(H)); H10X_HIP(c, entRead.alloc(H));
   {
     u64 m = (u64)c->prm.w; int s = 0; while (!(m & 1)) { m >>= 1; ++s; }
@@ -649,7 +632,7 @@
   }
   if (!c->entCodeBits) H10X_HIP(c, entCode.alloc(H));
   if (H) compact_entries_kernel<<<hmin<u32>(nBlocks, 8192), 256, 0, st>>>(stHash.p, stRead.p, capOff.p, dFb.p, nHash.p, c->blockOff.p, nBlocks,
-                                                                        c->keyInv, c->keyShift, c->entCodeBits, entHash.p, entCode.p, entRead.p);
+                                                                        c->keyInv, c->keyShift, c->entCodeBits, entHash.p, entCode.p, entRead.p, c->blocks.p);
   H10X_HIP(c, hipGetLastError());
   if (!hFb.empty()) H10X_HIP(c, hipStreamSynchronize(st));
   c->tstop(T_COMPACT);
diff --git a/hash10x_amd/csrc/stage_b.hip b/hash10x_amd/csrc/stage_b.hip
--- a/hash10x_amd/csrc/stage_b.hip
+++ b/hash10x_amd/csrc/stage_b.hip
@@ -17,17 +17,69 @@
     dHash[d] = sHash[i]; dFirst[d] = sCode[i]; segStart[d] = (u32)i; iota[d] = d;
   }
 }
-__global__ void seg_scatter_packed_kernel(const u64 *__restrict__ sKey, int cb,
-                                          const u32 *__restrict__ ord, u64 n, Val16 *__restrict__ dVal, u32 *__restrict__ dFirst, u32 *__restrict__ rows) {
-  u64 i = (u64)blockIdx.x * blockDim.x + threadIdx.x;
-  const u64 stride = (u64)gridDim.x * blockDim.x;
+constexpr int RUN_THREADS = 256, RUN_ROUNDS = RUN_TILE / RUN_THREADS, RUN_WAVES = RUN_THREADS / WAVE;
+static_assert(RUN_TILE % RUN_THREADS == 0 && RUN_ROUNDS * RUN_WAVES <= WAVE, "a tile's wave counts are scanned by one wave");
+__device__ __forceinline__ void run_edges(const u64 *__restrict__ sKey, int cb, u64 i, u64 n, u64 &k, bool &head, bool &tail) {
+  const int lane = threadIdx.x & (WAVE - 1);
+  const bool valid = i < n;
+  k = valid ? sKey[i] : 0;
+  u64 kp = __shfl_up(k, 1), kn = __shfl_down(k, 1);
+  if (lane == 0 && valid && i > 0) kp = sKey[i - 1];
+  if (lane == WAVE - 1 && i + 1 < n) kn = sKey[i + 1];
+  head = valid && (i == 0 || (k >> cb) != (kp >> cb));
+  tail = valid && (i + 1 == n || (kn >> cb) != (k >> cb));
+}
+__global__ __launch_bounds__(RUN_THREADS)
+void run_count_kernel(const u64 *__restrict__ sKey, int cb, u64 n, u32 *__restrict__ tileCount) {
+  __shared__ u32 sCount;
+  if (threadIdx.x == 0) sCount = 0;
+  __syncthreads();
+  const u64 t0 = (u64)blockIdx.x * RUN_TILE;
+  u32 mine = 0;
+#pragma unroll
+  for (int r = 0; r < RUN_ROUNDS; ++r) {
+    u64 k; bool head, tail;
+    run_edges(sKey, cb, t0 + (u64)r * RUN_THREADS + threadIdx.x, n, k, head, tail);
+    mine += (u32)__popcll(__ballot(head));
+  }
+  if ((threadIdx.x & (WAVE - 1)) == 0 && mine) atomicAdd(&sCount, mine);
+  __syncthreads();
+  if (threadIdx.x == 0) tileCount[blockIdx.x] = sCount;
+}
+__global__ __launch_bounds__(RUN_THREADS)
+void seg_scatter_packed_kernel(const u64 *__restrict__ sKey, int cb, const u64 *__restrict__ tileBase , u64 n,
+                               Val16 *__restrict__ dVal, u32 *__restrict__ dFirst, u32 *__restrict__ rows) {
+  __shared__ u32 sPre[RUN_ROUNDS * RUN_WAVES];
+  const int lane = threadIdx.x & (WAVE - 1), wave = threadIdx.x / WAVE;
   const u64 cmask = ((u64)1 << cb) - 1;
-  for (; i < n; i += stride) {
-    const u64 k = sKey[i]; const u32 code = (u32)(k & cmask);
+  const u64 t0 = (u64)blockIdx.x * RUN_TILE;
+  u64 k[RUN_ROUNDS], hb[RUN_ROUNDS]; u32 tl = 0;
+#pragma unroll
+  for (int r = 0; r < RUN_ROUNDS; ++r) {
+    bool head, tail;
+    run_edges(sKey, cb, t0 + (u64)r * RUN_THREADS + threadIdx.x, n, k[r], head, tail);
+    hb[r] = __ballot(head); tl |= tail ? 1u << r : 0u;
+    if (lane == 0) sPre[r * RUN_WAVES + wave] = (u32)__popcll(hb[r]);
+  }
+  __syncthreads();
+  if (wave == 0) {
+    const u32 v = lane < RUN_ROUNDS * RUN_WAVES ? sPre[lane] : 0u; u32 inc = v;
+#pragma unroll
+    for (int d = 1; d < WAVE; d <<= 1) { const u32 o = (u32)__shfl_up((int)inc, d); if (lane >= d) inc += o; }
+    if (lane < RUN_ROUNDS * RUN_WAVES) sPre[lane] = inc - v;
+  }
+  __syncthreads();
+  const u64 base = tileBase[blockIdx.x];
+#pragma unroll
+  for (int r = 0; r < RUN_ROUNDS; ++r) {
+    const u64 i = t0 + (u64)r * RUN_THREADS + threadIdx.x;
+    if (i >= n) continue;
+    const u32 code = (u32)(k[r] & cmask);
     rows[i] = code;
-    const u32 d = ord[i], d1 = ord[i + 1];
-    if (d1 != d) { dVal[d].a = k >> cb; dVal[d].b = (u32)i; dFirst[d] = code; }
-    if (i + 1 == n || ord[i + 2] != d1) dVal[d1 - 1].c = (u32)i + 1;
+    const bool head = (hb[r] >> lane) & 1;
+    const u32 d = (u32)(base + sPre[r * RUN_WAVES + wave] + (u32)__popcll(hb[r] & ((2ULL << lane) - 1))) - 1u;
+    if (head) { dVal[d].a = k[r] >> cb; dVal[d].b = (u32)i; dFirst[d] = code; }
+    if ((tl >> r) & 1) dVal[d].c = (u32)i + 1;
   }
 }
 __global__ void assign_index_v16_kernel(const Val16 *__restrict__ val, u32 U, u64 w , u64 *__restrict__ hashValue, u32 *__restrict__ hashDepth,
@@ -191,8 +243,8 @@
   }
 }
 int stageB_blockClassLists(Ctx *c, DevBuf<u32> &lists, DevBuf<u32> &counts) {
-  H10X_HIP(c, lists.alloc((size_t)3 * c->nBlocks)); H10X_HIP(c, counts.alloc(4));
-  H10X_HIP(c, hipMemsetAsync(counts.p, 0, 16, c->stream));
+  H10X_HIP(c, lists.alloc((size_t)3 * c->nBlocks)); H10X_HIP(c, counts.alloc(12));
+  H10X_HIP(c, hipMemsetAsync(counts.p, 0, 48, c->stream));
   if (c->nBlocks) block_class_kernel<<<divUp(c->nBlocks, 256), 256, 0, c->stream>>>(c->blockOff.p, c->nBlocks, lists.p, counts.p);
   return 0;
 }
@@ -398,16 +450,27 @@
   u32 U = 0;
   DevBuf<u64> dHash; DevBuf<u32> dFirst, segStart, iota, order, dFirstSorted; DevBuf<Val16> dVal, dValSorted;
   {
-    DevBuf<u32> ord;
-    H10X_HIP(c, ord.alloc(H + 2));
-    H10X_TRY(prim_run_ordinals_u64(c, pt, sHash.p, cb, ord.p, H));
-    H10X_TRY(c->readback(&U, ord.p + H, 4));
-    H10X_TRY(c->syncReadbacks());
+    DevBuf<u32> ord, tileCount, small; DevBuf<u64> tileBase;
+    const u32 nTiles = divUp(H, RUN_TILE);
+    if (cb && H) {
+      SizesRes hRuns{0, 0, 0};
+      H10X_HIP(c, tileCount.alloc(nTiles)); H10X_HIP(c, tileBase.alloc(nTiles)); H10X_HIP(c, small.alloc(4));
+      H10X_HIP(c, hipMemsetAsync(small.p, 0, 16, st));
+      run_count_kernel<<<nTiles, RUN_THREADS, 0, st>>>(sHash.p, cb, H, tileCount.p);
+      H10X_TRY(c->readback(&hRuns, small.p, sizeof hRuns));
+      { const SizesJob job{tileCount.p, tileBase.p, nTiles, 0xFFFFFFFFu, (SizesRes *)small.p, &pt}; H10X_TRY(c->syncReadbacks(&job)); }
+      U = (u32)hRuns.total;
+    } else if (H) {
+      H10X_HIP(c, ord.alloc(H + 2));
+      H10X_TRY(prim_run_ordinals_u64(c, pt, sHash.p, cb, ord.p, H));
+      H10X_TRY(c->readback(&U, ord.p + H, 4));
+      H10X_TRY(c->syncReadbacks());
+    }
     if ((u64)U + 1 > (tableSize >> 2) - 2) return c->fail("hashTableSize is too small");
     H10X_HIP(c, dFirst.alloc(U)); H10X_HIP(c, dFirstSorted.alloc(U));
     if (cb) { H10X_HIP(c, dVal.alloc(U)); H10X_HIP(c, dValSorted.alloc(U)); }
     else { H10X_HIP(c, dHash.alloc(U)); H10X_HIP(c, segStart.alloc((size_t)U + 1)); H10X_HIP(c, iota.alloc(U)); H10X_HIP(c, order.alloc(U)); }
-    if (H && cb) seg_scatter_packed_kernel<<<gH, 256, 0, st>>>(sHash.p, cb, ord.p, H, dVal.p, dFirst.p, sCode.p);
+    if (H && cb) seg_scatter_packed_kernel<<<nTiles, RUN_THREADS, 0, st>>>(sHash.p, cb, tileBase.p, H, dVal.p, dFirst.p, sCode.p);
     else if (H) {
       seg_scatter_kernel<<<gH, 256, 0, st>>>(sHash.p, sCode.p, ord.p, H, dHash.p, dFirst.p, segStart.p, iota.p);
       H10X_HIP(c, hipMemsetD32Async((hipDeviceptr_t)(segStart.p + U), (int)(u32)H, 1, st));
diff --git a/hash10x_amd/csrc/stage_c.hip b/hash10x_amd/csrc/stage_c.hip
--- a/hash10x_amd/csrc/stage_c.hip
+++ b/hash10x_amd/csrc/stage_c.hip
@@ -14,19 +14,30 @@
 constexpr int ROWS_IN_FLIGHT = 4;
 constexpr int RCHUNK = 4;
 
-__global__ void within_kernel(const u32 *__restrict__ depth, u32 hashNumber, int lo, int hi, u8 *__restrict__ within) {
-  const u32 i = blockIdx.x * blockDim.x + threadIdx.x;
-  if (i >= hashNumber) return;
-  const int n = (int)depth[i];
-  if (n >= lo && n < hi) within[i] = 1;
-}
-__global__ void within_depth_kernel(const u32 *__restrict__ depth, const u8 *__restrict__ within, u32 hashNumber, u32 *__restrict__ out,
-                                    const u64 *__restrict__ rowStart, u32 rowShift, u64 *__restrict__ rowInfo ) {
-  const u32 i = blockIdx.x * blockDim.x + threadIdx.x;
-  if (i < hashNumber) {
-    const u32 wd = within[i] ? depth[i] + 1 : 0;
-    out[i] = wd; if (rowInfo) rowInfo[i] = (u64)(u32)(rowStart[i] >> rowShift) | ((u64)wd << 32);
-  }
+__global__ __launch_bounds__(256)
+void within_depth_kernel(const u32 *__restrict__ depth, u8 *__restrict__ within, u32 hashNumber, int lo, int hi, int setRange, int fresh, u32 *__restrict__ out,
+                         const u64 *__restrict__ rowStart, u32 rowShift, u64 *__restrict__ rowInfo ,
+                         u32 *red) {
+  __shared__ u32 sMax;
+  if (threadIdx.x == 0) sMax = 0;
+  __syncthreads();
+  u32 m = 0;
+  for (u32 i = blockIdx.x * blockDim.x + threadIdx.x; i < hashNumber; i += gridDim.x * blockDim.x) {
+    const u32 d = depth[i];
+    u8 w = fresh ? (u8)0 : within[i];
+    if (setRange && (int)d >= lo && (int)d < hi && !w) { w = 1; within[i] = 1; }
+    else if (fresh) within[i] = 0;
+    const u32 wd = w ? d + 1 : 0;
+    if (out) out[i] = wd;
+    if (rowInfo) rowInfo[i] = (u64)(u32)(rowStart[i] >> rowShift) | ((u64)wd << 32);
+    m = wd > m ? wd : m;
+  }
+  if (!red) return;
+#pragma unroll
+  for (int sft = 32; sft; sft >>= 1) { const u32 o = (u32)__shfl_xor((int)m, sft); m = o > m ? o : m; }
+  if ((threadIdx.x & (WAVE - 1)) == 0 && m) atomicMax(&sMax, m);
+  __syncthreads();
+  if (threadIdx.x == 0 && sMax > __hip_atomic_load(red, __ATOMIC_RELAXED, __HIP_MEMORY_SCOPE_AGENT)) atomicMax(red, sMax);
 }
 
 template <typename KT>
@@ -131,29 +142,33 @@
   c->haveGood = false;
   c->tstart(T_GOOD);
   const u32 U1 = c->hashNumber; const u32 nBlocks = c->nBlocks; const u64 H = c->nEntries;
+  int setRange = 0, fresh = 0;
   if (!(c->haveRange && lo == c->rangeMin && hi == c->rangeMax)) {
-    if (!c->haveRange) { H10X_HIP(c, c->within.alloc(U1)); H10X_HIP(c, hipMemsetAsync(c->within.p, 0, U1, st)); }
-    within_kernel<<<divUp(U1, 256), 256, 0, st>>>(c->hashDepth.p, U1, lo, hi, c->within.p);
+    if (!c->haveRange) { H10X_HIP(c, c->within.alloc(U1)); fresh = 1; }
+    setRange = 1;
     c->haveRange = true; c->rangeMin = lo; c->rangeMax = hi;
     if (hi > 0 && (u32)hi > c->rangeHiMax) c->rangeHiMax = (u32)hi;
   }
   XGuard xGuard(c);
-  if (c->sharded) { c->tstop(T_GOOD); H10X_TRY(shard_exchangeRows(c)); c->tstart(T_GOOD); }
-  DevBuf<u64> key, keyS; DevBuf<u32> key32, keyS32, off32, segEnd, wdepth, red;
-  H10X_HIP(c, off32.alloc((size_t)nBlocks + 1));
-  H10X_HIP(c, segEnd.alloc(nBlocks)); H10X_HIP(c, wdepth.alloc(U1)); H10X_HIP(c, red.alloc(2));
+  if (c->sharded) {
+    if (setRange) within_depth_kernel<<<hmin<u32>(divUp(U1, 256), (u32)c->numCU * 8), 256, 0, st>>>(c->hashDepth.p, c->within.p, U1, lo, hi, setRange, fresh, nullptr, nullptr, 0, nullptr, nullptr);
+    setRange = fresh = 0;
+    c->tstop(T_GOOD); H10X_TRY(shard_exchangeRows(c)); c->tstart(T_GOOD);
+  }
+  DevBuf<u64> key, keyS; DevBuf<u32> key32, keyS32, off32, segEnd, wdepth, lists, counts;
+  H10X_HIP(c, segEnd.alloc(nBlocks)); H10X_HIP(c, wdepth.alloc(U1));
   H10X_HIP(c, c->nGood.alloc(nBlocks)); H10X_HIP(c, c->goodPos.alloc(H)); H10X_HIP(c, c->goodEntries.alloc(nBlocks)); H10X_HIP(c, c->goodRow.alloc(H));
   const u32 goodDepthBound = hmin<u32>(c->depthBound, c->rangeHiMax ? c->rangeHiMax - 1 : 0);
   const bool narrow = goodDepthBound <= 65535u;
   const bool byBlocks = narrow && c->maxBlockHashes <= BLOCK_SORT_MAX;
   DevBuf<u64> rowInfo; if (byBlocks) H10X_HIP(c, rowInfo.alloc(U1));
-  within_depth_kernel<<<divUp(U1, 256), 256, 0, st>>>(c->hashDepth.p, c->within.p, U1, wdepth.p, c->rowStart.p, (u32)c->rowShift, rowInfo.p);
-  H10X_TRY(prim_reduce_max_u32(c, pt, wdepth.p, red.p, U1));
+  if (byBlocks) H10X_TRY(stageB_blockClassLists(c, lists, counts));
+  else { H10X_HIP(c, counts.alloc(12)); H10X_HIP(c, hipMemsetAsync(counts.p, 0, 48, st)); }
+  u32 *const red = counts.p + 4;
+  within_depth_kernel<<<hmin<u32>(divUp(U1, 256), (u32)c->numCU * 8), 256, 0, st>>>(c->hashDepth.p, c->within.p, U1, lo, hi, setRange, fresh, wdepth.p, c->rowStart.p, (u32)c->rowShift, rowInfo.p, red);
   if (byBlocks) {
     int db = 1; while (db < 16 && (goodDepthBound >> db)) ++db;
     const int sortBits = db + 1;
-    DevBuf<u32> lists, counts;
-    H10X_TRY(stageB_blockClassLists(c, lists, counts));
     const unsigned gridBig = hmin<u32>(nBlocks, (u32)c->numCU * 8), gridSmall = hmin<u32>(nBlocks, 65535u * 4);
     const int side = c->maxBlockHashes > BLOCK_SORT_CAP1 ? 2 : (c->maxBlockHashes > BLOCK_SORT_CAP0 ? 1 : 0);
     ForkGuard forkGuard(c);
@@ -175,17 +190,16 @@
                                                                              key32.p, c->nGood.p, segEnd.p, c->goodEntries.p);
   else good_keys_kernel<u64><<<hmin<u32>(nBlocks, 16384), 256, 0, st>>>(c->clusHash.p, c->blockOff.p, c->blocks.p, nBlocks, wdepth.p,
                                                                       key.p, c->nGood.p, segEnd.p, c->goodEntries.p);
-  H10X_TRY(prim_reduce_max_u32(c, pt, c->nGood.p, red.p + 1, nBlocks));
-  DevBuf<u64> redSum; H10X_HIP(c, redSum.alloc(1));
-  H10X_TRY(prim_reduce_sum_u32_u64(c, pt, c->nGood.p, redSum.p, nBlocks));
-  u32 hr[2]; u64 sumGood = 0;
-  H10X_TRY(c->readback(hr, red.p, 8));
-  H10X_TRY(c->readback(&sumGood, redSum.p, 8));
-  H10X_TRY(c->syncReadbacks());
+  u32 hr[2]; u64 sumGood = 0; SizesRes hGood{0, 0, 0};
+  H10X_TRY(c->readback(hr, red, 4));
+  H10X_TRY(c->readback(&hGood, red + 4, sizeof hGood));
+  { const SizesJob job{c->nGood.p, nullptr, nBlocks, 0xFFFFFFFFu, (SizesRes *)(red + 4), &pt}; H10X_TRY(c->syncReadbacks(&job)); }
+  hr[1] = hGood.max; sumGood = hGood.total;
   hr[0] = hr[0] ? hr[0] - 1 : 0;
   c->maxGoodDepth = hr[0]; c->maxGood = hr[1]; c->meanGood = nBlocks > 1 ? (u32)(sumGood / (nBlocks - 1)) : 0;
-  offsets32c_kernel<<<divUp((u64)nBlocks + 1, 256), 256, 0, st>>>(c->blockOff.p, nBlocks + 1, off32.p);
   if (H && !byBlocks) {
+    H10X_HIP(c, off32.alloc((size_t)nBlocks + 1));
+    offsets32c_kernel<<<divUp((u64)nBlocks + 1, 256), 256, 0, st>>>(c->blockOff.p, nBlocks + 1, off32.p);
     if (narrow) {
       H10X_TRY(prim_seg_sort_keys_u32(c, pt, key32.p, keyS32.p, (u32)H, nBlocks, off32.p, segEnd.p, 0, 16 + bitsForC(hr[0])));
       good_pos_kernel<u32><<<(unsigned)hmin<u64>(divUp(H, 256), 65535u * 2), 256, 0, st>>>(keyS32.p, H, c->goodPos.p);
diff --git a/hash10x_amd/host/h10x_host.c b/hash10x_amd/host/h10x_host.c
--- a/hash10x_amd/host/h10x_host.c
+++ b/hash10x_amd/host/h10x_host.c
@@ -16,7 +16,7 @@
 #define ARRAY_MAGIC 8918274
 typedef struct { int32_t magic, pad0; uint64_t base; int32_t dim, size, max, pad1; } array_hdr;
 
-enum { N_KNOBS = 23 };
+enum { N_KNOBS = 24 };
 struct h10x_session {
   int k, w, r, B, N, chunk, ct, device;
   int timing;
@@ -30,7 +30,7 @@
   char err[1024];
 };
 static const char *const knobName[N_KNOBS] = {"cluster_stamps", "cluster_lds_budget", "cluster_first_global", "cluster_first_cap",
-                                              "cluster_big_ranks", "cluster_threads0", "cluster_budget0", "shard_row_shift", "shard_rows_fake_base", "stage_a_max_slots", "cluster_narrow_first", "index_no_pack", "shard_delta_lists", "index_priv_table", "cluster_tr_packed", "cluster_tr_est_div", "cluster_tr_class_t", "shard_reply_sort", "shard_owner_cut", "shard_overlap", "index_probed_table", "fqb_slab", "molmap_global"};
+                                              "cluster_big_ranks", "cluster_threads0", "cluster_budget0", "shard_row_shift", "shard_rows_fake_base", "stage_a_max_slots", "cluster_narrow_first", "index_no_pack", "shard_delta_lists", "index_priv_table", "cluster_tr_packed", "cluster_tr_est_div", "cluster_tr_class_t", "shard_reply_sort", "shard_owner_cut", "shard_overlap", "index_probed_table", "fqb_slab", "molmap_global", "sizes_max_n"};
 
 static int fail(h10x_session *s, const char *fmt, ...) {
   va_list ap; va_start(ap, fmt); vsnprintf(s->err, sizeof s->err, fmt, ap); va_end(ap);
diff --git a/include/h10x.h b/include/h10x.h
--- a/include/h10x.h
+++ b/include/h10x.h
@@ -314,6 +314,8 @@
 int  h10x_get_counters(h10x_ctx *ctx, h10x_counters *out);
 int  h10x_set_option(h10x_ctx *ctx, const char *name, int64_t value);
 
+#define H10X_RUN_TILE 2048
+
 #ifdef __cplusplus
 }
 #endif
diff --git a/scratch/sizes_switch.hip b/scratch/sizes_switch.hip
--- /dev/null
+++ b/scratch/sizes_switch.hip
@@ -0,0 +1,43 @@
+#include "../hash10x_amd/csrc/common.hpp"
+#include "../hash10x_amd/csrc/prim.hpp"
+#include <chrono>
+#include <algorithm>
+using namespace h10x;
+
+static int run(Ctx &c, size_t n) {
+  PrimTemp pt; DevBuf<u32> in, small; DevBuf<u64> out;
+  H10X_HIP(&c, in.alloc(n)); H10X_HIP(&c, out.alloc(n)); H10X_HIP(&c, small.alloc(4));
+  std::vector<u32> h(n); u64 want = 0; u32 wmax = 0;
+  for (size_t i = 0; i < n; ++i) { h[i] = (u32)((i * 2654435761u) >> 20) % 3000u; want += h[i]; wmax = std::max(wmax, h[i]); }
+  H10X_HIP(&c, hipMemcpy(in.p, h.data(), n * 4, hipMemcpyHostToDevice));
+  for (int mode = 0; mode < 2; ++mode) {
+    c.optSizesMax = mode == 0 ? (int64_t)n : 1;
+    std::vector<double> us;
+    for (int rep = 0; rep < 60; ++rep) {
+      SizesRes r{0, 0, 0};
+      const auto t0 = std::chrono::steady_clock::now();
+      H10X_HIP(&c, hipMemsetAsync(small.p, 0, 16, c.stream));
+      H10X_TRY(c.readback(&r, small.p, sizeof r));
+      const SizesJob job{in.p, out.p, n, 0xFFFFFFFFu, (SizesRes *)small.p, &pt};
+      H10X_TRY(c.syncReadbacks(&job));
+      const auto t1 = std::chrono::steady_clock::now();
+      if (r.total != want || r.max != wmax || r.count != 0) return c.fail("wrong sizes at n = %zu, mode %d: total %llu (want %llu), max %u (%u), count %u", n, mode, r.total, want, r.max, wmax, r.count);
+      if (rep >= 10) us.push_back(std::chrono::duration<double, std::micro>(t1 - t0).count());
+    }
+    std::sort(us.begin(), us.end());
+    printf("n %9zu  %-22s median %8.1f us  min %8.1f us\n", n, mode == 0 ? "one workgroup" : "library chain", us[us.size() / 2], us[0]);
+  }
+  return 0;
+}
+
+int main(int argc, char **argv) {
+  static Ctx c;
+  if (hipStreamCreateWithFlags(&c.stream, hipStreamNonBlocking) != hipSuccess) { fprintf(stderr, "no stream\n"); return 2; }
+  AllocScope::stream() = c.stream;
+  std::vector<size_t> ns;
+  for (int i = 1; i < argc; ++i) ns.push_back((size_t)atof(argv[i]));
+  if (ns.empty()) ns = {10000, 32768, 65536, 131072, 1000000, 1600000};
+  for (size_t n : ns) if (run(c, n)) { fprintf(stderr, "%s\n", c.err.c_str()); return 1; }
+  (void)hipStreamSynchronize(c.stream);
+  return 0;
+}
```

Result: no change. 511.8 million read-pairs/s, median of 4 (+1.3%).
